# xiaohong-huang/RTK-Visual-Inertial-Navigation

Hardware: AMD Instinct MI355X
Metric: gauss_newton_iterations_per_sec (higher is better)
Workload: dtype f64; 1 GPU; BASELINE cfg4: batch of 512 independent cfg3 windows (20 keyframes, 300 features, 3000 observations, 19 IMU factors, 10 satellites x 20 epochs carrier-phase+pseudorange, gauge prior) over the job, 8 dogleg iterations per solve; windows=512, windows_rank0=512

## Files before the change

### rtk_visual_inertial_navigation_amd/csrc/swf_engine.hip

```cpp
#include <hip/hip_runtime.h>
#include <algorithm>
#include <chrono>
#include <cmath>
#include <cstdio>
#include <cstdlib>
#include <cstring>
#include <string>
#include <memory>
#include <thread>
#include <vector>
#include "../../include/swf_solver.h"
#include "swf_kernels2.h"
#include "swf_kernels3.h"
#include "swf_kernels4.h"
#include "swf_lambda.h"
#include "swf_features.h"
#include "swf_fixprior.h"
#include "swf_plan.h"

static thread_local std::string g_err;
static int fail(int code, const std::string& msg) { g_err = msg; return code; }
#define HIPCHK(x) do { hipError_t e_ = (x); if (e_ != hipSuccess) return fail(SWF_E_NODEVICE, std::string(#x) + ": " + hipGetErrorString(e_)); } while (0)

extern "C" const char* swf_last_error(void) { return g_err.c_str(); }
// ... 101 lines not shown
        bytes = (bytes + 255) & ~(size_t)255;
        if (v.empty() || v.back().used + bytes > v.back().cap) {
            size_t want = std::max(bytes, v.empty() ? first : std::min<size_t>(2 * v.back().cap, (size_t)256 << 20));
            Slab sl;
            sl.dev = (char*)slab_cache().acquire(want);
            if (!sl.dev) return nullptr;
            sl.cap = want;
            if (mirrored) sl.host.assign(want, 0);
            v.push_back(std::move(sl));
        }
        Slab& sl = v.back();
        void* p = sl.dev + sl.used;
        sl.used += bytes;
        return p;
    }
    template <class T> int put(const std::vector<T>& h, const T** out, size_t min_elems = 1) {
        size_t n = std::max(h.size(), min_elems), bytes = n * sizeof(T);
        void* p = bump(data, bytes, true, (size_t)4 << 20);
        if (!p) return -1;
        Slab& sl = data.back();
        char* m = sl.host.data() + ((char*)p - sl.dev);
        if (!h.empty()) memcpy(m, h.data(), h.size() * sizeof(T));
        if (sealed) {
            if (hipMemcpy(p, m, (bytes + 255) & ~(size_t)255, hipMemcpyHostToDevice) != hipSuccess) return -1;
            sl.flushed = sl.used;
        }
        *out = (const T*)p;
        return 0;
    }
    template <class T> int zeros(size_t n, T** out) {
        n = std::max<size_t>(n, 1);
        void* p = bump(zero, n * sizeof(T), false, (size_t)16 << 20);
        if (!p) return -1;
        if (sealed) { if (hipMemset(p, 0, n * sizeof(T)) != hipSuccess) return -1; zero.back().flushed = zero.back().used; }
        *out = (T*)p;
        return 0;
    }
    int flush() {
        for (Slab& sl : data) if (sl.used > sl.flushed) { if (hipMemcpy(sl.dev + sl.flushed, sl.host.data() + sl.flushed, sl.used - sl.flushed, hipMemcpyHostToDevice) != hipSuccess) return -1; sl.flushed = sl.used; }
        for (Slab& sl : zero) if (sl.used > sl.flushed) { if (hipMemset(sl.dev + sl.flushed, 0, sl.used - sl.flushed) != hipSuccess) return -1; sl.flushed = sl.used; }
        sealed = true;
        return 0;
    }
    void release() {
        for (Slab& sl : data) slab_cache().give(sl.dev, sl.cap);
        for (Slab& sl : zero) slab_cache().give(sl.dev, sl.cap);
        data.clear(); zero.clear(); sealed = false;
    }
};

struct swf_batch {
    int device = 0;
    DevBatch D{};
    DevPool pool;
    hipStream_t stream = nullptr;
    std::vector<WinRec> win;
    std::vector<HostWin> hw;
    int max_tiles = 0, max_prior_dim = 0, max_red = 0, min_red = 1 << 30, n_cu = 256;
    bool clc_imu[5] = { false, false, false, false, false };
    CompArgs CA{}; CompMeta CM{}; int n_comp = 0, comp_nmax = 0, comp_nmin = 1 << 30; long long comp_ne = 0;
    bool comp_eigen_root = false;
    void* h_sum = nullptr; size_t h_sum_bytes = 0;
    double* h_x = nullptr;
    double* co_pose0 = nullptr; double* co_sb0 = nullptr;
    int* mg_tail = nullptr; double* mg_A = nullptr; double* mg_b = nullptr; double* mg_J = nullptr; double* mg_r0 = nullptr; double* mg_w = nullptr; int* mg_rank = nullptr; double* mg_M = nullptr;
    bool mg_valid = false; int mg_ld = 0;
    bool mg_host = false; std::vector<double> h_mgA, h_mgJ, h_mgb, h_mgr0, h_mgw; std::vector<int> h_mgrank;
    double* mg_resM = nullptr; double* mg_resb = nullptr; int* mg_resok = nullptr;
    int* mg_rot = nullptr; int* mg_bjok = nullptr; unsigned long long* mg_crit = nullptr;
    int* tc_tail = nullptr; double* tc_A = nullptr; double* tc_Q = nullptr; double* tc_X = nullptr; int* tc_rank = nullptr; bool tc_valid = false; int tc_ld = 0;
    int* am_first = nullptr; int4* am_pairs = nullptr; double* am_rec = nullptr; int am_rec_ld = 0;
    bool am_valid = false, am_host = false; std::vector<double> h_am;
    std::vector<int> am_nb;
    std::vector<int> am_h_first; std::vector<int4> am_h_pairs;
    FixWin* fx_win = nullptr; int* fx_tailcol = nullptr; double* fx_A = nullptr; double* fx_b = nullptr; double* fx_J = nullptr; double* fx_r0 = nullptr;
    double* fx_eig = nullptr; double* fx_x0 = nullptr; int* fx_rank = nullptr; int* fx_applied = nullptr; int fx_ldn = 0, fx_ldx = 0;
    bool fx_valid = false, fx_host = false; FixPriorArgs fx_args{};
    std::vector<FixWin> fx_h_win; std::vector<int> fx_h_tailcol, fx_sel;
    std::vector<double> h_fxA, h_fxb, h_fxJ, h_fxr0, h_fxeig, h_fxx0; std::vector<int> h_fxrank, h_fxapplied;
    bool fc_built = false, fc_valid = false, fc_host = false; FeatArgs fc{}; char* fc_out = nullptr; size_t fc_bytes = 0; int fc_nfeat = 0;
    std::vector<int> fc_feat0; std::vector<char> h_fc;
    hipStream_t aux = nullptr; hipEvent_t ev_fork[3] = { nullptr, nullptr, nullptr };
    ~swf_batch() {
        if (aux) { (void)hipStreamSynchronize(aux); handle_cache().give(aux); }
        for (auto& e : ev_fork) handle_cache().give(e, false);
    }
    WinState* ws_primary = nullptr; WinState* ws_alt = nullptr; WinState* ws_alt2 = nullptr;
    bool no_decide_fuse = false;
    bool no_step_fuse = false;
    int n_pch_split = 0;
    bool no_spec = false;
    bool no_comp_fuse = false;
    bool lat_fuse = false;
    bool rr4_has15 = false, rr4_has16 = false;
    int rr_nmax = 256;
    bool L_full = false;
    int asm_programs = 0;
    int ls_qpb = 1, ls_var = 0, ls_kms = 8; bool ls_folded = false, s_direct = false;
    bool full_final = false;
    int ls_gqpb = 4;
    int timing = 0;
    swf_timing last{};
    std::vector<hipEvent_t> ev;
    std::vector<int> ev_kind;
    int ev_used = 0;
    int64_t jac_bytes = 0, proj_bytes = 0, chol_flops = 0, lm_schur_flops = 0, lm_schur_flops_sym = 0, lm_schur_mfma = 0;
    int last_mode = -1;
};

extern "C" int swf_batch_create(const swf_flat_window* const* windows, int32_t n, void* stream, swf_batch** out) {
    if (!windows || n <= 0 || !out) return fail(SWF_E_INVALID, "swf_batch_create: bad arguments");
    int ndev = 0;
    if (hipGetDeviceCount(&ndev) != hipSuccess || ndev <= 0)
        return fail(SWF_E_NODEVICE, "no HIP device: this library has no CPU fallback");
    int n_cu = 256;
    { int dev = 0; hipDeviceProp_t pr; if (hipGetDevice(&dev) == hipSuccess && hipGetDeviceProperties(&pr, dev) == hipSuccess && pr.multiProcessorCount > 0) n_cu = pr.multiProcessorCount; }
    Plan B;
    {
        std::string err;
        int prc = plan_build(windows, n, plan_shape_from_env(n_cu), B, err);
        if (prc != SWF_OK) return fail(prc, err);
    }
    std::unique_ptr<swf_batch> owner(new swf_batch());
    swf_batch* b = owner.get();
    b->device = current_device();
    b->stream = (hipStream_t)stream;
    b->n_cu = n_cu;
    b->no_comp_fuse = getenv("SWF_NO_COMP_FUSE") != nullptr;
    b->no_spec = getenv("SWF_NO_SPEC_EVAL") != nullptr;
    b->no_step_fuse = getenv("SWF_NO_STEP_FUSE") != nullptr;
    b->no_decide_fuse = getenv("SWF_NO_DECIDE_FUSE") != nullptr;
    b->full_final = getenv("SWF_FULL_FINAL_ELIM") != nullptr;
    b->max_tiles = B.max_tiles; b->max_prior_dim = B.max_prior_dim; b->max_red = B.max_red; b->min_red = B.min_red;
    b->rr_nmax = B.rr_nmax; b->rr4_has15 = B.rr4_has15; b->rr4_has16 = B.rr4_has16; b->n_pch_split = B.n_pch_split;
    b->lat_fuse = B.lat_fuse; b->asm_programs = B.asm_programs;
    b->ls_qpb = B.ls_qpb; b->ls_var = B.ls_var; b->ls_kms = B.ls_kms; b->ls_gqpb = B.ls_gqpb; b->ls_folded = B.ls_folded; b->s_direct = B.s_direct;
    for (int k = 0; k < 5; k++) b->clc_imu[k] = B.clc_imu[k];
    b->n_comp = B.n_comp; b->comp_nmax = B.comp_nmax; b->comp_nmin = B.comp_nmin; b->comp_ne = B.comp_ne;
    b->jac_bytes = B.jac_bytes; b->proj_bytes = B.proj_bytes; b->chol_flops = B.chol_flops;
    b->lm_schur_flops = B.lm_schur_flops; b->lm_schur_flops_sym = B.lm_schur_flops_sym; b->lm_schur_mfma = B.lm_schur_mfma;
    if (B.want_aux) {
        bool ok = (b->aux = handle_cache().stream()) != nullptr;
        for (int i = 0; i < 3 && ok; i++) ok = (b->ev_fork[i] = handle_cache().event(false)) != nullptr;
        if (!ok) { handle_cache().give(b->aux); b->aux = nullptr; }
    }
    DevBatch& D = b->D;
    DevPool& P = b->pool;
    int rc = 0;
    D.n_win = n; D.n_x = (int)B.n_x; D.n_loc_total = (int)B.n_loc; D.max_iter_trace = SWF_MAX_TRACE; D.rr_nmax = B.rr_nmax;
    D.n_lmb = B.n_lmb; D.n_pch = B.n_pch; D.n_proj = B.n_proj; D.n_lm = B.n_lm; D.n_fr = B.n_fr; D.n_fsb = B.n_fsb;
    D.n_gf = (int)B.gf.size(); D.n_imu = (int)B.imu_gf.size(); D.n_sc = (int)B.sc_gf.size(); D.n_prior = (int)B.prior_gf.size(); D.n_idp = (int)B.idp_gf.size();
    D.n_cl = (int)B.cl.size(); D.n_pair = (int)B.pair.size(); D.n_pd = B.n_pd; D.n_po = B.n_po; D.n_cle = B.n_cle;
    for (int k = 0; k < 5; k++) D.n_clc[k] = B.n_clc[k];
    D.as_max_ne = B.as_max_ne; D.as_max_nv = B.as_max_nv;
#define PUT(field) rc |= P.put(B.field, &D.field)
    PUT(win);
    PUT(lmb_rec); PUT(pch_q); PUT(pch_r0); PUT(prior_nch);
    PUT(blk_xoff); PUT(blk_loc); PUT(blk_gs);
    PUT(loc2x); PUT(x_var);
    PUT(p_win); PUT(p_xpose); PUT(p_xex); PUT(p_xlm);
    PUT(p_lpose); PUT(p_llm); PUT(p_fr); PUT(p_lm); PUT(p_uv);
    PUT(lm_win); PUT(lm_obs0); PUT(lm_loc); PUT(lm_col); PUT(lm_fmask);
    PUT(sch_c0); PUT(sch_rec); PUT(sch_km);
    PUT(fr_obs0); PUT(fr_obs); PUT(fr_red);
    PUT(fsb_rec);
    PUT(fsb_perm); PUT(fsb_foff);
    PUT(gf);
    PUT(s_x); PUT(s_loc); PUT(s_ls); PUT(s_joff); PUT(s_ccol);
    PUT(imu_pre); PUT(cp_dat); PUT(pr_dat); PUT(dop_dat); PUT(sp_w); PUT(gx_dat);
    PUT(imu_gf); PUT(sc_gf); PUT(prior_gf); PUT(idp_gf);
    PUT(sc_jt); PUT(imu_jt);
    PUT(prior_dim); PUT(prior_Joff); PUT(prior_roff); PUT(prior_x0off);
    PUT(prior_Jt);
    PUT(prior_colloc); PUT(prior_colcc); PUT(s_pcol); PUT(s_pxo);
    PUT(prior_J); PUT(prior_r0); PUT(prior_x0);
    PUT(cl); PUT(cl_fac); PUT(cl_frow); PUT(cm_loc); PUT(cm_ls); PUT(cm_col);
    PUT(cv_loc);
    PUT(pc_coff); PUT(pc_cld); PUT(pc_voff);
    PUT(asw); PUT(s_tnz);
    PUT(as_dst); PUT(as_cnt); PUT(as_src0); PUT(as_aux); PUT(as_src);
    PUT(av_loc); PUT(av_red); PUT(av_cnt); PUT(av_src0); PUT(av_i); PUT(av_src);
    PUT(pair_d); PUT(pair_o);
    PUT(cle_rec);
    for (int k = 0; k < 5; k++) PUT(clc_rec[k]);
#undef PUT
    {
        const double* ci = nullptr; const double* di = nullptr;
        rc |= P.put(B.C_init, &ci); rc |= P.put(B.dgraw_init, &di);
        D.C = (double*)ci; D.cv_dgraw = (double*)di;
    }
    CompArgs& A = b->CA; CompMeta& Mt = b->CM;
    const int nc = B.n_comp;
    if (nc) {
        A.n = nc; A.want_jac = 1; A.n_iq = (int)B.co_iq_f.size();
        rc |= P.put(B.co_M, &A.M); rc |= P.put(B.co_N, &A.N); rc |= P.put(B.co_eo, &A.e_off); rc |= P.put(B.co_no, &A.n_off);
        rc |= P.put(B.co_pno, &A.pn_off); rc |= P.put(B.co_nno, &A.nn_off); rc |= P.put(B.co_go, &A.g_off); rc |= P.put(B.co_g2o, &A.g2_off);
        { const double* t1 = nullptr; const double* t2 = nullptr; rc |= P.put(B.co_pose, &t1); rc |= P.put(B.co_sb, &t2); A.pose = (double*)t1; A.sb = (double*)t2; }
        { const double* t1 = nullptr; const double* t2 = nullptr; rc |= P.put(B.co_pose, &t1); rc |= P.put(B.co_sb, &t2); b->co_pose0 = (double*)t1; b->co_sb0 = (double*)t2; }
        rc |= P.put(B.co_pose_lin, &A.pose_lin); rc |= P.put(B.co_sb_lin, &A.sb_lin); rc |= P.put(B.co_Hpp, &A.Hpp); rc |= P.put(B.co_HpN, &A.HpN);
        rc |= P.put(B.co_rhs_p, &A.rhs_p); rc |= P.put(B.co_HNN, &A.HNN); rc |= P.put(B.co_rhsN, &A.rhsN); rc |= P.put(B.co_pre, &A.pre); rc |= P.put(B.co_pbgw, &A.pbgw);
        rc |= P.put(B.co_mid, &A.mid); rc |= P.put(B.co_H12, &A.H12);
        rc |= P.put(B.co_iq_f, &A.iq_f); rc |= P.put(B.co_iq_k, &A.iq_k);
        rc |= P.put(B.co_win, &Mt.win); rc |= P.put(B.co_xo_off, &Mt.xo_off); rc |= P.put(B.co_xo, &Mt.xo);
        rc |= P.put(B.co_Joff, &Mt.Joff); rc |= P.put(B.co_roff, &Mt.roff); rc |= P.put(B.co_x0off, &Mt.x0off); rc |= P.put(B.co_Coff, &Mt.Coff); rc |= P.put(B.co_voff, &Mt.voff);
        Mt.prior_J = (double*)D.prior_J; Mt.prior_Jt = (double*)D.prior_Jt; Mt.prior_r0 = (double*)D.prior_r0; Mt.prior_x0 = (double*)D.prior_x0;
    }
    rc |= P.zeros((size_t)B.fs_tot * FS_VAL, &D.fs_part);
    rc |= P.zeros((size_t)std::max<long long>(B.n_loc, 1), &D.jsc);
    rc |= P.zeros(B.n_x, &D.x); rc |= P.zeros(B.n_x, &D.xc); rc |= P.zeros(B.n_x, &D.x0);
    rc |= P.zeros(B.n_loc, &D.g); rc |= P.zeros(B.n_loc, &D.diag); rc |= P.zeros(B.n_loc, &D.rhs); rc |= P.zeros(B.n_loc, &D.vc);
    rc |= P.zeros(B.n_loc, &D.y); rc |= P.zeros(B.n_loc, &D.step);
    rc |= P.zeros(B.S_tot, &D.S); rc |= P.zeros(B.Lt_tot, &D.L);
    if (B.want_Linv) rc |= P.zeros((size_t)n * (CB_MAXT - 1) * 256, &D.Linv);
    if (B.want_Wk) rc |= P.zeros(B.Lt_tot, &D.Wk);
    rc |= P.zeros((size_t)n, &D.ws); rc |= P.zeros((size_t)n, &b->ws_alt); rc |= P.zeros((size_t)n, &b->ws_alt2); rc |= P.zeros((size_t)n * SWF_MAX_TRACE, &D.trace);
    b->ws_primary = D.ws;
    size_t np = (size_t)D.n_proj;
    rc |= P.zeros(2 * np, &D.p_r); rc |= P.zeros(12 * np, &D.p_Jp); rc |= P.zeros(6 * np, &D.p_Jl);
    rc |= P.zeros((size_t)std::max(1, D.n_fsb), &D.p_cpart); rc |= P.zeros((size_t)std::max(1, D.n_lmb), &D.p_apart);
    rc |= P.zeros((size_t)std::max(1, D.n_pch), &D.pr_cpart); rc |= P.zeros((size_t)std::max(1, D.n_pch), &D.pr_apart);
    rc |= P.zeros(6 * (size_t)D.n_lm, &D.lm_Einv); rc |= P.zeros(3 * (size_t)D.n_lm, &D.lm_g);
    rc |= P.zeros(B.P_tot * GEMM_SPLIT, &D.P);
    rc |= P.zeros((size_t)std::max(1, 6 * B.n_fr) * GEMM_SPLIT, &D.lmq);
    rc |= P.zeros((size_t)B.r_tot, &D.g_r); rc |= P.zeros((size_t)B.j_tot, &D.g_J);
    rc |= P.zeros((size_t)D.n_gf, &D.g_cost); rc |= P.zeros((size_t)D.n_gf, &D.g_aux);
    rc |= P.zeros((size_t)B.v_tot, &D.cv_graw); rc |= P.zeros((size_t)B.v_tot, &D.cv_cs);
    rc |= P.zeros((size_t)B.e_tot, &D.cE);
    if (nc) {
        const size_t ne = (size_t)B.co_eo[nc], nn = (size_t)B.co_no[nc], ng = (size_t)B.co_go[nc], ng2 = (size_t)B.co_g2o[nc];
        rc |= P.zeros(ne * 225, &A.hmn_inv); rc |= P.zeros(ne * 225, &A.hmn_2); rc |= P.zeros(ne * 225, &A.hmn_0);
        rc |= P.zeros((size_t)B.co_pno[nc], &A.hmn_N); rc |= P.zeros(ne * 15, &A.rhsmn);
        rc |= P.zeros(ng2, &A.Hd); rc |= P.zeros(ng, &A.rd); rc |= P.zeros(ng2, &A.Ld); rc |= P.zeros(ng, &A.r0);
        rc |= P.zeros((size_t)nc * 32, &A.old); rc |= P.zeros(nn, &A.N_old); rc |= P.zeros((size_t)nc, &A.history); rc |= P.zeros((size_t)nc, &A.status);
        rc |= P.zeros((size_t)nc * 32, &Mt.outer); rc |= P.zeros(nn, &Mt.Nv); rc |= P.zeros((size_t)nc, &Mt.active);
        A.outer = Mt.outer; A.Nv = Mt.Nv; A.active = Mt.active;
        rc |= P.zeros(ng, &A.res_out); rc |= P.zeros(ng2, &A.jac_out);
        rc |= P.zeros((ne + nc) * 450, &A.Jw); rc |= P.zeros((ne + nc) * 16, &A.rw);
        rc |= P.zeros((size_t)nc, &A.todo);
    }
    if (!rc) rc = P.flush();
    if (rc) { P.release(); return fail(SWF_E_NODEVICE, "device allocation / upload failed"); }
    b->win = std::move(B.win); b->hw = std::move(B.hw);
    *out = owner.release();
    int urc = swf_batch_upload_state(b);
    if (urc != SWF_OK) { swf_batch_destroy(b); *out = nullptr; return urc; }
    return SWF_OK;
}

extern "C" int swf_shard_partition(int32_t n, int32_t G, int32_t k, int32_t* first, int32_t* count) {
    if (n < 0 || G <= 0 || k < 0 || k >= G || !first || !count) return fail(SWF_E_INVALID, "swf_shard_partition: bad arguments");
    const int q = n / G, r = n % G;
    *first = k * q + std::min(k, r); *count = q + (k < r ? 1 : 0);
    return SWF_OK;
}

extern "C" int swf_batch_create_on(int32_t device, const swf_flat_window* const* windows, int32_t n, void* stream, swf_batch** out) {
    int ndev = 0;
    if (hipGetDeviceCount(&ndev) != hipSuccess || ndev <= 0) return fail(SWF_E_NODEVICE, "no HIP device: this library has no CPU fallback");
    if (device < 0 || device >= ndev || device >= SWF_MAX_DEVICES) return fail(SWF_E_INVALID, "swf_batch_create_on: no such device");
    DeviceGuard dg_(device);
    return swf_batch_create(windows, n, stream, out);
}

extern "C" int swf_batch_create_sharded(const swf_flat_window* const* windows, int32_t n, uint32_t device_mask,
                                        swf_batch** out_batches, int32_t* out_first, int32_t* out_count, int32_t* n_batches) {
    if (!windows || n <= 0 || !out_batches || !n_batches) return fail(SWF_E_INVALID, "swf_batch_create_sharded: bad arguments");
    int ndev = 0;
    if (hipGetDeviceCount(&ndev) != hipSuccess || ndev <= 0) return fail(SWF_E_NODEVICE, "no HIP device: this library has no CPU fallback");
    std::vector<int> devs;
    for (int d = 0; d < ndev && d < SWF_MAX_DEVICES; d++) if (device_mask == 0 || ((device_mask >> d) & 1u)) devs.push_back(d);
    if (devs.empty()) return fail(SWF_E_INVALID, "swf_batch_create_sharded: device_mask selects no visible device");
    const int G = (int)std::min<size_t>(devs.size(), (size_t)n);
    *n_batches = 0;
    for (int k = 0; k < G; k++) {
        int32_t lo = 0, cnt = 0;
        swf_shard_partition(n, G, k, &lo, &cnt);
        const int hi = lo + cnt;
        swf_batch* bk = nullptr;
        int rc = swf_batch_create_on(devs[k], windows + lo, hi - lo, nullptr, &bk);
        if (rc != SWF_OK) { for (int q = 0; q < *n_batches; q++) swf_batch_destroy(out_batches[q]); *n_batches = 0; return rc; }
        out_batches[k] = bk;
        if (out_first) out_first[k] = lo;
        if (out_count) out_count[k] = hi - lo;
        *n_batches = k + 1;
    }
    return SWF_OK;
}

extern "C" int swf_batch_device(swf_batch* b, int32_t* device) { if (!b || !device) return fail(SWF_E_INVALID, "bad arguments"); *device = b->device; return SWF_OK; }

extern "C" int swf_batch_destroy(swf_batch* b) {
    if (!b) return SWF_OK;
    DeviceGuard dg_(b->device);
    (void)hipStreamSynchronize(b->stream);
    if (b->aux) (void)hipStreamSynchronize(b->aux);
    for (auto& e : b->ev) handle_cache().give(e, true);
    if (b->h_x) (void)hipHostFree(b->h_x);
    if (b->h_sum) (void)hipHostFree(b->h_sum);
    b->pool.release();
    delete b;
    return SWF_OK;
}

extern "C" int swf_batch_upload_state(swf_batch* b) {
    DeviceGuard dg_(b ? b->device : -1);
    if (!b) return fail(SWF_E_INVALID, "null batch");
    const size_t nx = (size_t)b->D.n_x;
    if (!b->h_x && nx) HIPCHK(hipHostMalloc((void**)&b->h_x, nx * sizeof(double), hipHostMallocDefault));
    double* xh = b->h_x;
    for (size_t i = 0; i < b->win.size(); i++) {
        const HostWin& h = b->hw[i];
        double* p = xh + b->win[i].x_base;
        memcpy(p, h.pose, sizeof(double) * 7 * h.n_pose); p += 7 * h.n_pose;
        memcpy(p, h.sb, sizeof(double) * 9 * h.n_sb); p += 9 * h.n_sb;
        memcpy(p, h.lm, sizeof(double) * 3 * h.n_lm); p += 3 * h.n_lm;
        memcpy(p, h.sc, sizeof(double) * h.n_sc);
    }
    HIPCHK(hipMemcpyAsync(b->D.x, xh, nx * sizeof(double), hipMemcpyHostToDevice, b->stream));
    HIPCHK(hipMemcpyAsync(b->D.x0, b->D.x, nx * sizeof(double), hipMemcpyDeviceToDevice, b->stream));
    HIPCHK(hipMemcpyAsync(b->D.xc, b->D.x, nx * sizeof(double), hipMemcpyDeviceToDevice, b->stream));
    std::vector<double> hp, hs;
    if (b->n_comp) {
        hp.resize((size_t)b->comp_ne * 7); hs.resize((size_t)b->comp_ne * 9);
        for (size_t i = 0; i < b->win.size(); i++) {
            const HostWin& h = b->hw[i];
            if (!h.comp_ne) continue;
            memcpy(hp.data() + (size_t)h.comp_e0 * 7, h.comp_pose, sizeof(double) * 7 * h.comp_ne);
            memcpy(hs.data() + (size_t)h.comp_e0 * 9, h.comp_sb, sizeof(double) * 9 * h.comp_ne);
        }
        HIPCHK(hipMemcpyAsync(b->co_pose0, hp.data(), hp.size() * sizeof(double), hipMemcpyHostToDevice, b->stream));
        HIPCHK(hipMemcpyAsync(b->co_sb0, hs.data(), hs.size() * sizeof(double), hipMemcpyHostToDevice, b->stream));
        HIPCHK(hipMemcpyAsync(b->CA.pose, b->co_pose0, hp.size() * sizeof(double), hipMemcpyDeviceToDevice, b->stream));
        HIPCHK(hipMemcpyAsync(b->CA.sb, b->co_sb0, hs.size() * sizeof(double), hipMemcpyDeviceToDevice, b->stream));
        HIPCHK(hipMemsetAsync(b->CA.history, 0, (size_t)b->n_comp * sizeof(int), b->stream));
// ... 83 lines not shown
            }
            slot = b->ev_used++;
            b->ev_kind.push_back(kind);
            (void)hipEventRecord(b->ev[2 * slot], bst);
        }
        ~Bracket() { if (slot >= 0) (void)hipEventRecord(L.b->ev[2 * slot + 1], bst); }
    };
    static int nb(size_t n, int per) { return (int)((n + per - 1) / per); }
    bool comp_fused = false;
    bool comp_fuse_ok(int write_S) const {
        const DevBatch& D = b->D;
        if (!b->n_comp || !write_S || b->no_comp_fuse || !b->lat_fuse || b->aux || b->comp_eigen_root) return false;
        if (b->comp_nmax > CO_SMALLN || b->ls_var > 1 || !D.n_lm || D.n_imu || D.n_idp || b->max_prior_dim > PRIOR_LDS_DIM) return false;
        if (D.n_clc[0] || D.n_clc[1]) return false;
        const int crow = (b->n_comp + D.n_win - 1) / D.n_win;
        return (long long)D.n_win * (GEMM_SPLIT / b->ls_qpb + crow) <= b->n_cu;
    }
    void lin_eval(int write_S, bool spec = false) {
        DevBatch Dv = b->D; Dv.spec = spec ? 1 : 0;
        const DevBatch& D = Dv;
        comp_fused = !spec && comp_fuse_ok(write_S);
        if (comp_fused) {
            hipLaunchKernelGGL(k_comp_gather_prep, dim3(b->n_comp), dim3(256), 0, st, D, b->CA, b->CM);
            Segs S{}; S.e[0] = D.n_fsb; S.e[1] = S.e[0] + nb(D.n_sc, 256);
            {
                Bracket t(*this, SWF_K_EVAL_PS);
                hipLaunchKernelGGL(k_eval_ps_comp_imu, dim3(S.e[1] + (b->CA.n_iq + 7) / 8), dim3(256), 0, st, D, S, b->CA);
            }
            {
                Bracket t(*this, SWF_K_LM_SCHUR);
                lm_qpb = b->ls_qpb; lm_folded = b->ls_folded;
                const int np = GEMM_SPLIT / b->ls_qpb, crow = (b->n_comp + D.n_win - 1) / D.n_win;
                const int qpb = b->ls_qpb, sd = b->s_direct ? 1 : 0, kms = b->ls_kms;
                dim3 grid(D.n_win, np + crow);
                if (b->ls_var == 0) hipLaunchKernelGGL((k_lm_comp<8, 2, 2, 80>), grid, dim3(LS_NT(8, 2)), 0, st, D, O, b->CA, b->CM, qpb, 0, kms, sd, np);
                else hipLaunchKernelGGL((k_lm_comp<8, 5, 2, 144>), grid, dim3(LS_NT(8, 2)), 0, st, D, O, b->CA, b->CM, qpb, 0, kms, sd, np);
                lm_next = ls_tiles_per_launch();
            }
            if (D.n_prior) {
                Segs P{}; P.e[2] = D.n_pch;
                hipLaunchKernelGGL((k_eval_ps<true, true>), dim3(P.e[2]), dim3(256), 0, st, D, P);
            }
            return;
        }
        if (b->n_comp && !spec) {
            const bool wide = b->n_comp <= 2 * b->n_cu;
            {
            hipLaunchKernelGGL(k_comp_gather_prep, dim3(b->n_comp), dim3(256), 0, st, D, b->CA, b->CM);
            hipLaunchKernelGGL(k_comp_imu, dim3((b->CA.n_iq + 7) / 8), dim3(256), 0, st, b->CA);
            if (b->comp_nmin <= CO_SMALLN) {
                if (wide) hipLaunchKernelGGL((k_comp_elim<CO_SMALLN, 1024>), dim3(b->n_comp), dim3(1024), 0, st, b->CA, 0);
                else {
                    if (b->comp_nmin <= CO_TINYN) hipLaunchKernelGGL((k_comp_elim<CO_TINYN, 256>), dim3(b->n_comp), dim3(256), 0, st, b->CA, 0);
                    if (b->comp_nmax > CO_TINYN) hipLaunchKernelGGL((k_comp_elim<CO_SMALLN, 256>), dim3(b->n_comp), dim3(256), 0, st, b->CA, CO_TINYN + 1);
                }
            }
            if (b->comp_nmax > CO_SMALLN) {
                if (wide) hipLaunchKernelGGL((k_comp_elim<CO_MAXN, 1024>), dim3(b->n_comp), dim3(1024), 0, st, b->CA, CO_SMALLN + 1);
                else hipLaunchKernelGGL((k_comp_elim<CO_MAXN, 256>), dim3(b->n_comp), dim3(256), 0, st, b->CA, CO_SMALLN + 1);
            }
            if (b->comp_eigen_root) {
                if (b->comp_nmax <= CO_SMALLN) hipLaunchKernelGGL(k_comp_eigroot<CO_SMALLN>, dim3(b->n_comp), dim3(256), 0, st, b->CA);
                else hipLaunchKernelGGL(k_comp_eigroot<CO_MAXN>, dim3(b->n_comp), dim3(512), 0, st, b->CA);
            }
            hipLaunchKernelGGL(k_comp_scatter, dim3(b->n_comp), dim3(256), 0, st, D, b->CA, b->CM);
            }
        }
        const bool fork = b->aux && !spec;
        hipStream_t sa = fork ? b->aux : st;
        if (fork) { (void)hipEventRecord(b->ev_fork[0], st); (void)hipStreamWaitEvent(b->aux, b->ev_fork[0], 0); }
        bool imu_fused = false;
        if (D.n_proj + D.n_sc + D.n_prior) {
            Bracket t(*this, SWF_K_EVAL_PS);
            bool pf = b->max_prior_dim <= PRIOR_LDS_DIM;
            Segs S{}; S.e[0] = D.n_fsb; S.e[1] = S.e[0] + nb(D.n_sc, 256); S.e[2] = S.e[1] + (pf ? D.n_pch : 0);
            imu_fused = b->lat_fuse && D.n_imu > 0;
            S.e[3] = S.e[2] + (imu_fused ? nb(D.n_imu, IMU_FPB) : 0);
            if (imu_fused) hipLaunchKernelGGL((k_eval_ps<true, true, true>), dim3(S.e[3]), dim3(256), 0, st, D, S);
            else hipLaunchKernelGGL((k_eval_ps<true, true>), dim3(S.e[2]), dim3(256), 0, st, D, S);
        }
        if (D.n_idp) hipLaunchKernelGGL(k_eval_idp<true>, GRID(D.n_idp, 128), dim3(128), 0, st, D);
        if (D.n_prior && b->max_prior_dim > PRIOR_LDS_DIM) { Bracket t(*this, SWF_K_EVAL_PRIOR); hipLaunchKernelGGL(k_eval_prior<true>, dim3(D.n_pch), dim3(256), (2 * b->max_prior_dim + 16) * sizeof(double), st, D); }
        if (fork) (void)hipEventRecord(b->ev_fork[1], st);
        if (D.n_imu && !imu_fused) { Bracket t(*this, SWF_K_EVAL_IMU, sa); hipLaunchKernelGGL(k_eval_imu<true>, GRID(D.n_imu, IMU_FPB), dim3(IMU_FPB * IMU_LPF), 0, sa, D); }
    }
    void lin_elim(int write_S) {
        DevBatch& D = b->D;
        bool clq_fused = false;
        if (comp_fused) {
            Bracket t(*this, SWF_K_CLIQUE_ELIM);
            if (D.n_clc[3]) {
                hipLaunchKernelGGL(k_clique_big2, dim3(D.n_clc[3] + D.n_clc[2]), dim3(CB_NT), 0, st, D, O);
                if (D.n_clc[4]) hipLaunchKernelGGL(k_clique_tall<false>, dim3(D.n_clc[4]), dim3(256), 0, st, D, O);
            } else if (D.n_clc[4] + D.n_clc[2]) hipLaunchKernelGGL(k_clique_tall2, dim3(D.n_clc[4] + D.n_clc[2]), dim3(256), 0, st, D, O);
        } else if (D.n_lm) {
            Bracket t(*this, write_S ? SWF_K_LM_SCHUR : SWF_K_LM_ELIM);
            lm_qpb = b->ls_qpb; lm_folded = b->ls_folded;
            if (!write_S && !b->full_final) {
                dim3 grid(D.n_win, GEMM_SPLIT / b->ls_gqpb);
                hipLaunchKernelGGL((k_lm_schur<8, 2, 2, 80, false, true>), grid, dim3(256), 0, st, D, O, b->ls_gqpb, 0, 0, 0);
            } else if (!write_S) {
                dim3 grid(D.n_win, GEMM_SPLIT / lm_qpb);
                hipLaunchKernelGGL((k_lm_schur<8, 2, 2, 80, false>), grid, dim3(256), 0, st, D, O, lm_qpb, 0, 0, 0);
            } else {
                const int crow = D.n_win > 0 ? (D.n_clc[2] + D.n_win - 1) / D.n_win : 0;
                clq_fused = clq_fuse_ok();
                lm_launch(0, st, clq_fused ? crow : 0);
                lm_next = ls_tiles_per_launch();
            }
        }
        {
            hipStream_t sa = b->aux ? b->aux : st;
            if (b->aux) (void)hipStreamWaitEvent(b->aux, b->ev_fork[1], 0);
            auto cstream = [&](int cls) { return (b->aux && !b->clc_imu[cls]) ? st : sa; };
            if (comp_fused) {
                for (; lm_next < b->max_tiles; lm_next += ls_tiles_per_launch()) { Bracket t(*this, SWF_K_LM_SCHUR, sa); lm_launch(lm_next, sa); }
            } else {
            const bool grad = !write_S && !b->full_final;
            if (D.n_clc[1]) {
                Bracket t(*this, SWF_K_CLIQUE_ELIM, cstream(1));
                if (grad) hipLaunchKernelGGL((k_clique_elim<32, 48, 9, 1, true>), dim3(D.n_clc[1]), dim3(64), 0, cstream(1), D, O);
                else hipLaunchKernelGGL((k_clique_elim<32, 48, 9, 1>), dim3(D.n_clc[1]), dim3(64), 0, cstream(1), D, O);
            }
            if (D.n_clc[0]) {
                Bracket t(*this, SWF_K_CLIQUE_ELIM, cstream(0));
                if (grad) hipLaunchKernelGGL((k_clique_elim<48, 32, 1, 0, true>), dim3(D.n_clc[0]), dim3(64), 0, cstream(0), D, O);
                else hipLaunchKernelGGL((k_clique_elim<48, 32, 1, 0>), dim3(D.n_clc[0]), dim3(64), 0, cstream(0), D, O);
            }
            if (D.n_clc[2] && !clq_fused) {
                Bracket t(*this, SWF_K_CLIQUE_ELIM, cstream(2));
                if (b->lat_fuse) {
                    if (grad) hipLaunchKernelGGL(k_clique_elim4<true>, dim3(D.n_clc[2]), dim3(256), 0, cstream(2), D, O);
                    else hipLaunchKernelGGL(k_clique_elim4<false>, dim3(D.n_clc[2]), dim3(256), 0, cstream(2), D, O);
                }
                else if (grad) hipLaunchKernelGGL((k_clique_elim<64, 64, 9, 2, true>), dim3(D.n_clc[2]), dim3(64), 0, cstream(2), D, O);
                else hipLaunchKernelGGL((k_clique_elim<64, 64, 9, 2>), dim3(D.n_clc[2]), dim3(64), 0, cstream(2), D, O);
            }
            if (D.n_clc[3]) { Bracket t(*this, SWF_K_CLIQUE_ELIM, cstream(3)); hipLaunchKernelGGL(k_clique_big, dim3(D.n_clc[3]), dim3(CB_NT), 0, cstream(3), D, O); }
            if (D.n_clc[4]) {
                Bracket t(*this, SWF_K_CLIQUE_ELIM, cstream(4));
                if (grad) hipLaunchKernelGGL(k_clique_tall<true>, dim3(D.n_clc[4]), dim3(256), 0, cstream(4), D, O);
                else hipLaunchKernelGGL(k_clique_tall<false>, dim3(D.n_clc[4]), dim3(256), 0, cstream(4), D, O);
            }
            if (write_S && D.n_lm) {
                for (; lm_next < b->max_tiles; lm_next += ls_tiles_per_launch()) { Bracket t(*this, SWF_K_LM_SCHUR, sa); lm_launch(lm_next, sa); }
            }
            }
            if (b->aux) (void)hipEventRecord(b->ev_fork[2], b->aux);
        }
        if (b->n_pch_split) hipLaunchKernelGGL(k_prior_graw, dim3(D.n_pch), dim3(256), 0, st, D);
        if (b->aux) (void)hipStreamWaitEvent(st, b->ev_fork[2], 0);
        if (D.n_pd) {
            Bracket t(*this, SWF_K_ASSEMBLE);
            const int nbS = write_S ? nb((size_t)D.as_max_ne, 256) : 0, nbV = nb((size_t)D.as_max_nv, 256);
            hipLaunchKernelGGL(k_assemble_flat, dim3(nbS + nbV, D.n_win), dim3(256), 0, st, D, O, write_S, nbS);
        }
    }
    void reduced() {
        DevBatch& D = b->D;
        Bracket t(*this, SWF_K_CHOL);
        if (b->max_red <= CB_NMAX) {
            if (b->min_red <= b->rr_nmax) {
                if (b->min_red <= 224) hipLaunchKernelGGL(k_chol_rr4<14>, dim3(D.n_win), dim3(R4_NT), 0, st, D, export_full ? 1 : 0);
                if (b->rr4_has15) hipLaunchKernelGGL(k_chol_rr4<15>, dim3(D.n_win), dim3(R4_NT), 0, st, D, export_full ? 1 : 0);
                if (b->rr4_has16) hipLaunchKernelGGL(k_chol_rr4<16>, dim3(D.n_win), dim3(R4_NT), 0, st, D, export_full ? 1 : 0);
            }
            if (b->max_red > b->rr_nmax && D.Wk) {
                const int Tc = (b->max_red + 15) / 16;
                const int nbw = std::max(1, std::min(CC_NB, b->n_cu / D.n_win));
                for (int j = 0; j < Tc; j += 2) hipLaunchKernelGGL(k_chol_col, dim3(D.n_win, nbw), dim3(CC_NT), 0, st, D, j);
                hipLaunchKernelGGL(k_chol_big<true>, dim3(D.n_win), dim3(1024), 0, st, D);
            } else if (b->max_red > b->rr_nmax) hipLaunchKernelGGL(k_chol_big<false>, dim3(D.n_win), dim3(1024), 0, st, D);
        }
        else if (b->max_red + 1 <= 256) hipLaunchKernelGGL(k_chol_solve<256>, dim3(D.n_win), dim3(256), 0, st, D);
        else hipLaunchKernelGGL(k_chol_solve<1024>, dim3(D.n_win), dim3(1024), 0, st, D);
    }
    void step_rest() {
        DevBatch& D = b->D;
        {
            Bracket t(*this, SWF_K_POST_CHOL);
            Segs S{};
            S.e[0] = D.n_lmb; S.e[1] = S.e[0] + nb((size_t)D.n_cle * 16, 256);
            S.e[2] = S.e[1]; S.e[3] = S.e[2] + nb(D.n_sc, 256);
            S.e[4] = S.e[3] + nb((size_t)D.n_imu * 16, 256); S.e[5] = S.e[4] + D.n_pch;
            if (D.n_win < b->n_cu) { if (S.e[5]) hipLaunchKernelGGL(k_post_chol<0>, dim3(S.e[5]), dim3(256), 0, st, D, O, S); }
            else {
                if (S.e[0]) hipLaunchKernelGGL(k_post_chol<1>, dim3(S.e[0]), dim3(256), 0, st, D, O, S);
                if (S.e[5] > S.e[0]) hipLaunchKernelGGL(k_post_chol<2>, dim3(S.e[5] - S.e[0]), dim3(256), 0, st, D, O, S);
            }
        }
        if (!step_fused) dogleg();
    }
    bool step_fused = false;
    void dogleg() {
        DevBatch& D = b->D;
        Bracket t(*this, SWF_K_DOGLEG);
        if (b->lat_fuse) hipLaunchKernelGGL((k_dogleg<16, 4>), dim3(D.n_win), dim3(CTL_NT), 0, st, D, O);
        else hipLaunchKernelGGL((k_dogleg<4, 2>), dim3(D.n_win), dim3(CTL_NT), 0, st, D, O);
    }
    bool clq_fuse_ok() const {
        const DevBatch& D = b->D;
        const int crow = D.n_win > 0 ? (D.n_clc[2] + D.n_win - 1) / D.n_win : 0;
        return b->lat_fuse && b->ls_var <= 2 && D.n_lm > 0 && D.n_clc[2] > 0 && !D.n_clc[0] && !D.n_clc[1]
               && (long long)D.n_win * (GEMM_SPLIT / b->ls_qpb + crow) <= b->n_cu;
    }
    bool decide_fuse_ok() const { return step_fused && !b->no_decide_fuse && clq_fuse_ok() && b->ls_var <= 1 && b->max_tiles <= ls_tiles_per_launch(); }
    bool step_fuse_ok() const {
        const DevBatch& D = b->D;
        return b->lat_fuse && !b->no_step_fuse && !b->aux && D.n_win == 1 && b->win[0].x_n <= XCL_MAX && b->max_prior_dim <= PRIOR_LDS_DIM && !D.n_idp
               && D.n_fsb + nb(D.n_sc, 256) + D.n_pch + nb(D.n_imu, IMU_FPB) > 0;
    }
    void step_eval(bool jac = true) {
        DevBatch& D = b->D;
        Bracket t(*this, jac ? SWF_K_EVAL_PS : SWF_K_POST_DOGLEG);
        Segs S{}; S.e[0] = D.n_fsb; S.e[1] = S.e[0] + nb(D.n_sc, 256); S.e[2] = S.e[1] + D.n_pch;
        const bool imu = D.n_imu > 0;
        S.e[3] = S.e[2] + (imu ? nb(D.n_imu, IMU_FPB) : 0);
        WinState* out = ws_next(D.ws);
        WinState* clr = decide_fused ? ws_next(out) : nullptr;
        if (!jac) {
            if (imu) hipLaunchKernelGGL((k_step_eval<true, false>), dim3(S.e[3]), dim3(256), 0, st, D, O, S, out, b->win[0], clr);
            else hipLaunchKernelGGL((k_step_eval<false, false>), dim3(S.e[2]), dim3(256), 0, st, D, O, S, out, b->win[0], clr);
        } else if (imu) hipLaunchKernelGGL((k_step_eval<true>), dim3(S.e[3]), dim3(256), 0, st, D, O, S, out, b->win[0], clr);
        else hipLaunchKernelGGL((k_step_eval<false>), dim3(S.e[2]), dim3(256), 0, st, D, O, S, out, b->win[0], clr);
        D.ws = out;
    }
    void decide() {
        DevBatch& D = b->D;
        { Bracket t(*this, SWF_K_DECIDE); hipLaunchKernelGGL(k_decide, dim3(D.n_win), dim3(CTL_NT), 0, st, D, O); }
    }
    void cand_eval() {
        DevBatch& D = b->D;
        {
            Bracket t(*this, SWF_K_POST_DOGLEG);
            Segs S{};
            S.e[0] = D.n_fsb; S.e[1] = S.e[0] + nb(D.n_sc, 256);
            S.e[2] = S.e[1] + (b->max_prior_dim <= PRIOR_LDS_DIM ? D.n_pch : 0);
            bool fuse_imu = D.n_win < b->n_cu;
            S.e[3] = S.e[2] + (fuse_imu ? nb(D.n_imu, IMU_FPB) : 0);
            if (S.e[3] && fuse_imu) hipLaunchKernelGGL((k_post_dogleg<true, 0>), dim3(S.e[3]), dim3(256), 0, st, D, O, S);
            else if (S.e[3]) {
                if (S.e[0]) hipLaunchKernelGGL((k_post_dogleg<false, 1>), dim3(S.e[0]), dim3(256), 0, st, D, O, S);
                if (S.e[3] > S.e[0]) hipLaunchKernelGGL((k_post_dogleg<false, 2>), dim3(S.e[3] - S.e[0]), dim3(256), 0, st, D, O, S);
            }
            if (!fuse_imu && D.n_imu) hipLaunchKernelGGL(k_eval_imu<false>, GRID(D.n_imu, IMU_FPB), dim3(IMU_FPB * IMU_LPF), 0, st, D);
            if (D.n_idp) hipLaunchKernelGGL(k_eval_idp<false>, GRID(D.n_idp, 128), dim3(128), 0, st, D);
        }
        {
            Bracket t(*this, SWF_K_CAND_EVAL);
            if (D.n_prior && b->max_prior_dim > PRIOR_LDS_DIM) hipLaunchKernelGGL(k_eval_prior<false>, dim3(D.n_pch), dim3(256), (2 * b->max_prior_dim + 16) * sizeof(double), st, D);
        }
        decide();
    }
};
}

extern "C" int swf_batch_solve(swf_batch* b, const swf_options* opt) {
    DeviceGuard dg_(b ? b->device : -1);
    if (!b || !opt) return fail(SWF_E_INVALID, "swf_batch_solve: bad arguments");
    if (opt->max_num_iterations < 0 || opt->max_num_iterations >= SWF_MAX_TRACE) return fail(SWF_E_INVALID, "max_num_iterations out of range");
    if (opt->trust_region_strategy != SWF_DOGLEG && opt->trust_region_strategy != SWF_LEVENBERG_MARQUARDT) return fail(SWF_E_INVALID, "unknown trust_region_strategy");
    if (opt->composite_root != SWF_ROOT_PIVOTED_CHOLESKY && opt->composite_root != SWF_ROOT_EIGEN) return fail(SWF_E_INVALID, "unknown composite_root");
    b->comp_eigen_root = opt->composite_root == SWF_ROOT_EIGEN;
    if (opt->jacobi_scaling && opt->trust_region_strategy == SWF_DOGLEG && opt->step_mode == SWF_OPTIMIZE)
        return fail(SWF_E_UNSUPPORTED, "jacobi_scaling with the dogleg strategy (the reference sets jacobi_scaling = 0 wherever it selects DOGLEG: R/swf/swf.cpp:26-27)");
    DevBatch& D = b->D;
    Launcher L{ b, to_devopt(opt), b->stream };
    L.export_full = opt->step_mode == SWF_ASSEMBLE_ELIMINATE_ONLY;
    b->L_full = L.export_full || b->min_red > b->rr_nmax || b->max_red > CB_NMAX;
    hipStream_t st = b->stream;
    b->ev_used = 0; b->ev_kind.clear();
    int nlin = 0;
    {
        Launcher::Bracket total(L, SWF_K_TOTAL);
        hipLaunchKernelGGL(k_init, dim3(D.n_win), dim3(256), 0, st, D, L.O);
        auto LIN = [&](int write_S) { L.lin_eval(write_S); L.lin_elim(write_S); nlin++; };
        LIN(1);
        if (opt->step_mode == SWF_ASSEMBLE_ELIMINATE_ONLY) {
            L.reduced();
        } else {
            const bool spec = opt->trust_region_strategy == SWF_DOGLEG && !b->n_comp && !b->no_spec;
            L.step_fused = L.step_fuse_ok();
            for (int it = 1; it <= opt->max_num_iterations; it++) {
                L.reduced();
                L.step_rest();
                if (spec) {
                    L.decide_fused = it < opt->max_num_iterations && L.decide_fuse_ok();
                    if (L.step_fused) L.step_eval(); else L.lin_eval(1, true);
                    if (!L.decide_fused) L.decide();
                    if (b->aux) (void)hipEventRecord(b->ev_fork[1], st);
                    L.lin_elim(it < opt->max_num_iterations ? 1 : 0); nlin++;
                }
                else {
                    if (L.step_fused) { L.decide_fused = false; L.step_eval(false); L.decide(); } else L.cand_eval();
                    LIN(it < opt->max_num_iterations ? 1 : 0);
                }
            }
        }
        hipLaunchKernelGGL(k_finalize, dim3(D.n_win), dim3(256), 0, st, D, L.O, b->ws_primary);
        D.ws = b->ws_primary;
    }
    HIPCHK(hipGetLastError());
    b->last = swf_timing{};
    b->last.jacobian_bytes = b->jac_bytes; b->last.proj_bytes = b->proj_bytes; b->last.chol_flops = b->chol_flops;
    b->last.lm_schur_flops = b->lm_schur_flops; b->last.n_obs = b->D.n_proj;
    b->last.lm_schur_flops_sym = b->lm_schur_flops_sym; b->last.lm_schur_mfma = b->lm_schur_mfma;
    b->last.n_linearizations = nlin;
    b->last_mode = opt->step_mode; b->mg_valid = false; b->tc_valid = false; b->am_valid = false; b->fx_valid = false; b->fc_valid = false;
// ... 494 lines not shown
    const int rc = swf_internal_feature_launch(b->fc, b->stream);
    if (rc) return rc;
    b->fc_valid = true; b->fc_host = false;
    return SWF_OK;
}

extern "C" int swf_batch_get_feature_check(swf_batch* b, int32_t w, double* mean_err, double* depth, int32_t* n_obs, uint8_t* flags,
                                           int32_t* rejected, int32_t* n_rejected, int32_t* n_feat) {
    DeviceGuard dg_(b ? b->device : -1);
    if (!b || w < 0 || w >= (int)b->win.size()) return fail(SWF_E_INVALID, "bad window index");
    if (!b->fc_valid) return fail(SWF_E_STATE, "swf_batch_get_feature_check before swf_batch_check_features (or after a new solve / state upload)");
    if (!b->fc_host) {
        b->h_fc.resize(b->fc_bytes);
        HIPCHK(hipMemcpyAsync(b->h_fc.data(), b->fc_out, b->fc_bytes, hipMemcpyDeviceToHost, b->stream));
        HIPCHK(hipStreamSynchronize(b->stream));
        b->fc_host = true;
    }
    const size_t nf = (size_t)b->fc_nfeat, nw = b->win.size(), f0 = (size_t)b->fc_feat0[w], n = (size_t)b->fc_feat0[w + 1] - f0;
    const double* h_mean = (const double*)b->h_fc.data(); const double* h_depth = h_mean + nf;
    const int* h_nobs = (const int*)(h_depth + nf); const int* h_rej = h_nobs + nf; const int* h_nrej = h_rej + nf;
    const unsigned char* h_flags = (const unsigned char*)(h_nrej + nw);
    if (n_feat) *n_feat = (int32_t)n;
    if (mean_err) memcpy(mean_err, h_mean + f0, n * sizeof(double));
    if (depth) memcpy(depth, h_depth + f0, n * sizeof(double));
    if (n_obs) memcpy(n_obs, h_nobs + f0, n * sizeof(int));
    if (flags) memcpy(flags, h_flags + f0, n);
    if (rejected) memcpy(rejected, h_rej + f0, (size_t)h_nrej[w] * sizeof(int));
    if (n_rejected) *n_rejected = h_nrej[w];
    return SWF_OK;
}

extern "C" int swf_batch_get_prior(swf_batch* b, int32_t w, double* A, double* bv, double* J, double* r0, double* eig, int32_t* n_out, int32_t* rank) {
    DeviceGuard dg_(b ? b->device : -1);
    if (!b || w < 0 || w >= (int)b->win.size()) return fail(SWF_E_INVALID, "bad window index");
    if (!b->mg_valid) return fail(SWF_E_STATE, "swf_batch_get_prior before swf_batch_marginalize");
    HIPCHK(hipStreamSynchronize(b->stream));
    size_t n = (size_t)b->hw[w].tail_dim, o2 = (size_t)w * b->mg_ld * b->mg_ld, o1 = (size_t)w * b->mg_ld;
    if (n_out) *n_out = (int32_t)n;
    const size_t nw = b->win.size(), tot2 = nw * b->mg_ld * b->mg_ld, tot1 = nw * b->mg_ld;
    if (nw >= 8 && tot2 <= ((size_t)1 << 23)) {
        if (!b->mg_host) {
            b->h_mgA.resize(tot2); b->h_mgJ.resize(tot2); b->h_mgb.resize(tot1); b->h_mgr0.resize(tot1); b->h_mgw.resize(tot1); b->h_mgrank.resize(nw);
            HIPCHK(hipMemcpy(b->h_mgA.data(), b->mg_A, tot2 * sizeof(double), hipMemcpyDeviceToHost));
            HIPCHK(hipMemcpy(b->h_mgJ.data(), b->mg_J, tot2 * sizeof(double), hipMemcpyDeviceToHost));
            HIPCHK(hipMemcpy(b->h_mgb.data(), b->mg_b, tot1 * sizeof(double), hipMemcpyDeviceToHost));
            HIPCHK(hipMemcpy(b->h_mgr0.data(), b->mg_r0, tot1 * sizeof(double), hipMemcpyDeviceToHost));
            HIPCHK(hipMemcpy(b->h_mgw.data(), b->mg_w, tot1 * sizeof(double), hipMemcpyDeviceToHost));
            HIPCHK(hipMemcpy(b->h_mgrank.data(), b->mg_rank, nw * sizeof(int), hipMemcpyDeviceToHost));
            b->mg_host = true;
        }
        if (A) memcpy(A, b->h_mgA.data() + o2, n * n * sizeof(double));
        if (J) memcpy(J, b->h_mgJ.data() + o2, n * n * sizeof(double));
        if (bv) memcpy(bv, b->h_mgb.data() + o1, n * sizeof(double));
        if (r0) memcpy(r0, b->h_mgr0.data() + o1, n * sizeof(double));
        if (eig) memcpy(eig, b->h_mgw.data() + o1, n * sizeof(double));
        if (rank) *rank = b->h_mgrank[(size_t)w];
        return SWF_OK;
    }
    if (A) HIPCHK(hipMemcpy(A, b->mg_A + o2, n * n * sizeof(double), hipMemcpyDeviceToHost));
    if (J) HIPCHK(hipMemcpy(J, b->mg_J + o2, n * n * sizeof(double), hipMemcpyDeviceToHost));
    if (bv) HIPCHK(hipMemcpy(bv, b->mg_b + o1, n * sizeof(double), hipMemcpyDeviceToHost));
    if (r0) HIPCHK(hipMemcpy(r0, b->mg_r0 + o1, n * sizeof(double), hipMemcpyDeviceToHost));
    if (eig) HIPCHK(hipMemcpy(eig, b->mg_w + o1, n * sizeof(double), hipMemcpyDeviceToHost));
    if (rank) HIPCHK(hipMemcpy(rank, b->mg_rank + w, sizeof(int32_t), hipMemcpyDeviceToHost));
    return SWF_OK;
}

extern "C" int swf_batch_export_vectors(swf_batch* b, int32_t w, double* grad, double* diag, double* y) {
    DeviceGuard dg_(b ? b->device : -1);
    if (!b || w < 0 || w >= (int)b->win.size()) return fail(SWF_E_INVALID, "bad window index");
    const WinRec& W = b->win[w];
    size_t n = (size_t)W.n_loc;
    HIPCHK(hipStreamSynchronize(b->stream));
    if (grad) HIPCHK(hipMemcpy(grad, b->D.g + W.loc_base, n * sizeof(double), hipMemcpyDeviceToHost));
    if (diag) HIPCHK(hipMemcpy(diag, b->D.diag + W.loc_base, n * sizeof(double), hipMemcpyDeviceToHost));
    if (y) HIPCHK(hipMemcpy(y, b->D.y + W.loc_base, n * sizeof(double), hipMemcpyDeviceToHost));
    return SWF_OK;
}

extern "C" int swf_batch_export_jacobian(swf_batch* b, int32_t w, double* r, double* J, int32_t* n_res_out, int32_t* n_loc_out) {
    DeviceGuard dg_(b ? b->device : -1);
    if (!b || w < 0 || w >= (int)b->win.size()) return fail(SWF_E_INVALID, "bad window index");
    const WinRec& W = b->win[w];
    const DevBatch& D = b->D;
    const int ngf = W.gf1 - W.gf0, nobs = W.proj1 - W.proj0;
    std::vector<GFac> gf((size_t)std::max(ngf, 0));
    HIPCHK(hipStreamSynchronize(b->stream));
    if (ngf > 0) HIPCHK(hipMemcpy(gf.data(), D.gf + W.gf0, (size_t)ngf * sizeof(GFac), hipMemcpyDeviceToHost));
    const int nproj_all = b->hw[w].n_proj_all;
    int nres = 2 * nproj_all;
    for (const GFac& G : gf) if (G.type != GF_PROJX) nres += G.nres;
    if (n_res_out) *n_res_out = nres;
    if (n_loc_out) *n_loc_out = W.n_loc;
    if (!r && !J) return SWF_OK;
    if (b->last_mode < 0) return fail(SWF_E_STATE, "swf_batch_export_jacobian before any solve");
    const size_t nl = (size_t)W.n_loc, N = (size_t)D.n_proj;
    if (J) memset(J, 0, (size_t)nres * nl * sizeof(double));
    auto dl = [&](void* dst, const void* src, size_t bytes) { return bytes == 0 || hipMemcpy(dst, src, bytes, hipMemcpyDeviceToHost) == hipSuccess; };
    bool ok = true;
    if (nobs > 0) {
        std::vector<double> pr(2 * (size_t)nobs), Jp(12 * (size_t)nobs), Jl(6 * (size_t)nobs);
        std::vector<int> lp((size_t)nobs), ll((size_t)nobs);
        for (int k = 0; k < 2; k++) ok &= dl(pr.data() + (size_t)k * nobs, D.p_r + k * N + W.proj0, (size_t)nobs * 8);
        for (int k = 0; k < 12; k++) ok &= dl(Jp.data() + (size_t)k * nobs, D.p_Jp + k * N + W.proj0, (size_t)nobs * 8);
        for (int k = 0; k < 6; k++) ok &= dl(Jl.data() + (size_t)k * nobs, D.p_Jl + k * N + W.proj0, (size_t)nobs * 8);
        ok &= dl(lp.data(), D.p_lpose + W.proj0, (size_t)nobs * 4); ok &= dl(ll.data(), D.p_llm + W.proj0, (size_t)nobs * 4);
        if (!ok) return fail(SWF_E_NODEVICE, "download failed");
        for (int q = 0; q < nobs; q++) {
            const size_t row = 2 * (size_t)b->hw[w].p_orig[q];
            for (int a = 0; a < 2; a++) {
                if (r) r[row + a] = pr[(size_t)a * nobs + q];
                if (!J) continue;
                if (lp[q] >= 0) for (int c = 0; c < 6; c++) J[(row + a) * nl + (lp[q] - W.loc_base) + c] = (c < 3 && ll[q] >= 0) ? -Jl[(size_t)(a * 3 + c) * nobs + q] : Jp[(size_t)(a * 6 + c) * nobs + q];
                if (ll[q] >= 0) for (int c = 0; c < 3; c++) J[(row + a) * nl + (ll[q] - W.loc_base) + c] = Jl[(size_t)(a * 3 + c) * nobs + q];
            }
        }
    }
    size_t row_seq = 2 * (size_t)nproj_all;
    for (const GFac& G : gf) {
        const size_t row = G.type == GF_PROJX ? 2 * (size_t)G.pad : row_seq;
        std::vector<int> sloc((size_t)G.nslot), sls((size_t)G.nslot), sj((size_t)G.nslot), spc((size_t)G.nslot);
        ok &= dl(sloc.data(), D.s_loc + G.slot0, (size_t)G.nslot * 4); ok &= dl(sls.data(), D.s_ls + G.slot0, (size_t)G.nslot * 4);
        ok &= dl(sj.data(), D.s_joff + G.slot0, (size_t)G.nslot * 4); ok &= dl(spc.data(), D.s_pcol + G.slot0, (size_t)G.nslot * 4);
        if (r) ok &= dl(r + row, D.g_r + G.roff, (size_t)G.nres * 8);
        if (J && G.type == GF_PRIOR) {
            int dim = 0; long long jo = 0;
            ok &= dl(&dim, D.prior_dim + G.data, 4); ok &= dl(&jo, D.prior_Joff + G.data, 8);
            std::vector<double> PJ((size_t)dim * dim);
            ok &= dl(PJ.data(), D.prior_J + jo, PJ.size() * 8);
            for (int sl = 0; sl < G.nslot; sl++) {
                if (sloc[sl] < 0) continue;
                for (int k = 0; k < G.nres; k++) for (int c = 0; c < sls[sl]; c++)
                    J[(row + k) * nl + (sloc[sl] - W.loc_base) + c] = PJ[(size_t)k * dim + spc[sl] + c];
            }
        } else if (J) {
            for (int sl = 0; sl < G.nslot; sl++) {
                if (sloc[sl] < 0 || sj[sl] < 0) continue;
                std::vector<double> blk((size_t)sls[sl] * G.jld);
                ok &= dl(blk.data(), D.g_J + sj[sl], (((size_t)sls[sl] - 1) * G.jld + G.nres) * 8);
                for (int k = 0; k < G.nres; k++) for (int c = 0; c < sls[sl]; c++)
                    J[(row + k) * nl + (sloc[sl] - W.loc_base) + c] = blk[(size_t)c * G.jld + k];
            }
        }
        if (G.type != GF_PROJX) row_seq += G.nres;
    }
    if (!ok) return fail(SWF_E_NODEVICE, "download failed");
    return SWF_OK;
}

extern "C" int swf_debug_plan_check(const swf_flat_window* const* windows, int32_t n, int32_t n_cu, int32_t ls_variant, int32_t ls_qpb, int32_t ls_grad_qpb,
                                    int32_t flags, int32_t corrupt_table, int32_t corrupt_index, int32_t* info) {
    if (!windows || n <= 0 || n_cu <= 0) return fail(SWF_E_INVALID, "swf_debug_plan_check: bad arguments");
    PlanShape sh;
    sh.n_cu = n_cu; sh.ls_variant = ls_variant; sh.ls_qpb = ls_qpb; sh.ls_grad_qpb = ls_grad_qpb; sh.no_lat_fuse = flags & 1; sh.no_chol_col = flags & 2;
    Plan B; std::string err;
    int rc = plan_build(windows, n, sh, B, err);
    if (rc != SWF_OK) return fail(rc, err);
    if (corrupt_table) {
        const size_t i = (size_t)corrupt_index;
        if (corrupt_table == 1 && i < B.as_src.size()) B.as_src[i] += 1 << 28;
        else if (corrupt_table == 2 && i < B.sch_rec.size()) B.sch_rec[i] ^= 1;
        else if (corrupt_table == 3 && i < B.s_tnz.size() && B.s_tnz[i]) B.s_tnz[i] &= B.s_tnz[i] - 1;
        else if (corrupt_table == 4 && i < B.prior_colloc.size()) B.prior_colloc[i] ^= 1;
        else if (corrupt_table == 5 && i < B.loc2x.size()) B.loc2x[i] ^= 1;
        else if (corrupt_table == 6 && i < B.co_voff.size()) B.co_voff[i] += 1 << 28;
        else if (corrupt_table == 7 && i < B.pair_o.size()) B.pair_o[i].q_base += 8;
        else return fail(SWF_E_INVALID, "swf_debug_plan_check: nothing to corrupt there");
    }
    if (info) {
        const int v[12] = { B.ls_var, B.ls_qpb, B.ls_gqpb, B.ls_folded, B.lat_fuse, B.want_aux, B.want_Linv, B.want_Wk, B.asm_programs, B.n_pch_split, B.max_red, B.n_pch };
        for (int k = 0; k < 12; k++) info[k] = v[k];
    }
    rc = plan_validate(B, err);
    return rc == SWF_OK ? SWF_OK : fail(rc, err);
}

#ifdef SWF_PROFILE_CHOL
extern "C" int swf_debug_chol_stamps(unsigned long long* out) {
    if (hipDeviceSynchronize() != hipSuccess) return SWF_E_NODEVICE;
    if (hipMemcpyFromSymbol(out, HIP_SYMBOL(g_chol_stamps), 64 * sizeof(unsigned long long)) != hipSuccess) return SWF_E_NODEVICE;
    return SWF_OK;
}
#endif

#ifdef SWF_PROFILE_CHOLW
extern "C" int swf_debug_chol_wstep(int step) {
    if (hipDeviceSynchronize() != hipSuccess) return SWF_E_NODEVICE;
    unsigned long long z[16 * 8] = { 0 };
    if (hipMemcpyToSymbol(HIP_SYMBOL(g_chol_wst), z, sizeof(z)) != hipSuccess) return SWF_E_NODEVICE;
    if (hipMemcpyToSymbol(HIP_SYMBOL(g_chol_wstep), &step, sizeof(int)) != hipSuccess) return SWF_E_NODEVICE;
    return SWF_OK;
}
extern "C" int swf_debug_chol_wstamps(unsigned long long* out) {
    if (hipDeviceSynchronize() != hipSuccess) return SWF_E_NODEVICE;
    if (hipMemcpyFromSymbol(out, HIP_SYMBOL(g_chol_wst), 16 * 8 * sizeof(unsigned long long)) != hipSuccess) return SWF_E_NODEVICE;
    return SWF_OK;
}
extern "C" int swf_debug_chol_pstamps(unsigned long long* out) {
    if (hipDeviceSynchronize() != hipSuccess) return SWF_E_NODEVICE;
    if (hipMemcpyFromSymbol(out, HIP_SYMBOL(g_chol_pst), 16 * sizeof(unsigned long long)) != hipSuccess) return SWF_E_NODEVICE;
    return SWF_OK;
}
extern "C" int swf_debug_chol_cstamps(unsigned long long* out) {
    if (hipDeviceSynchronize() != hipSuccess) return SWF_E_NODEVICE;
    if (hipMemcpyFromSymbol(out, HIP_SYMBOL(g_chol_cst), 32 * sizeof(unsigned long long)) != hipSuccess) return SWF_E_NODEVICE;
    return SWF_OK;
}
#endif

#ifdef SWF_PROFILE_DOG
extern "C" int swf_debug_dog_stamps(unsigned long long* out) {
    if (hipDeviceSynchronize() != hipSuccess) return SWF_E_NODEVICE;
    if (hipMemcpyFromSymbol(out, HIP_SYMBOL(g_dog_stamps), 16 * sizeof(unsigned long long)) != hipSuccess) return SWF_E_NODEVICE;
    return SWF_OK;
}
#endif

#ifdef SWF_PROFILE_CLQ
extern "C" int swf_debug_clq_stamps(unsigned long long* out) {
    if (hipDeviceSynchronize() != hipSuccess) return SWF_E_NODEVICE;
    if (hipMemcpyFromSymbol(out, HIP_SYMBOL(g_clq_stamps), 16 * sizeof(unsigned long long)) != hipSuccess) return SWF_E_NODEVICE;
    return SWF_OK;
}
#endif

#ifdef SWF_PROFILE_EVAL
extern "C" int swf_debug_eval_stamps(unsigned long long* out) {
    if (hipDeviceSynchronize() != hipSuccess) return SWF_E_NODEVICE;
    if (hipMemcpyFromSymbol(out, HIP_SYMBOL(g_eval_stamps), 16 * sizeof(unsigned long long)) != hipSuccess) return SWF_E_NODEVICE;
    return SWF_OK;
}
#endif

#ifdef SWF_PROFILE_GEMM
extern "C" int swf_debug_gemm_stamps(unsigned long long* out) {
    if (hipDeviceSynchronize() != hipSuccess) return SWF_E_NODEVICE;
    if (hipMemcpyFromSymbol(out, HIP_SYMBOL(g_gemm_stamps), 16 * sizeof(unsigned long long)) != hipSuccess) return SWF_E_NODEVICE;
    return SWF_OK;
}
#endif


struct swf_composite {
    CompArgs A{};
    std::vector<void*> bufs;
    int n = 0, nmax = 0, nmin = 0; long long sumM = 0, sumN = 0, sumG = 0, sumG2 = 0;
    std::vector<int> M;
    bool eigen_root = false;
    hipStream_t stream = nullptr;
    ~swf_composite() { for (void* p : bufs) (void)hipFree(p); }
};

extern "C" int swf_composite_destroy(swf_composite* c) { delete c; return SWF_OK; }

extern "C" int swf_composite_create(int32_t n, const int32_t* M, const int32_t* N, const double* pose, const double* sb,
                                    const double* pose_lin, const double* sb_lin, const double* Hpp, const double* HpN,
                                    const double* rhs_p, const double* HNN, const double* rhsN, const double* pre,
                                    const double pbg[3], const double gw[3], void* stream, swf_composite** out) {
    if (!out || n <= 0 || !M || !N || !pose || !sb || !pose_lin || !sb_lin || !Hpp || !HpN || !rhs_p || !HNN || !rhsN || !pre || !pbg || !gw)
        return fail(SWF_E_INVALID, "swf_composite_create: null argument");
    std::vector<int> eo(n + 1, 0), no(n + 1, 0);
    std::vector<long long> pno(n + 1, 0), nno(n + 1, 0), go(n + 1, 0), g2o(n + 1, 0);
    int nmax_ = 0, nmin_ = 1 << 30;
    for (int f = 0; f < n; f++) {
        if (M[f] < 1) return fail(SWF_E_INVALID, "composite factor without hidden epochs");
        if (N[f] < 0 || N[f] > CO_MAXN) return fail(SWF_E_UNSUPPORTED, "composite factor with more than 64 ambiguities");
        nmax_ = std::max(nmax_, (int)N[f]); nmin_ = std::min(nmin_, (int)N[f]);
        eo[f + 1] = eo[f] + M[f]; no[f + 1] = no[f] + N[f];
        pno[f + 1] = pno[f] + 15LL * M[f] * N[f]; nno[f + 1] = nno[f] + (long long)N[f] * N[f];
        go[f + 1] = go[f] + 30 + N[f]; g2o[f + 1] = g2o[f] + (long long)(30 + N[f]) * (30 + N[f]);
    }
    std::unique_ptr<swf_composite> c(new swf_composite());
    c->n = n; c->nmax = nmax_; c->nmin = nmin_; c->sumM = eo[n]; c->sumN = no[n]; c->sumG = go[n]; c->sumG2 = g2o[n]; c->stream = (hipStream_t)stream;
    bool bad = false;
    auto up = [&](const void* src, size_t bytes) -> void* {
        void* d = nullptr;
        if (hipMalloc(&d, std::max<size_t>(bytes, 8)) != hipSuccess) { bad = true; return nullptr; }
        c->bufs.push_back(d);
        if (src) { if (hipMemcpy(d, src, bytes, hipMemcpyHostToDevice) != hipSuccess) bad = true; }
        else if (hipMemset(d, 0, std::max<size_t>(bytes, 8)) != hipSuccess) bad = true;
        return d;
    };
    CompArgs& A = c->A;
    const size_t D = sizeof(double);
    A.n = n;
    A.M = (const int*)up(M, n * sizeof(int)); A.N = (const int*)up(N, n * sizeof(int));
    A.e_off = (const int*)up(eo.data(), (n + 1) * sizeof(int)); A.n_off = (const int*)up(no.data(), (n + 1) * sizeof(int));
    A.pn_off = (const long long*)up(pno.data(), (n + 1) * sizeof(long long)); A.nn_off = (const long long*)up(nno.data(), (n + 1) * sizeof(long long));
    A.g_off = (const long long*)up(go.data(), (n + 1) * sizeof(long long)); A.g2_off = (const long long*)up(g2o.data(), (n + 1) * sizeof(long long));
    A.pose = (double*)up(pose, c->sumM * 7 * D); A.sb = (double*)up(sb, c->sumM * 9 * D);
    A.pose_lin = (const double*)up(pose_lin, c->sumM * 7 * D); A.sb_lin = (const double*)up(sb_lin, c->sumM * 9 * D);
    A.Hpp = (const double*)up(Hpp, c->sumM * 225 * D); A.HpN = (const double*)up(HpN, pno[n] * D); A.rhs_p = (const double*)up(rhs_p, c->sumM * 15 * D);
    A.HNN = (const double*)up(HNN, nno[n] * D); A.rhsN = (const double*)up(rhsN, c->sumN * D);
    A.pre = (const double*)up(pre, (size_t)(c->sumM + n) * SWF_PRE_DOUBLES * D);
    {
        std::vector<double> pg((size_t)n * 6);
        for (int f = 0; f < n; f++) for (int k = 0; k < 3; k++) { pg[(size_t)f * 6 + k] = pbg[k]; pg[(size_t)f * 6 + 3 + k] = gw[k]; }
        A.pbgw = (const double*)up(pg.data(), pg.size() * D);
    }
    A.active = nullptr;
    A.hmn_inv = (double*)up(nullptr, c->sumM * 225 * D); A.hmn_2 = (double*)up(nullptr, c->sumM * 225 * D); A.hmn_0 = (double*)up(nullptr, c->sumM * 225 * D);
    A.hmn_N = (double*)up(nullptr, pno[n] * D); A.rhsmn = (double*)up(nullptr, c->sumM * 15 * D);
    A.Hd = (double*)up(nullptr, c->sumG2 * D); A.rd = (double*)up(nullptr, c->sumG * D); A.Ld = (double*)up(nullptr, c->sumG2 * D); A.r0 = (double*)up(nullptr, c->sumG * D);
    A.old = (double*)up(nullptr, (size_t)n * 32 * D); A.N_old = (double*)up(nullptr, c->sumN * D);
    A.history = (int*)up(nullptr, n * sizeof(int)); A.status = (int*)up(nullptr, n * sizeof(int));
    A.outer = (const double*)up(nullptr, (size_t)n * 32 * D); A.Nv = (const double*)up(nullptr, c->sumN * D);
    A.res_out = (double*)up(nullptr, c->sumG * D); A.jac_out = (double*)up(nullptr, c->sumG2 * D);
    A.Jw = (double*)up(nullptr, (size_t)(c->sumM + n) * 450 * D); A.rw = (double*)up(nullptr, (size_t)(c->sumM + n) * 16 * D);
    {
        std::vector<int> qf, qk;
        for (int f = 0; f < n; f++) for (int k = 0; k <= M[f]; k++) { qf.push_back(f); qk.push_back(k); }
        A.n_iq = (int)qf.size();
        A.iq_f = (const int*)up(qf.data(), qf.size() * sizeof(int)); A.iq_k = (const int*)up(qk.data(), qk.size() * sizeof(int));
        A.todo = (int*)up(nullptr, n * sizeof(int));
    }
    A.mid = (const int*)up(nullptr, n * sizeof(int)); A.H12 = (const double*)up(nullptr, (size_t)n * 225 * D);
    c->M.assign(M, M + n);
    if (bad) return fail(SWF_E_NODEVICE, "swf_composite_create: device allocation / upload failed");
    *out = c.release();
// ... 53 lines not shown
```

### rtk_visual_inertial_navigation_amd/csrc/swf_kernels.h

```cpp
#pragma once
#include "swf_dev.h"

struct DevOpt {
    int max_iter, step_mode, strategy, jacobi;
    double r0, max_r, min_r, min_rel_dec, ftol, gtol, ptol, min_mu, max_mu, mu_inc, min_diag, max_diag;
};



__device__ __forceinline__ double damp_diag(const DevOpt& O, double d, double* jsc_slot, bool first) {
    if (!O.jacobi) return clampd(d, O.min_diag, O.max_diag);
    double q;
    if (first) { double r = 1.0 + sqrt(d > 0.0 ? d : 0.0); q = r * r; *jsc_slot = q; }
    else q = *jsc_slot;
    return clampd(d / q, O.min_diag, O.max_diag) * q;
}

template <bool JAC> __device__ __forceinline__ bool eval_gate(const DevBatch& B, const WinState& s) { return B.spec == 2 ? true : (JAC && !B.spec) ? s.need_lin != 0 : s.eval_cand != 0; }
template <bool JAC> __device__ __forceinline__ const double* eval_src(const DevBatch& B) { return (JAC && !B.spec) ? B.x : B.xc; }

#include "swf_gnss_range.h"

template <bool JAC, bool STORE>
__device__ __forceinline__ double proj_core(const DevBatch& B, int i, const WinRec& W, const double* P, const double* E, const double* X,
// ... 1121 lines not shown
            for (int j = 0; j < MAXE; j++) {
                double v = (lane < de && j < de) ? Me[lane * d + j] : 0.0;
                if (j == lane) v += s.mu * (lane < de ? damp_diag(O, v, B.jsc + C.e_loc + lane, s.iter == 0) : clampd(v, O.min_diag, O.max_diag));
                row[j] = v; row[MAXE + j] = (j == lane) ? 1.0 : 0.0;
            }
            bool bad = false;
#pragma unroll
            for (int k = 0; k < MAXE; k++) {
                if (k < de) {
                    double piv = readlane_d(row[k], k);
                    if (!(piv > 0.0)) bad = true;
                    double ip = __builtin_amdgcn_rcp(piv);
                    ip = ip * (2.0 - piv * ip); ip = ip * (2.0 - piv * ip);
                    double aik = row[k];
#pragma unroll
                    for (int j = 0; j < 2 * MAXE; j++) {
                        double akj = readlane_d(row[j], k) * ip;
                        row[j] = (lane == k) ? akj : row[j] - aik * akj;
                    }
                }
            }
            if (bad && lane == 0) { s.lin_fail = 1; bad_s = 1; }
            if (lane < MAXE) {
#pragma unroll
                for (int j = 0; j < MAXE; j++) Ei[lane][j] = (!bad && lane < de && j < de) ? row[MAXE + j] : 0.0;
            }
        }
        __syncthreads();
        if (bad_s) return;
        if (tid < 9) { double v = 0; for (int j = 0; j < de; j++) v += Ei[tid][j] * ge[j]; Eg[tid] = v; }
        for (int e = tid; e < de * df; e += CB_NT) {
            const int a = e / df, j = e - a * df;
            double tj = 0;
            for (int b2 = 0; b2 < de; b2++) tj += Ei[a][b2] * Me[b2 * d + de + j];
            Tt[a * df + j] = tj;
        }
        __syncthreads();
        double* E = B.cE + C.e_off;
        for (int e = tid; e < de * de; e += CB_NT) E[e] = Ei[e / de][e % de];
        for (int j = tid; j < df; j += CB_NT) {
            double v = 0;
            for (int a = 0; a < de; a++) { E[de * de + a * df + j] = Me[a * d + de + j]; v -= Me[a * d + de + j] * Eg[a]; }
            B.cv_cs[C.v_off + j] = v;
        }
        if (tid < de) E[de * de + de * df + tid] = ge[tid];
    } else {
        for (int j = tid; j < df; j += CB_NT) B.cv_cs[C.v_off + j] = 0.0;
    }
    const long long ntri = (long long)df * (df + 1) / 2;
    for (long long t = tid; t < ntri; t += CB_NT) {
        int i = (int)((sqrt(8.0 * (double)t + 1.0) - 1.0) * 0.5);
        while ((long long)(i + 1) * (i + 2) / 2 <= t) i++;
        while ((long long)i * (i + 1) / 2 > t) i--;
        int j = (int)(t - (long long)i * (i + 1) / 2);
        const double* ci = Jc + (size_t)(de + i) * ldj; const double* cj = Jc + (size_t)(de + j) * ldj;
        double m = 0;
#pragma unroll 4
        for (int k = 0; k < nrow; k++) m += ci[k] * cj[k];
        for (int a = 0; a < de; a++) m -= Me[a * d + de + i] * Tt[a * df + j];
        Cm[(size_t)i * df + j] = m; Cm[(size_t)j * df + i] = m;
    }
}
#undef bad_s
__global__ void __launch_bounds__(CB_NT) k_clique_big(DevBatch B, DevOpt O) {
    __shared__ double Me[CB_MAXED];
    __shared__ double Tt[CB_MAXED];
    __shared__ double Ei[9][9];
    __shared__ double Eg[9], ge[9];
    __shared__ int bad_sv;
    __shared__ double Jl[CB_LDS_J];
    if ((int)blockIdx.x >= B.n_clc[3]) return;
    const Clique& C = B.clc_rec[3][blockIdx.x];
    if ((long long)(C.n_rows | 1) * (C.d_e + C.d_f) <= CB_LDS_J) d_clique_big<true>(B, O, Me, Tt, Ei, Eg, ge, &bad_sv, Jl);
    else d_clique_big<false>(B, O, Me, Tt, Ei, Eg, ge, &bad_sv, Jl);
}
#define CB_LDS_J2 11008
__global__ void __launch_bounds__(CB_NT) k_clique_big2(DevBatch B, DevOpt O) {
    if ((int)blockIdx.x >= B.n_clc[3]) {
        static_assert(CB_NT >= 256, "k_clique_big2: the clique rows keep the four waves d_clique_elim<..., NW = 4> synchronises");
        if (threadIdx.x >= 256) return;
        d_clique_elim<64, 64, 9, 2, 8, 4, 4>(B, O, (int)blockIdx.x - B.n_clc[3]);
        return;
    }
    __shared__ double Me[CB_MAXED];
    __shared__ double Tt[CB_MAXED];
    __shared__ double Ei[9][9];
    __shared__ double Eg[9], ge[9];
    __shared__ int bad_sv;
    __shared__ double Jl[CB_LDS_J2];
    const Clique& C = B.clc_rec[3][blockIdx.x];
    if ((long long)(C.n_rows | 1) * (C.d_e + C.d_f) <= CB_LDS_J2) d_clique_big<true>(B, O, Me, Tt, Ei, Eg, ge, &bad_sv, Jl);
    else d_clique_big<false>(B, O, Me, Tt, Ei, Eg, ge, &bad_sv, Jl);
}

#define FS_HALF 14
__device__ __forceinline__ void d_eval_proj_fs(const DevBatch& B, int blk, double (*V)[FS_HALF], int* foff) {
    ProjBlk<true> Q;
    Q.load(B, blk);
#ifdef SWF_PROFILE_EVAL
    unsigned long long& te_ = Q.te_;
#endif
    const int tid = threadIdx.x, cnt = Q.cnt, nF = Q.nF, rk = Q.rk;
    if (!Q.gate) return;
    if (tid <= nF) foff[tid] = Q.fo;
    for (int e = tid + FS_BLK; e <= nF; e += FS_BLK) foff[e] = B.fsb_foff[Q.foff0 + e];
    double keep[20];
#pragma unroll
    for (int k = 0; k < 20; k++) keep[k] = 0.0;
    double cost = 0.0;
    if (tid < cnt) cost = d_eval_proj_at<true>(B, Q, keep);
    EST(3);
    {
        __shared__ double csum[16];
        cost = block_sum(cost, csum);
        if (tid == 0) B.p_cpart[blk] = cost;
    }
    EST(4);
    double val[FS_VAL];
    {
        const double* a = keep; const double* b = keep + 6;
        int k = 0;
#pragma unroll
        for (int i = 0; i < 6; i++)
#pragma unroll
            for (int j = 0; j <= i; j++) val[k++] = a[i] * a[j] + b[i] * b[j];
#pragma unroll
        for (int i = 0; i < 6; i++) val[21 + i] = a[i] * keep[12] + b[i] * keep[13];
    }
    double* out = B.fs_part + (size_t)Q.out0 * FS_VAL;
#pragma unroll
    for (int half = 0; half < 2; half++) {
        const int v0 = half * FS_HALF, nv = half == 0 ? FS_HALF : FS_VAL - FS_HALF;
        if (half) __syncthreads();
        if (tid < cnt) {
#pragma unroll
            for (int k = 0; k < FS_HALF; k++) if (k < nv) V[rk][k] = val[v0 + k];
        }
        __syncthreads();
        for (int e = tid; e < nF * nv; e += FS_BLK) {
            int f = e / nv, v = e - f * nv;
            double acc = 0;
            int q = foff[f], q1 = foff[f + 1];
            for (; q + 4 <= q1; q += 4) {
                double x0 = V[q][v], x1 = V[q + 1][v], x2 = V[q + 2][v], x3 = V[q + 3][v];
                acc += x0; acc += x1; acc += x2; acc += x3;
            }
            for (; q < q1; q++) acc += V[q][v];
            out[f * FS_VAL + v0 + v] = acc;
        }
    }
    EST(5);
}

__device__ __forceinline__ double as_sum(const double* base, const int* src, int n, int add = 0) {
    double v = 0;
    int c = 0;
    for (; c + 4 <= n; c += 4) {
        const int i0 = src[c], i1 = src[c + 1], i2 = src[c + 2], i3 = src[c + 3];
        const double x0 = base[i0 + add], x1 = base[i1 + add], x2 = base[i2 + add], x3 = base[i3 + add];
        v += x0; v += x1; v += x2; v += x3;
    }
    for (; c < n; c++) v += base[src[c] + add];
    return v;
}
__global__ void __launch_bounds__(256) k_assemble_flat(DevBatch B, DevOpt O, int write_S, int nbS) {
    const AsmWin& A = B.asw[blockIdx.y];
    const WinState& s = B.ws[A.win];
    if (!s.need_lin) return;
    const int tid = threadIdx.x;
    if ((int)blockIdx.x < nbS) {
        if (!write_S) return;
        const int e = blockIdx.x * 256 + tid;
        if (e >= A.ne) return;
        const int k = A.se0 + e;
        const unsigned cnt = B.as_cnt[k];
        const int nC = AS_NC(cnt), nP = AS_NP(cnt), nH = AS_NH(cnt);
        const int* src = B.as_src + B.as_src0[k];
        const int dst = B.as_dst[k];
        double* S = B.S + A.S_base;
        const double* C = B.C + A.C_base;
        const double sold = AS_SOLD(cnt) ? S[dst] : 0.0;
        double v = as_sum(C, src, nC);
        if (AS_SOLD(cnt)) v = sold + v;
        else if (nP) v -= as_sum(B.P + A.P_base, src + nC, nP);
        double hs = 0;
        if (nH) { hs = as_sum(B.fs_part + (size_t)A.fs_base * FS_VAL, src + nC + nP, nH); v += hs; }
        if (AS_DIAG(cnt)) {
            const double* dgr = B.cv_dgraw + A.v_base;
            const int* sd = src + nC + nP + nH;
            double dg = hs;
            int c = 0;
            for (; c + 4 <= nC; c += 4) { const double x0 = dgr[sd[c]], x1 = dgr[sd[c + 1]], x2 = dgr[sd[c + 2]], x3 = dgr[sd[c + 3]]; dg += x0; dg += x1; dg += x2; dg += x3; }
            for (; c < nC; c++) dg += dgr[sd[c]];
            v += s.mu * damp_diag(O, dg, B.jsc + A.loc_base + B.as_aux[k], s.iter == 0);
        }
        S[dst] = v;
        return;
    }
    const int e = (blockIdx.x - nbS) * 256 + tid;
    if (e >= A.nv) return;
    const int k = A.ve0 + e;
    const unsigned cnt = B.av_cnt[k];
    const int nC = AS_NC(cnt), nQ = AS_NP(cnt), nH = AS_NH(cnt);
    const int* src = B.av_src + B.av_src0[k];
    double gi = 0, dg = 0, cs = 0;
    if (nH) {
        const double* fs = B.fs_part + (size_t)A.fs_base * FS_VAL;
        const int i = B.av_i[k];
        const double g0 = as_sum(fs, src, nH, 21 + i), h0 = as_sum(fs, src, nH, i * (i + 1) / 2 + i);
        const double q0 = as_sum(B.lmq + A.q_base, src + nH + nC, nQ);
        gi = g0; dg = h0; cs = -q0;
    }
    {
        const double* gr = B.cv_graw + A.v_base; const double* dgr = B.cv_dgraw + A.v_base; const double* csr = B.cv_cs + A.v_base;
        int c = 0;
        for (; c + 2 <= nC; c += 2) {
            const int v0 = src[nH + c], v1 = src[nH + c + 1];
            const double a0 = gr[v0], b0 = dgr[v0], c0_ = csr[v0], a1 = gr[v1], b1 = dgr[v1], c1_ = csr[v1];
            gi += a0; dg += b0; cs += c0_; gi += a1; dg += b1; cs += c1_;
        }
        for (; c < nC; c++) { const int vo = src[nH + c]; gi += gr[vo]; dg += dgr[vo]; cs += csr[vo]; }
    }
    const int loc = A.loc_base + B.av_loc[k];
    B.g[loc] = gi; B.diag[loc] = dg; B.vc[loc] = gi / clampd(dg, O.min_diag, O.max_diag);
    if (write_S) { B.rhs[loc] = gi + cs; B.S[A.S_base + (size_t)A.n_red * A.n_red + B.av_red[k]] = gi + cs; }
}
```

### rtk_visual_inertial_navigation_amd/csrc/swf_plan.cpp

```cpp
#include <algorithm>
#include <array>
#include <cstdlib>
#include <cstring>
#include <map>
#include <string>
#include <vector>
#include "swf_plan.h"

namespace {
int refuse(std::string& err, int code, const std::string& msg) { err = msg; return code; }
int ls_ncw(int var) { return var <= 1 ? 8 : 12; }
int ls_tpw(int var) { return var == 0 ? 2 : var == 1 ? 5 : 6; }

int plan_window(Plan& B, const swf_flat_window* w, int wi, HostWin& hw, std::string& err) {
    WinRec R{};
    const int nP = w->n_pose, nS = w->n_sb, nL = w->n_lm, nC = w->n_sc;
    const int nb = nP + nS + nL + nC;
    if (nb <= 0) return refuse(err, SWF_E_INVALID, "empty window");
    hw = HostWin{ w->pose, w->sb, w->lm, w->sc, nP, nS, nL, nC, 0 };
    R.x_base = (int)B.n_x; R.blk_base = (int)B.blk_xoff.size(); R.n_blk = nb;
    R.loc_base = (int)B.n_loc;
    std::vector<int> gs(nb), ls(nb), xo(nb), loc(nb, -1), grp(nb, -1);
    int xoff = 0;
    for (int b = 0; b < nb; b++) {
// ... 583 lines not shown
        auto tile_rows = [&](unsigned long long fm) {
            unsigned t = 0;
            for (int f = 0; f < W.nF && f < 64; f++) if ((fm >> f) & 1ULL) { t |= 1u << ((6 * f) / 16); t |= 1u << ((6 * f + 5) / 16); }
            return t;
        };
        std::vector<int> ord; std::vector<unsigned> trs((size_t)(W.lm1 - W.lm0), 0u);
        for (int l = W.lm0; l < W.lm1; l++) {
            if (B.lm_loc[l] < 0) continue;
            int k = B.lm_obs0[l + 1] - B.lm_obs0[l];
            if (k > 64) return refuse(err, SWF_E_UNSUPPORTED, "landmark with more than 64 observations");
            trs[(size_t)(l - W.lm0)] = tile_rows(B.lm_fmask[l]);
            ord.push_back(l);
        }
        auto key = [&](int l) { unsigned t = trs[(size_t)(l - W.lm0)]; int lo = t ? __builtin_ctz(t) : 0, hi = t ? 31 - __builtin_clz(t) : 0; return hi * 64 + lo; };
        std::stable_sort(ord.begin(), ord.end(), [&](int x, int y) { return key(x) < key(y); });
        const int first_task = (int)(rec.size() / 32);
        task_tiles.clear();
        size_t at = 0; int lw = 4;
        auto new_task = [&]() { at = rec.size(); rec.resize(at + 32, 0); for (int g = 0; g < 4; g++) rec[at + g * 8] = -1; task_tiles.emplace_back((size_t)ntl, 0u); lw = 0; };
        for (int l : ord) {
            int o0 = B.lm_obs0[l], k = B.lm_obs0[l + 1] - o0;
            if (lw >= 4) new_task();
            int* r = &rec[at + (size_t)lw * 8];
            r[0] = l; r[1] = B.lm_loc[l]; r[2] = o0; r[3] = o0 + k; r[4] = 3 * lw; r[5] = 0; r[6] = 0; r[7] = 0;
            unsigned t = trs[(size_t)(l - W.lm0)];
            const unsigned ks = lw == 0 ? 1u : lw == 1 ? 3u : lw == 2 ? 6u : 4u;
            std::vector<unsigned>& tt = task_tiles.back();
            for (int tr = 0; tr < nt; tr++) {
                if (!((t >> tr) & 1u)) continue;
                tt[(size_t)tr] |= ks;
                for (int tc = 0; tc < tr; tc++) if ((t >> tc) & 1u) tt[(size_t)(nt + tr * (tr - 1) / 2 + tc)] |= ks;
            }
            lw++;
        }
        if (task_tiles.size() & 1) new_task();
        const int ntask = (int)task_tiles.size();
        for (int c = 0; c < ntask / TW; c++) {
            size_t kw = km.size(); km.resize(kw + (size_t)B.ls_kms, 0);
            for (int g = 0; g < TW; g++) {
                const std::vector<unsigned>& tt = task_tiles[(size_t)(c * TW + g)];
                for (int e = 0; e < ntl; e++) if (tt[(size_t)e]) {
                    B.lm_schur_mfma += __builtin_popcount(tt[(size_t)e]);
                    int lp = e / (NCW * TPW), r = e % (NCW * TPW), sl = r / NCW, cw = r % NCW;
                    km[kw + (size_t)(lp * NCW + cw)] |= (tt[(size_t)e] << (3 * g)) << (3 * TW * sl);
                }
            }
        }
        const int np = ntask / 2;
        for (int sp = 0; sp < GEMM_SPLIT; sp++) c0.push_back(first_task + 2 * (int)((long long)sp * np / GEMM_SPLIT));
    }
    c0.push_back((int)(rec.size() / 32));
    rec.resize(rec.size() + (size_t)32 * 4 * LS_NB, 0);
    km.resize(km.size() + (size_t)B.ls_kms * 2, 0);
    return SWF_OK;
}

void plan_frame_sums(Plan& B) {
    B.fr_obs0.push_back((int)B.fr_obs.size());
    B.fsb_obs0.push_back(B.n_proj); B.fsb_perm.resize((size_t)B.n_proj + 1, 0);
    std::vector<int>& rec = B.fsb_rec;
    rec.assign((size_t)8 * std::max(B.n_fsb, 1), 0);
    for (int k = 0; k < B.n_fsb; k++) {
        int* r = rec.data() + (size_t)8 * k;
        r[0] = B.fsb_win[(size_t)k]; r[1] = B.fsb_obs0[(size_t)k]; r[2] = B.fsb_obs0[(size_t)k + 1] - B.fsb_obs0[(size_t)k];
        r[3] = B.fsb_foff0[(size_t)k]; r[4] = B.fsb_out0[(size_t)k]; r[5] = B.win[(size_t)r[0]].nF;
    }
}

int plan_jt_records(Plan& B, std::string& err) {
    bool fits = true;
    auto jt_recs = [&](const std::vector<int>& list) {
        std::vector<JtRec> out(list.size());
        for (size_t q = 0; q < list.size(); q++) {
            const GFac& G = B.gf[(size_t)list[q]];
            JtRec& r = out[q];
            r = JtRec{};
            r.win = G.win; r.nres = G.nres; r.jld = G.jld; r.nslot = G.nslot; r.roff = G.roff; r.f = list[q];
            if (G.nslot > JT_MAXSLOT) { fits = false; continue; }
            for (int t = 0; t < JT_MAXSLOT; t++) {
                const bool has = t < G.nslot;
                r.joff[t] = has ? B.s_joff[(size_t)G.slot0 + t] : -1; r.loc[t] = has ? B.s_loc[(size_t)G.slot0 + t] : 0; r.ls[t] = has ? B.s_ls[(size_t)G.slot0 + t] : 0;
            }
        }
        return out;
    };
    B.sc_jt = jt_recs(B.sc_gf); B.imu_jt = jt_recs(B.imu_gf);
    if (!fits) return refuse(err, SWF_E_UNSUPPORTED, "scalar / IMU factor with more than JT_MAXSLOT parameter blocks");
    return SWF_OK;
}

void plan_prior_maps(Plan& B) {
    std::vector<double>& Jt = B.prior_Jt;
    Jt.assign(B.prior_J.size(), 0.0);
    for (size_t k = 0; k < B.prior_dim.size(); k++) {
        const size_t n = (size_t)B.prior_dim[k]; const double* J = B.prior_J.data() + B.prior_Joff[k]; double* T = Jt.data() + B.prior_Joff[k];
        for (size_t r = 0; r < n; r++) for (size_t c = 0; c < n; c++) T[c * n + r] = J[r * n + c];
    }
    std::vector<int>&cl = B.prior_colloc, &cc = B.prior_colcc, &pcol = B.s_pcol, &pxo = B.s_pxo;
    cl.assign(B.prior_r0.size(), -1); cc.assign(B.prior_r0.size(), -1); pcol.assign(B.s_ls.size(), 0); pxo.assign(B.s_ls.size(), 0);
    for (const GFac& G : B.gf) {
        if (G.type != GF_PRIOR) continue;
        int col = 0, xo = 0;
        for (int t = 0; t < G.nslot; t++) {
            int l = B.s_ls[G.slot0 + t], lo = B.s_loc[G.slot0 + t], mc = B.s_ccol[G.slot0 + t];
            pcol[G.slot0 + t] = col; pxo[G.slot0 + t] = xo;
            for (int q = 0; q < l; q++) {
                cl[(size_t)B.prior_roff[G.data] + col + q] = lo >= 0 ? lo + q : -1;
                cc[(size_t)B.prior_roff[G.data] + col + q] = mc >= 0 ? mc + q : -1;
            }
            col += l; xo += (l == 6 ? 7 : l);
        }
    }
    std::vector<int>& cvl = B.cv_loc;
    cvl.assign((size_t)std::max(B.v_tot, 1), 0);
    for (const Clique& c : B.cl)
        for (int m = c.mem0; m < c.mem1; m++)
            for (int q = 0; q < B.cm_ls[(size_t)m]; q++) cvl[(size_t)c.v_off + (size_t)B.cm_col[(size_t)m] + (size_t)q] = B.cm_loc[(size_t)m] + q;
}

void plan_pair_clique_classes(Plan& B, std::vector<int>& pd, std::vector<int>& po) {
    std::vector<int> clc[5], cle;
    for (size_t i = 0; i < B.pair.size(); i++) {
        Pair& Pq = B.pair[i]; const WinRec& Rw = B.win[Pq.win];
        Pq.fsb0 = Rw.fsb0; Pq.fsb1 = Rw.fsb1; Pq.n = Rw.n_red; Pq.m = 6 * Rw.nF; Pq.S_base = Rw.S_base; Pq.P_base = Rw.P_base; Pq.q_base = (long long)6 * Rw.fr_base * GEMM_SPLIT;
        if (B.s_direct && !Pq.is_diag && Pq.fa >= 0 && Pq.fb >= 0 && Pq.c0 == Pq.c1) continue;
        (Pq.is_diag ? pd : po).push_back((int)i);
    }
    std::stable_sort(po.begin(), po.end(), [&](int a, int c) {
        return (B.pair[a].la * B.pair[a].lb + 15) / 16 > (B.pair[c].la * B.pair[c].lb + 15) / 16; });
    for (size_t i = 0; i < B.cl.size(); i++) {
        const Clique& c = B.cl[i];
        if (c.d_e > 0) cle.push_back((int)i);
        if (c.is_static) continue;
        int d = c.d_e + c.d_f;
        int cls = (c.d_e <= 1 && d <= 32 && c.n_rows <= 48) ? 0 : (c.n_rows <= 32 && d <= 48) ? 1 : (c.n_rows <= CLQ_MAXR && d <= CLQ_MAXD) ? 2 : (c.n_rows <= CLQ_TALLR && d <= 64) ? 4 : 3;
        if (B.lat_fuse && cls < 2) cls = 2;
        clc[cls].push_back((int)i);
        for (int q = c.fac0; q < c.fac1; q++) if (B.gf[B.cl_fac[q]].type == GF_IMU) B.clc_imu[cls] = true;
    }
    B.n_pd = (int)pd.size(); B.n_po = (int)po.size(); B.n_cle = (int)cle.size();
    std::vector<Pair>&vd = B.pair_d, &vo = B.pair_o;
    for (int i : pd) vd.push_back(B.pair[i]);
    for (int i : po) vo.push_back(B.pair[i]);
    for (int i : cle) B.cle_rec.push_back(B.cl[i]);
    for (int k = 0; k < 5; k++) {
        for (int i : clc[k]) B.clc_rec[k].push_back(B.cl[i]);
        B.n_clc[k] = (int)clc[k].size();
    }
}

int plan_asm_programs(Plan& B, const std::vector<int>& pd, const std::vector<int>& po, std::string& err) {
    const int n_part = B.s_direct ? 0 : B.ls_folded ? 1 : GEMM_SPLIT, n_qpart = B.ls_folded ? 1 : GEMM_SPLIT;
    const int n = B.n_win;
    struct Prog { std::vector<int> dst, src0, aux, src, vloc, vred, vsrc0, vi, vsrc; std::vector<unsigned> cnt, vcnt; };
    std::vector<AsmWin>& asw = B.asw;
    asw.assign((size_t)n, AsmWin{});
    std::vector<int>&t_dst = B.as_dst, &t_src0 = B.as_src0, &t_aux = B.as_aux, &t_src = B.as_src, &tv_loc = B.av_loc, &tv_red = B.av_red, &tv_src0 = B.av_src0, &tv_i = B.av_i, &tv_src = B.av_src;
    std::vector<unsigned>&t_cnt = B.as_cnt, &tv_cnt = B.av_cnt;
    std::map<std::vector<int>, std::array<int, 4>> seen;
    std::vector<std::vector<int>> wpairs((size_t)n);
    for (int i : pd) wpairs[(size_t)B.pair[i].win].push_back(i);
    for (int i : po) wpairs[(size_t)B.pair[i].win].push_back(i);
    bool overflow = false;
    std::vector<unsigned>& tnz = B.s_tnz;
    tnz.assign((size_t)n * 4, 0u);
    for (const Pair& Pq : B.pair) {
        if (B.win[(size_t)Pq.win].n_red > 256) continue;
        for (int I = Pq.ra / 16; I <= (Pq.ra + Pq.la - 1) / 16; I++)
            for (int J = Pq.rb / 16; J <= (Pq.rb + Pq.lb - 1) / 16 && J < I; J++) { const int t = I * (I - 1) / 2 + J; tnz[(size_t)Pq.win * 4 + (t >> 5)] |= 1u << (t & 31); }
    }
    for (int w = 0; w < n; w++) {
        const WinRec& Rw = B.win[w];
        AsmWin& A = asw[(size_t)w];
        A.win = w; A.n_red = Rw.n_red; A.m = 6 * Rw.nF; A.loc_base = Rw.loc_base; A.S_base = Rw.S_base;
        A.P_base = Rw.P_base * GEMM_SPLIT; A.q_base = (long long)6 * Rw.fr_base * GEMM_SPLIT;
        A.fs_base = Rw.fsb1 > Rw.fsb0 ? B.fsb_out0[(size_t)Rw.fsb0] : 0;
        long long Cb = -1; int vb = -1;
        for (int c = Rw.cl0; c < Rw.cl1; c++) { if (Cb < 0 || B.cl[c].C_off < Cb) Cb = B.cl[c].C_off; if (vb < 0 || B.cl[c].v_off < vb) vb = B.cl[c].v_off; }
        A.C_base = Cb < 0 ? 0 : Cb; A.v_base = vb < 0 ? 0 : vb;
        Prog Pg;
        const int nfsb = Rw.fsb1 - Rw.fsb0, mm = A.m;
        for (int pi_ : wpairs[(size_t)w]) {
            const Pair& Pq = B.pair[(size_t)pi_];
            const bool frame_pair = Pq.fa >= 0 && Pq.fb >= 0, obs = Pq.is_diag && Pq.fa >= 0;
            const int ncon = Pq.c1 - Pq.c0;
            for (int i = 0; i < Pq.la; i++) for (int j = 0; j < Pq.lb; j++) {
                if (Pq.is_diag && j > i) continue;
                const bool dg = Pq.is_diag && i == j;
                const int nP = frame_pair ? n_part : 0, nH = obs ? nfsb : 0;
                if (ncon > 4095 || nH > 4095) overflow = true;
                Pg.dst.push_back((Pq.ra + i) * Pq.n + Pq.rb + j);
                Pg.cnt.push_back((unsigned)ncon | ((unsigned)nP << 12) | ((unsigned)nH << 17) | ((dg ? 1u : 0u) << 29) | ((frame_pair && B.s_direct ? 1u : 0u) << 30));
                Pg.src0.push_back((int)Pg.src.size());
                Pg.aux.push_back(dg ? (Pq.loc_a - Rw.loc_base) + i : 0);
                for (int c = Pq.c0; c < Pq.c1; c++) Pg.src.push_back((int)(B.pc_coff[(size_t)c] + (long long)i * B.pc_cld[(size_t)c] + j - A.C_base));
                if (nP) {
                    const int pr = 6 * Pq.fa + i, pc = 6 * Pq.fb + j;
                    const long long pel = pr >= pc ? (long long)pr * mm + pc : (long long)pc * mm + pr;
                    for (int q = 0; q < nP; q++) Pg.src.push_back((int)((long long)q * mm * mm + pel));
                }
                if (nH) {
                    const int hi = i > j ? i : j, lo = i > j ? j : i;
                    for (int k2 = Rw.fsb0; k2 < Rw.fsb1; k2++) Pg.src.push_back((B.fsb_out0[(size_t)k2] - A.fs_base + Pq.fa) * FS_VAL + hi * (hi + 1) / 2 + lo);
                }
                if (dg) for (int c = Pq.c0; c < Pq.c1; c++) Pg.src.push_back(B.pc_voff[(size_t)c] + i - A.v_base);
            }
            if (!Pq.is_diag) continue;
            for (int i = 0; i < Pq.la; i++) {
                const int nH = obs ? nfsb : 0, nQ = obs ? n_qpart : 0;
                Pg.vloc.push_back(Pq.loc_a - Rw.loc_base + i); Pg.vred.push_back(Pq.ra + i); Pg.vi.push_back(obs ? i : 0);
                Pg.vcnt.push_back((unsigned)ncon | ((unsigned)nQ << 12) | ((unsigned)nH << 17));
                Pg.vsrc0.push_back((int)Pg.vsrc.size());
                if (nH) for (int k2 = Rw.fsb0; k2 < Rw.fsb1; k2++) Pg.vsrc.push_back((B.fsb_out0[(size_t)k2] - A.fs_base + Pq.fa) * FS_VAL);
                for (int c = Pq.c0; c < Pq.c1; c++) Pg.vsrc.push_back(B.pc_voff[(size_t)c] + i - A.v_base);
                for (int q = 0; q < nQ; q++) Pg.vsrc.push_back(q * mm + 6 * Pq.fa + i);
            }
        }
        std::vector<int> key;
        key.reserve(Pg.dst.size() * 4 + Pg.src.size() + Pg.vloc.size() * 5 + Pg.vsrc.size() + 8);
        key.push_back((int)Pg.dst.size()); key.push_back((int)Pg.vloc.size());
        key.insert(key.end(), Pg.dst.begin(), Pg.dst.end()); for (unsigned c : Pg.cnt) key.push_back((int)c);
        key.insert(key.end(), Pg.src0.begin(), Pg.src0.end()); key.insert(key.end(), Pg.aux.begin(), Pg.aux.end()); key.insert(key.end(), Pg.src.begin(), Pg.src.end());
        key.insert(key.end(), Pg.vloc.begin(), Pg.vloc.end()); key.insert(key.end(), Pg.vred.begin(), Pg.vred.end()); for (unsigned c : Pg.vcnt) key.push_back((int)c);
        key.insert(key.end(), Pg.vsrc0.begin(), Pg.vsrc0.end()); key.insert(key.end(), Pg.vi.begin(), Pg.vi.end()); key.insert(key.end(), Pg.vsrc.begin(), Pg.vsrc.end());
        auto it = seen.find(key);
        if (it == seen.end()) {
            const int se0 = (int)t_dst.size(), ve0 = (int)tv_loc.size(), so = (int)t_src.size(), vo = (int)tv_src.size();
            t_dst.insert(t_dst.end(), Pg.dst.begin(), Pg.dst.end()); t_cnt.insert(t_cnt.end(), Pg.cnt.begin(), Pg.cnt.end()); t_aux.insert(t_aux.end(), Pg.aux.begin(), Pg.aux.end());
            for (int x : Pg.src0) t_src0.push_back(x + so);
            t_src.insert(t_src.end(), Pg.src.begin(), Pg.src.end());
            tv_loc.insert(tv_loc.end(), Pg.vloc.begin(), Pg.vloc.end()); tv_red.insert(tv_red.end(), Pg.vred.begin(), Pg.vred.end()); tv_cnt.insert(tv_cnt.end(), Pg.vcnt.begin(), Pg.vcnt.end());
            tv_i.insert(tv_i.end(), Pg.vi.begin(), Pg.vi.end());
            for (int x : Pg.vsrc0) tv_src0.push_back(x + vo);
            tv_src.insert(tv_src.end(), Pg.vsrc.begin(), Pg.vsrc.end());
            it = seen.emplace(std::move(key), std::array<int, 4>{ se0, (int)Pg.dst.size(), ve0, (int)Pg.vloc.size() }).first;
        }
        A.se0 = it->second[0]; A.ne = it->second[1]; A.ve0 = it->second[2]; A.nv = it->second[3];
        B.as_max_ne = std::max(B.as_max_ne, A.ne); B.as_max_nv = std::max(B.as_max_nv, A.nv);
    }
    if (overflow) return refuse(err, SWF_E_UNSUPPORTED, "assembly program: more than 4095 contributions to one entry of the reduced system");
    B.asm_programs = (int)seen.size();
    auto nonempty_i = [](std::vector<int>& v) { if (v.empty()) v.push_back(0); };
    auto nonempty_u = [](std::vector<unsigned>& v) { if (v.empty()) v.push_back(0u); };
    nonempty_i(t_dst); nonempty_u(t_cnt); nonempty_i(t_src0); nonempty_i(t_aux); nonempty_i(t_src);
    nonempty_i(tv_loc); nonempty_i(tv_red); nonempty_u(tv_cnt); nonempty_i(tv_src0); nonempty_i(tv_i); nonempty_i(tv_src);
    return SWF_OK;
}

int plan_composite(Plan& B, std::string& err) {
    B.n_comp = (int)B.co_M.size();
    if (B.n_comp) {
        const int nc = B.n_comp;
        std::vector<int>&eo = B.co_eo, &no = B.co_no, &roff = B.co_roff, &x0off = B.co_x0off, &voff = B.co_voff;
        std::vector<long long>&pno = B.co_pno, &nno = B.co_nno, &go = B.co_go, &g2o = B.co_g2o, &Joff = B.co_Joff, &Coff = B.co_Coff;
        eo.assign(nc + 1, 0); no.assign(nc + 1, 0); roff.assign(nc, 0); x0off.assign(nc, 0); voff.assign(nc, 0);
        pno.assign(nc + 1, 0); nno.assign(nc + 1, 0); go.assign(nc + 1, 0); g2o.assign(nc + 1, 0); Joff.assign(nc, 0); Coff.assign(nc, 0);
        for (int f = 0; f < nc; f++) {
            const int M = B.co_M[f], N = B.co_N[f], G = 30 + N;
            B.comp_nmax = std::max(B.comp_nmax, N); B.comp_nmin = std::min(B.comp_nmin, N);
            eo[f + 1] = eo[f] + M; no[f + 1] = no[f] + N; pno[f + 1] = pno[f] + 15LL * M * N; nno[f + 1] = nno[f] + (long long)N * N;
            go[f + 1] = go[f] + G; g2o[f + 1] = g2o[f] + (long long)G * G;
            const GFac& Gf = B.gf[B.co_gf[f]];
            const Clique& Cq = B.cl[Gf.clique];
            if (Cq.is_static ? (Cq.d_f != G || Cq.d_e != 0) : (Cq.d_e <= 0)) return refuse(err, SWF_E_UNSUPPORTED, "composite factor: its blocks must all be variable");
            Joff[f] = B.prior_Joff[Gf.data]; roff[f] = B.prior_roff[Gf.data]; x0off[f] = B.prior_x0off[Gf.data];
            Coff[f] = Cq.is_static ? Cq.C_off : -1; voff[f] = Cq.is_static ? Cq.v_off : -1;
        }
        B.comp_ne = eo[nc];
        std::vector<int>&qf = B.co_iq_f, &qk = B.co_iq_k;
        for (int f = 0; f < nc; f++) for (int k = 0; k <= B.co_M[f]; k++) { qf.push_back(f); qk.push_back(k); }
    }
    return SWF_OK;
}
}

PlanShape plan_shape_from_env(int n_cu) {
    auto num = [](const char* name) { const char* v = getenv(name); return v ? atoi(v) : 0; };
    PlanShape sh;
    sh.n_cu = n_cu;
    sh.no_lat_fuse = getenv("SWF_NO_LAT_FUSE") != nullptr; sh.no_chol_col = getenv("SWF_NO_CHOL_COL") != nullptr;
    sh.ls_variant = num("SWF_LS_VARIANT"); sh.ls_qpb = num("SWF_LS_QPB"); sh.ls_grad_qpb = num("SWF_LS_GRAD_QPB");
    return sh;
}

int plan_build(const swf_flat_window* const* windows, int n, const PlanShape& sh, Plan& B, std::string& err) {
    int rc;
    B.hw.resize((size_t)n);
    for (int i = 0; i < n; i++) if ((rc = plan_window(B, windows[i], i, B.hw[(size_t)i], err)) != SWF_OK) return rc;
    if (B.n_x > 0x7fffffffLL || B.n_loc > 0x7fffffffLL) return refuse(err, SWF_E_UNSUPPORTED, "batch too large for 32-bit offsets");
    B.n_win = n; B.n_cu = sh.n_cu;
    B.n_proj = (int)B.p_win.size(); B.n_lm = (int)B.lm_win.size(); B.n_fsb = (int)B.fsb_win.size();
    B.lat_fuse = n * 8 <= B.n_cu && !sh.no_lat_fuse;
    B.want_aux = (n * 16 <= B.n_cu && !B.lat_fuse) || (2 * n >= B.n_cu && n <= B.n_cu);
    plan_counters(B);
    if ((rc = plan_lm_blocks(B, err)) != SWF_OK) return rc;
    plan_prior_chunks(B);
    if (B.loc2x.empty()) B.loc2x.push_back(-1);
    B.lm_obs0.push_back(B.n_proj);
    plan_schur_shape(B, sh);
    if ((rc = plan_schur_tasks(B, err)) != SWF_OK) return rc;
    plan_frame_sums(B);
    if ((rc = plan_jt_records(B, err)) != SWF_OK) return rc;
    plan_prior_maps(B);
    std::vector<int> pd, po;
    plan_pair_clique_classes(B, pd, po);
    if ((rc = plan_asm_programs(B, pd, po, err)) != SWF_OK) return rc;
    B.C_init.resize((size_t)B.C_tot, 0.0); B.dgraw_init.resize((size_t)B.v_tot, 0.0);
    if ((rc = plan_composite(B, err)) != SWF_OK) return rc;
    B.want_Linv = B.max_red > B.rr_nmax && B.max_red <= CB_NMAX;
    B.want_Wk = B.max_red > B.rr_nmax && B.max_red <= CC_NMAX && n * 4 <= B.n_cu && !sh.no_chol_col;
    return SWF_OK;
}

int plan_validate(const Plan& B, std::string& err) {
#define NEED(cond, table, i) do { if (!(cond)) { err = std::string("plan_validate: ") + (table) + " [" + std::to_string((long long)(i)) + "]: " #cond; return SWF_E_INVALID; } } while (0)
    auto in = [](long long v, long long lo, long long hi) { return v >= lo && v < hi; };
    const int n = B.n_win;
    const long long n_gf = (long long)B.gf.size(), n_cl = (long long)B.cl.size(), n_slot = (long long)B.s_x.size();
    NEED((int)B.win.size() == n && (int)B.asw.size() == n && (int)B.s_tnz.size() == 4 * n, "win", n);
    NEED((int)B.lm_obs0.size() == B.n_lm + 1 && (int)B.lm_fmask.size() == B.n_lm && (int)B.fr_obs0.size() == B.n_fr + 1, "lm_obs0", B.n_lm);
    NEED((int)B.sch_c0.size() == n * GEMM_SPLIT + 1, "sch_c0", B.sch_c0.size());
    for (int q = 0; q < B.n_proj; q++) {
        NEED(in(B.p_win[q], 0, n), "p_win", q);
        const WinRec& W = B.win[B.p_win[q]];
        NEED(in(q, W.proj0, W.proj1) && in(B.p_xpose[q], 0, B.n_x) && in(B.p_xex[q], 0, B.n_x) && in(B.p_xlm[q], 0, B.n_x), "p_x*", q);
        NEED(in(B.p_lpose[q], -1, B.n_loc) && in(B.p_llm[q], -1, B.n_loc) && in(B.p_fr[q], -1, W.nF) && in(B.p_lm[q], W.lm0, W.lm1), "p_l*", q);
        NEED(in(q, B.lm_obs0[B.p_lm[q]], B.lm_obs0[B.p_lm[q] + 1]), "lm_obs0", B.p_lm[q]);
    }
    for (int l = 0; l < B.n_lm; l++) NEED(B.lm_obs0[l] <= B.lm_obs0[l + 1] && in(B.lm_obs0[l], 0, B.n_proj + 1) && in(B.lm_loc[l], -1, B.n_loc) && in(B.lm_win[l], 0, n), "lm_obs0", l);
    for (int f = 0; f < B.n_fr; f++) for (int o = B.fr_obs0[f]; o < B.fr_obs0[f + 1]; o++) NEED(in(o, 0, (long long)B.fr_obs.size()) && in(B.fr_obs[o], 0, B.n_proj), "fr_obs", o);
    for (int k = 0; k < B.n_fsb; k++) {
        const int* r = &B.fsb_rec[(size_t)8 * k];
        NEED(in(r[0], 0, n), "fsb_rec", k);
        const WinRec& W = B.win[r[0]];
        NEED(in(k, W.fsb0, W.fsb1) && r[1] >= W.proj0 && r[2] >= 1 && r[2] <= FS_BLK && r[1] + r[2] <= W.proj1 && r[5] == W.nF, "fsb_rec", k);
        NEED(r[3] >= 0 && r[3] + W.nF + 1 <= (long long)B.fsb_foff.size() && r[4] >= 0 && r[4] + W.nF <= B.fs_tot, "fsb_rec", k);
        std::vector<char> hit((size_t)r[2], 0);
        for (int t = 0; t < r[2]; t++) { const int p = B.fsb_perm[(size_t)r[1] + t]; NEED(in(p, 0, r[2]) && !hit[p], "fsb_perm", r[1] + t); hit[p] = 1; }
        for (int f = 0; f <= W.nF; f++) NEED(in(B.fsb_foff[(size_t)r[3] + f], 0, r[2] + 1), "fsb_foff", r[3] + f);
    }
    for (long long f = 0; f < n_gf; f++) {
        const GFac& G = B.gf[f];
        NEED(in(G.win, 0, n) && G.nslot >= 0 && G.slot0 >= 0 && G.slot0 + G.nslot <= n_slot && G.roff >= 0 && G.roff + G.nres <= B.r_tot && in(G.clique, -1, n_cl), "gf", f);
        for (int t = G.slot0; t < G.slot0 + G.nslot; t++) {
            NEED(in(B.s_x[t], 0, B.n_x) && in(B.s_loc[t], -1, B.n_loc) && B.s_loc[t] + B.s_ls[t] <= B.n_loc, "s_loc", t);
            NEED(B.s_joff[t] == -1 || (B.s_joff[t] >= 0 && B.s_joff[t] + (long long)(B.s_ls[t] - 1) * G.jld + G.nres <= B.j_tot), "s_joff", t);
        }
    }
    for (int pass = 0; pass < 2; pass++) {
        const std::vector<JtRec>& jt = pass ? B.imu_jt : B.sc_jt; const std::vector<int>& list = pass ? B.imu_gf : B.sc_gf;
        NEED(jt.size() == list.size(), pass ? "imu_jt" : "sc_jt", jt.size());
        for (size_t q = 0; q < jt.size(); q++) {
            const JtRec& r = jt[q];
            NEED(in(r.f, 0, n_gf) && r.f == list[q] && in(r.win, 0, n) && r.roff >= 0 && r.roff + r.nres <= B.r_tot && in(r.nslot, 0, JT_MAXSLOT + 1), pass ? "imu_jt" : "sc_jt", q);
            for (int t = 0; t < JT_MAXSLOT; t++)
                NEED(r.loc[t] >= -1 && r.loc[t] + r.ls[t] <= B.n_loc && (r.joff[t] == -1 || (r.loc[t] >= 0 && r.joff[t] >= 0 && r.joff[t] + (long long)(r.ls[t] - 1) * r.jld + r.nres <= B.j_tot)) && (t < r.nslot || r.joff[t] == -1), pass ? "imu_jt" : "sc_jt", q);
        }
    }
    {
        int ch = 0;
        std::vector<int> w_first(n, -1), w_end(n, 0);
        for (size_t q = 0; q < B.prior_gf.size(); q++) {
            NEED(in(B.prior_gf[q], 0, n_gf), "prior_gf", q);
            const GFac& G = B.gf[B.prior_gf[q]];
            NEED(G.type == GF_PRIOR && in(G.data, 0, (long long)B.prior_dim.size()) && B.prior_dim[G.data] == G.nres, "prior_gf", q);
            const long long dim = G.nres;
            NEED(B.prior_Joff[G.data] >= 0 && B.prior_Joff[G.data] + dim * dim <= (long long)B.prior_J.size() && B.prior_Jt.size() == B.prior_J.size(), "prior_Joff", G.data);
            NEED(B.prior_roff[G.data] >= 0 && B.prior_roff[G.data] + dim <= (long long)B.prior_r0.size() && B.prior_x0off[G.data] >= 0, "prior_roff", G.data);
            const int nch = B.prior_nch[q];
            NEED(nch >= 1 && (dim > PRIOR_SPLIT_DIM ? (long long)nch * PRIOR_CHUNK >= dim && (long long)(nch - 1) * PRIOR_CHUNK < dim : nch == 1), "prior_nch", q);
            for (int c = 0; c < nch; c++, ch++) NEED(ch < B.n_pch && B.pch_q[ch] == (int)q && B.pch_r0[ch] == (nch > 1 ? c * PRIOR_CHUNK : 0), "pch_q", ch);
            if (w_first[G.win] < 0) w_first[G.win] = ch - nch;
            w_end[G.win] = ch;
        }
        NEED(ch == B.n_pch, "pch_q", ch);
        for (int w = 0; w < n; w++) NEED(w_first[w] < 0 ? B.win[w].pch0 == B.win[w].pch1 : (B.win[w].pch0 == w_first[w] && B.win[w].pch1 == w_end[w]), "win.pch", w);
    }
    NEED((long long)B.loc2x.size() >= std::max<long long>(B.n_loc, 1) && (long long)B.x_var.size() == B.n_x && B.blk_xoff.size() == B.blk_loc.size() && B.blk_xoff.size() == B.blk_gs.size(), "loc2x", B.loc2x.size());
    for (int w = 0; w < n; w++) {
        const WinRec& W = B.win[w];
        NEED(W.blk_base >= 0 && W.n_blk >= 0 && W.blk_base + W.n_blk <= (long long)B.blk_xoff.size() && W.x_base >= 0 && W.x_base + W.x_n <= B.n_x && W.loc_base >= 0 && W.loc_base + W.n_loc <= B.n_loc, "win.blk", w);
        int xo = W.x_base; long long nvar = 0;
        for (int b = W.blk_base; b < W.blk_base + W.n_blk; b++) {
            const int gs = B.blk_gs[b], ls = gs == 7 ? 6 : gs, lo = B.blk_loc[b];
            NEED((gs == 7 || gs == 9 || gs == 3 || gs == 1) && B.blk_xoff[b] == xo && xo + gs <= W.x_base + W.x_n, "blk_xoff", b);
            NEED(lo == -1 || (lo >= W.loc_base && lo + ls <= W.loc_base + W.n_loc), "blk_loc", b);
            for (int k = 0; k < gs; k++) NEED(B.x_var[(size_t)xo + k] == (lo >= 0 ? 1 : 0), "x_var", xo + k);
            if (lo >= 0) { nvar += ls; for (int k = 0; k < ls; k++) NEED(B.loc2x[(size_t)lo + k] == (gs == 7 ? -1 : xo + k), "loc2x", lo + k); }
            xo += gs;
        }
        NEED(xo == W.x_base + W.x_n && nvar == W.n_loc, "blk_gs: the blocks do not fill the window", w);
        std::vector<char> hit((size_t)(W.lm1 - W.lm0), 0);
        for (int l = W.lm0; l < W.lm1; l++) { const int c = B.lm_col[l]; NEED(c >= 0 && c % 3 == 0 && c / 3 < W.lm1 - W.lm0 && !hit[c / 3], "lm_col", l); hit[c / 3] = 1; }
    }
    NEED(B.prior_colloc.size() == B.prior_r0.size() && B.prior_colcc.size() == B.prior_r0.size() && (long long)B.s_pcol.size() == n_slot && (long long)B.s_pxo.size() == n_slot && (long long)B.s_ccol.size() == n_slot, "prior_colloc", B.prior_colloc.size());
    for (long long f = 0; f < n_gf; f++) {
        const GFac& G = B.gf[f];
        const long long d = G.clique >= 0 ? B.cl[G.clique].d_e + B.cl[G.clique].d_f : 0;
        for (int t = G.slot0; t < G.slot0 + G.nslot; t++) NEED(B.s_ccol[t] == -1 || (B.s_ccol[t] >= 0 && B.s_ccol[t] + B.s_ls[t] <= d), "s_ccol", t);
        if (G.type != GF_PRIOR) continue;
        NEED(in(G.data, 0, (long long)B.prior_dim.size()), "gf.data", f);
        const long long roff = B.prior_roff[G.data], x0o = B.prior_x0off[G.data];
        const long long gsum = ((size_t)G.data + 1 < B.prior_x0off.size() ? B.prior_x0off[G.data + 1] : (long long)B.prior_x0.size()) - x0o;
        int col = 0, xo = 0;
        for (int t = G.slot0; t < G.slot0 + G.nslot; t++) {
            const int l = B.s_ls[t];
            NEED(B.s_pcol[t] == col && col + l <= G.nres && B.s_pxo[t] == xo && xo + (l == 6 ? 7 : l) <= gsum, "s_pcol", t);
            for (int q = 0; q < l; q++) {
                NEED(B.prior_colloc[(size_t)roff + col + q] == (B.s_loc[t] >= 0 ? B.s_loc[t] + q : -1), "prior_colloc", roff + col + q);
                NEED(B.prior_colcc[(size_t)roff + col + q] == (B.s_ccol[t] >= 0 ? B.s_ccol[t] + q : -1), "prior_colcc", roff + col + q);
            }
            col += l; xo += l == 6 ? 7 : l;
        }
        NEED(col == G.nres && xo == gsum, "s_pcol: the slots do not fill the prior", f);
    }
    {
        size_t k = 0;
        for (const Clique& C : B.cl) if (C.d_e > 0) { NEED(k < B.cle_rec.size() && !memcmp(&B.cle_rec[k], &C, sizeof(Clique)), "cle_rec", k); k++; }
        NEED((int)k == B.n_cle && k == B.cle_rec.size(), "cle_rec", k);
    }
    if (const int nc = B.n_comp) {
        NEED((int)B.co_M.size() == nc && (int)B.co_N.size() == nc && (int)B.co_gf.size() == nc && (int)B.co_win.size() == nc && (int)B.co_mid.size() == nc && (int)B.co_xo_off.size() == nc + 1, "co_M", nc);
        NEED((int)B.co_eo.size() == nc + 1 && (int)B.co_no.size() == nc + 1 && (int)B.co_pno.size() == nc + 1 && (int)B.co_nno.size() == nc + 1 && (int)B.co_go.size() == nc + 1 && (int)B.co_g2o.size() == nc + 1, "co_eo", nc);
        NEED((int)B.co_Joff.size() == nc && (int)B.co_roff.size() == nc && (int)B.co_x0off.size() == nc && (int)B.co_Coff.size() == nc && (int)B.co_voff.size() == nc, "co_Joff", nc);
        NEED(B.co_eo[0] == 0 && B.co_no[0] == 0 && B.co_pno[0] == 0 && B.co_nno[0] == 0 && B.co_go[0] == 0 && B.co_g2o[0] == 0 && B.co_xo_off[0] == 0, "co_eo", 0);
        size_t iq = 0;
        for (int f = 0; f < nc; f++) {
            const long long M = B.co_M[f], N = B.co_N[f], G = 30 + N;
            NEED(M >= 1 && N >= 0 && N <= CO_MAXN && in(B.co_win[f], 0, n) && in(B.co_mid[f], 0, M) && in(B.co_gf[f], 0, n_gf) && B.gf[B.co_gf[f]].type == GF_PRIOR && B.gf[B.co_gf[f]].nres == G, "co_M", f);
            NEED(B.co_eo[f + 1] == B.co_eo[f] + M && B.co_no[f + 1] == B.co_no[f] + N && B.co_pno[f + 1] == B.co_pno[f] + 15 * M * N && B.co_nno[f + 1] == B.co_nno[f] + N * N, "co_eo", f + 1);
            NEED(B.co_go[f + 1] == B.co_go[f] + G && B.co_g2o[f + 1] == B.co_g2o[f] + G * G && B.co_xo_off[f + 1] == B.co_xo_off[f] + 4 + N && B.co_xo_off[f + 1] <= (long long)B.co_xo.size(), "co_go", f + 1);
            for (int q = B.co_xo_off[f]; q < B.co_xo_off[f + 1]; q++) NEED(in(B.co_xo[q], B.win[B.co_win[f]].x_base, (long long)B.win[B.co_win[f]].x_base + B.win[B.co_win[f]].x_n), "co_xo", q);
            NEED(B.co_Joff[f] >= 0 && B.co_Joff[f] + G * G <= (long long)B.prior_J.size() && B.co_roff[f] >= 0 && B.co_roff[f] + G <= (long long)B.prior_r0.size() && B.co_x0off[f] >= 0 && B.co_x0off[f] + 32 + N <= (long long)B.prior_x0.size(), "co_Joff", f);
            NEED((B.co_Coff[f] == -1 && B.co_voff[f] == -1) || (B.co_Coff[f] >= 0 && B.co_Coff[f] + G * G <= B.C_tot && B.co_voff[f] >= 0 && B.co_voff[f] + G <= B.v_tot), "co_Coff", f);
            for (int k = 0; k <= M; k++, iq++) NEED(iq < B.co_iq_f.size() && iq < B.co_iq_k.size() && B.co_iq_f[iq] == f && B.co_iq_k[iq] == k, "co_iq_f", iq);
        }
        const size_t ne = (size_t)B.co_eo[nc];
        NEED(iq == B.co_iq_f.size() && (long long)ne == B.comp_ne && B.co_pose.size() == ne * 7 && B.co_sb.size() == ne * 9 && B.co_pose_lin.size() == ne * 7 && B.co_sb_lin.size() == ne * 9, "co_pose", ne);
        NEED(B.co_Hpp.size() == ne * 225 && B.co_rhs_p.size() == ne * 15 && (long long)B.co_HpN.size() == B.co_pno[nc] && (long long)B.co_HNN.size() == B.co_nno[nc] && (long long)B.co_rhsN.size() == B.co_no[nc], "co_Hpp", ne);
        NEED(B.co_pre.size() == (ne + nc) * SWF_PRE_DOUBLES && B.co_H12.size() == (size_t)nc * 225 && B.co_pbgw.size() == (size_t)nc * 6 && (int)B.co_xo.size() == B.co_xo_off[nc], "co_pre", ne);
    }
    std::map<std::array<long long, 3>, int> cl_seen;
    for (long long c = 0; c < n_cl; c++) {
        const Clique& C = B.cl[c]; const long long d = C.d_e + C.d_f;
        NEED(in(C.win, 0, n) && in(c, B.win[C.win].cl0, B.win[C.win].cl1) && C.fac0 >= 0 && C.fac0 <= C.fac1 && C.fac1 <= (long long)B.cl_fac.size() && C.mem0 >= 0 && C.mem0 <= C.mem1 && C.mem1 <= (long long)B.cm_loc.size(), "cl", c);
        NEED(in(C.e_loc, -1, B.n_loc) && C.C_off >= 0 && C.C_off + (long long)C.d_f * C.d_f <= B.C_tot && C.v_off >= 0 && C.v_off + C.d_f <= B.v_tot && C.e_off >= 0 && C.e_off + C.d_e * d + C.d_e <= B.e_tot, "cl", c);
        NEED(C.r_off >= 0 && C.r_off + C.n_rows <= B.r_tot && (C.is_static || (C.j_off >= 0 && C.j_off + C.n_rows * d <= B.j_tot)), "cl", c);
        for (int q = C.fac0; q < C.fac1; q++) NEED(in(B.cl_fac[q], 0, n_gf) && in(B.cl_frow[q], 0, C.n_rows + 1), "cl_fac", q);
        for (int m = C.mem0; m < C.mem1; m++) {
            NEED(B.cm_loc[m] >= 0 && B.cm_loc[m] + B.cm_ls[m] <= B.n_loc && B.cm_col[m] >= 0 && B.cm_col[m] + B.cm_ls[m] <= C.d_f, "cm_loc", m);
            for (int q = 0; q < B.cm_ls[m]; q++) NEED(B.cv_loc[(size_t)C.v_off + B.cm_col[m] + q] == B.cm_loc[m] + q, "cv_loc", C.v_off + B.cm_col[m] + q);
        }
        if (!C.is_static) cl_seen[{ C.fac0, C.mem0, C.e_off }] = 0;
    }
    for (int k = 0; k < 5; k++) {
        NEED((int)B.clc_rec[k].size() == B.n_clc[k], "clc_rec", k);
        for (const Clique& C : B.clc_rec[k]) {
            const long long d = C.d_e + C.d_f; const int R = C.n_rows;
            auto it = cl_seen.find({ C.fac0, C.mem0, C.e_off });
            NEED(it != cl_seen.end() && it->second++ == 0, "clc_rec", k);
            NEED(k == 0 ? (C.d_e <= 1 && d <= 32 && R <= 48) : k == 1 ? (R <= 32 && d <= 48) : k == 2 ? (R <= CLQ_MAXR && d <= CLQ_MAXD) : k == 4 ? (R <= CLQ_TALLR && d <= 64)
                        : (d <= CB_MAXD && C.d_e <= 9 && (long long)C.d_e * d <= CB_MAXED), "clc_rec", k);
        }
    }
    for (auto& kv : cl_seen) NEED(kv.second == 1, "clc_rec: a clique in no class, fac0", kv.first[0]);
    const int TW = B.ls_var <= 1 ? 2 : 1, NCW = ls_ncw(B.ls_var), TPW = ls_tpw(B.ls_var);
    NEED((long long)B.sch_rec.size() >= ((long long)B.sch_c0.back() + 4 * LS_NB) * 32 && (long long)B.sch_km.size() >= ((long long)B.sch_c0.back() / TW + 2) * B.ls_kms, "sch_rec", B.sch_rec.size());
    std::vector<std::vector<const Pair*>> wpair((size_t)n);
    auto pair_ok = [&](const Pair& P) {
        if (!in(P.win, 0, n)) return false;
        const WinRec& W = B.win[P.win];
        return P.ra >= 0 && P.la >= 1 && P.ra + P.la <= W.n_red && P.rb >= 0 && P.lb >= 1 && P.rb + P.lb <= W.n_red && P.rb <= P.ra && in(P.fa, -1, W.nF) && in(P.fb, -1, W.nF)
            && P.c0 >= 0 && P.c0 <= P.c1 && P.c1 <= (long long)B.pc_coff.size() && (P.is_diag ? (P.ra == P.rb && P.la == P.lb) : P.ra != P.rb) && P.loc_a == W.loc_base + W.n_e + P.ra
            && P.fsb0 == W.fsb0 && P.fsb1 == W.fsb1 && P.n == W.n_red && P.m == 6 * W.nF && P.S_base == W.S_base && P.P_base == W.P_base && P.q_base == 6LL * W.fr_base * GEMM_SPLIT;
    };
    NEED((int)B.pair_d.size() == B.n_pd && (int)B.pair_o.size() == B.n_po, "pair_d", B.pair_d.size());
    for (const Pair& P : B.pair) NEED(pair_ok(P), "pair", &P - B.pair.data());
    for (const Pair& P : B.pair_d) { NEED(pair_ok(P) && P.is_diag, "pair_d", &P - B.pair_d.data()); wpair[P.win].push_back(&P); }
    for (const Pair& P : B.pair_o) { NEED(pair_ok(P) && !P.is_diag, "pair_o", &P - B.pair_o.data()); wpair[P.win].push_back(&P); }
    std::map<std::array<int, 4>, std::vector<int>> programs;
    for (int w = 0; w < n; w++) {
        const WinRec& W = B.win[w];
        NEED(W.n_e + W.n_red == W.n_loc && W.loc_base >= 0 && W.loc_base + W.n_loc <= B.n_loc && W.x_base >= 0 && W.x_base + W.x_n <= B.n_x, "win", w);
        NEED(W.S_base >= 0 && W.S_base + (long long)(W.n_red + 1) * W.n_red <= B.S_tot && W.Lt_base + (long long)(W.n_red + 1) * (W.n_red + 1) <= B.Lt_tot && W.P_base + 36LL * W.nF * W.nF <= B.P_tot, "win", w);
        NEED(W.fr_base >= 0 && W.fr_base + W.nF <= B.n_fr && W.nF <= LS_MAXF && W.lm0 <= W.lm1 && W.lm1 <= B.n_lm, "win", w);
        for (int f = 0; f < W.nF; f++) NEED(B.fr_red[W.fr_base + f] >= 0 && B.fr_red[W.fr_base + f] + 6 <= W.n_red, "fr_red", W.fr_base + f);
        {
            int l = W.lm0;
            for (int k = W.lmb0; k < W.lmb1; k++) {
                const int* r = &B.lmb_rec[(size_t)4 * k];
                NEED(k < B.n_lmb && r[2] == l && r[3] >= 1 && r[3] <= 256 && l + r[3] <= W.lm1 && r[0] == B.lm_obs0[l] && r[1] == B.lm_obs0[l + r[3]] - r[0] && r[1] <= 256, "lmb_rec", k);
                l += r[3];
            }
            NEED(l == W.lm1, "lmb_rec", W.lmb1);
        }
        {
            const int* c0 = &B.sch_c0[(size_t)w * GEMM_SPLIT];
            const int t0 = c0[0], t1 = c0[GEMM_SPLIT], m = 6 * W.nF, nt = (m + 15) / 16;
            for (int sp = 0; sp < GEMM_SPLIT; sp++) NEED(c0[sp] >= 0 && c0[sp] <= c0[sp + 1] && (c0[sp] & 1) == 0, "sch_c0", w * GEMM_SPLIT + sp);
            NEED(((t1 - t0) & 1) == 0 && (w > 0 || t0 == 0), "sch_c0", w * GEMM_SPLIT);
            std::vector<int> times((size_t)(W.lm1 - W.lm0), 0);
            for (int t = t0; t < t1; t++) for (int g = 0; g < 4; g++) {
                const int* r = &B.sch_rec[((size_t)t * 4 + g) * 8]; const int L = r[0];
                if (L == -1) continue;
                NEED(in(L, W.lm0, W.lm1) && B.lm_loc[L] >= 0 && r[1] == B.lm_loc[L] && r[2] == B.lm_obs0[L] && r[3] == B.lm_obs0[L + 1] && r[3] - r[2] <= 64 && r[4] == 3 * g, "sch_rec", ((size_t)t * 4 + g) * 8);
                times[L - W.lm0]++;
                unsigned rows = 0;
                for (int f = 0; f < W.nF && f < 64; f++) if ((B.lm_fmask[L] >> f) & 1ULL) { rows |= 1u << ((6 * f) / 16); rows |= 1u << ((6 * f + 5) / 16); }
                const unsigned ks = g == 0 ? 1u : g == 1 ? 3u : g == 2 ? 6u : 4u;
                for (int tr = 0; tr < nt; tr++) for (int tc = 0; tc <= tr; tc++) {
                    if (!((rows >> tr) & 1u) || !((rows >> tc) & 1u)) continue;
                    const int e = tr == tc ? tr : nt + tr * (tr - 1) / 2 + tc, lp = e / (NCW * TPW), rr = e % (NCW * TPW), sl = rr / NCW, cw = rr % NCW;
                    const size_t word = (size_t)(t / TW) * B.ls_kms + (size_t)(lp * NCW + cw);
                    NEED(lp * NCW + cw < B.ls_kms && (((unsigned)B.sch_km[word] >> (3 * TW * sl + 3 * (t % TW))) & ks) == ks, "sch_km", word);
                }
            }
            for (int l = W.lm0; l < W.lm1; l++) NEED(times[l - W.lm0] == (B.lm_loc[l] >= 0 ? 1 : 0), "sch_rec: landmark", l);
        }
        for (int p = W.pair0; p < W.pair1; p++) {
            const Pair& P = B.pair[p];
            NEED(P.win == w, "pair", p);
            for (int c = P.c0; c < P.c1; c++) NEED(B.pc_coff[c] >= 0 && B.pc_coff[c] + (long long)(P.la - 1) * B.pc_cld[c] + P.lb <= B.C_tot && B.pc_voff[c] >= 0 && B.pc_voff[c] + P.la <= B.v_tot, "pc_coff", c);
            if (W.n_red > 256) continue;
            for (int I = P.ra / 16; I <= (P.ra + P.la - 1) / 16; I++) for (int J = P.rb / 16; J <= (P.rb + P.lb - 1) / 16 && J < I; J++) {
                const int t = I * (I - 1) / 2 + J;
                NEED((B.s_tnz[(size_t)w * 4 + (t >> 5)] >> (t & 31)) & 1u, "s_tnz", w * 4 + (t >> 5));
            }
        }
        const AsmWin& A = B.asw[w];
        const long long nS = (long long)B.as_dst.size(), nV = (long long)B.av_loc.size(), mm = A.m;
        NEED(A.win == w && A.n_red == W.n_red && A.m == 6 * W.nF && A.se0 >= 0 && A.se0 + A.ne <= nS && A.ve0 >= 0 && A.ve0 + A.nv <= nV && A.ne <= B.as_max_ne && A.nv <= B.as_max_nv, "asw", w);
        NEED(A.S_base == W.S_base && A.C_base >= 0 && A.v_base >= 0 && A.fs_base >= 0 && A.P_base == W.P_base * GEMM_SPLIT && A.q_base == 6LL * W.fr_base * GEMM_SPLIT && A.loc_base == W.loc_base, "asw", w);
        const long long fs_n = (B.fs_tot - A.fs_base) * FS_VAL, P_n = B.P_tot * GEMM_SPLIT - A.P_base, q_n = (long long)std::max(1, 6 * B.n_fr) * GEMM_SPLIT - A.q_base;
        std::vector<char> written((size_t)W.n_red * W.n_red, 0);
        for (int k = A.se0; k < A.se0 + A.ne; k++) {
            const unsigned cnt = B.as_cnt[k]; const int nC = AS_NC(cnt), nP = AS_NP(cnt), nH = AS_NH(cnt), s0 = B.as_src0[k], dst = B.as_dst[k];
            NEED(in(dst, 0, (long long)W.n_red * W.n_red) && dst % W.n_red <= dst / W.n_red && !written[dst], "as_dst", k);
            written[dst] = 1;
            NEED(s0 >= 0 && s0 + nC + nP + nH + (AS_DIAG(cnt) ? nC : 0) <= (long long)B.as_src.size() && in(B.as_aux[k], 0, W.n_loc) && (!AS_SOLD(cnt) || B.s_direct), "as_src0", k);
            const int* s = &B.as_src[s0];
            for (int c = 0; c < nC; c++) NEED(in(A.C_base + s[c], 0, B.C_tot), "as_src", s0 + c);
            for (int c = nC; c < nC + nP; c++) NEED(in(s[c], 0, P_n) && s[c] < GEMM_SPLIT * mm * mm, "as_src", s0 + c);
            for (int c = nC + nP; c < nC + nP + nH; c++) NEED(in(s[c], 0, fs_n), "as_src", s0 + c);
            if (AS_DIAG(cnt)) for (int c = nC + nP + nH; c < 2 * nC + nP + nH; c++) NEED(in(A.v_base + s[c], 0, B.v_tot), "as_src", s0 + c);
        }
        for (int k = A.ve0; k < A.ve0 + A.nv; k++) {
            const unsigned cnt = B.av_cnt[k]; const int nC = AS_NC(cnt), nQ = AS_NP(cnt), nH = AS_NH(cnt), s0 = B.av_src0[k];
            NEED(in(B.av_loc[k], 0, W.n_loc) && in(B.av_red[k], 0, W.n_red) && in(B.av_i[k], 0, 6) && s0 >= 0 && s0 + nH + nC + nQ <= (long long)B.av_src.size(), "av_src0", k);
            const int* s = &B.av_src[s0];
            for (int c = 0; c < nH; c++) NEED(s[c] >= 0 && s[c] + FS_VAL <= fs_n, "av_src", s0 + c);
            for (int c = nH; c < nH + nC; c++) NEED(in(A.v_base + s[c], 0, B.v_tot), "av_src", s0 + c);
            for (int c = nH + nC; c < nH + nC + nQ; c++) NEED(in(s[c], 0, q_n), "av_src", s0 + c);
        }
        for (const Pair* P : wpair[w]) for (int i = 0; i < P->la; i++) for (int j = 0; j < (P->is_diag ? i + 1 : P->lb); j++)
            NEED(P->ra + i < W.n_red && P->rb + j < W.n_red && written[(size_t)(P->ra + i) * W.n_red + P->rb + j], "as_dst: an entry of pair_d / pair_o is missing, window", w);
        std::vector<int>& key = programs[{ A.se0, A.ne, A.ve0, A.nv }];
        if (key.empty()) {
            key.push_back(A.ne);
            for (int k = A.se0; k < A.se0 + A.ne; k++) {
                const unsigned cnt = B.as_cnt[k]; const int len = AS_NC(cnt) * (AS_DIAG(cnt) ? 2 : 1) + AS_NP(cnt) + AS_NH(cnt);
                key.push_back(B.as_dst[k]); key.push_back((int)cnt); key.push_back(B.as_aux[k]);
                key.insert(key.end(), &B.as_src[B.as_src0[k]], &B.as_src[B.as_src0[k]] + len);
            }
            for (int k = A.ve0; k < A.ve0 + A.nv; k++) {
                const unsigned cnt = B.av_cnt[k]; const int len = AS_NC(cnt) + AS_NP(cnt) + AS_NH(cnt);
                key.push_back(B.av_loc[k]); key.push_back(B.av_red[k]); key.push_back((int)cnt); key.push_back(B.av_i[k]);
                key.insert(key.end(), &B.av_src[B.av_src0[k]], &B.av_src[B.av_src0[k]] + len);
            }
        }
    }
    NEED((int)programs.size() == B.asm_programs, "asw: programs", programs.size());
    for (auto a = programs.begin(); a != programs.end(); ++a) for (auto b = std::next(a); b != programs.end(); ++b)
        NEED(a->second != b->second, "asw: two copies of one program, se0", b->first[0]);
    return SWF_OK;
#undef NEED
}
```

### rtk_visual_inertial_navigation_amd/csrc/swf_plan.h

```cpp
#pragma once
#include <string>
#include <vector>
#include "../../include/swf_solver.h"
#include "swf_records.h"

struct FeatWinSrc {
    int x_base = 0, n_pose = 0, n_sb = 0, n_lm = 0, n_sc = 0;
    std::vector<int> proj_idx; std::vector<double> proj_uv;
    std::vector<int> idp_kind, idp_idx; std::vector<double> idp_pts;
    double pbg[3] = { 0, 0, 0 }; double sqrt_info = 0;
};

struct HostWin {
    double *pose, *sb, *lm, *sc;
    int n_pose, n_sb, n_lm, n_sc;
    int tail_dim;
    double *comp_pose = nullptr, *comp_sb = nullptr;
    int comp_e0 = 0, comp_ne = 0;
    std::vector<int> p_orig;
    int n_proj_all = 0;
    std::vector<int> tail_x;
    FeatWinSrc feat;
    struct LinPrior { int gf, dim, gsum; std::vector<int> col_x; };
    std::vector<LinPrior> lin_prior;
};

struct PlanShape {
    int n_cu = 256;
    bool no_lat_fuse = false;
    int ls_variant = 0;
    int ls_qpb = 0;
    int ls_grad_qpb = 0;
    bool no_chol_col = false;
};
PlanShape plan_shape_from_env(int n_cu);

struct Plan {
    std::vector<WinRec> win;
    std::vector<HostWin> hw;
    std::vector<int> blk_xoff, blk_loc, blk_gs, loc2x;
    std::vector<unsigned char> x_var;
    std::vector<int> p_win, p_xpose, p_xex, p_xlm, p_lpose, p_llm, p_fr, p_lm;
    std::vector<double> p_uv;
    std::vector<int> lm_win, lm_obs0, lm_loc, lm_col;
    std::vector<unsigned long long> lm_fmask;
    std::vector<int> fsb_win, fsb_obs0, fsb_perm, fsb_foff, fsb_foff0, fsb_out0;
    long long fs_tot = 0;
    std::vector<int> fr_obs0, fr_obs, fr_red;
    std::vector<GFac> gf;
    std::vector<int> s_x, s_loc, s_ls, s_joff, s_ccol;
    std::vector<double> imu_pre, cp_dat, pr_dat, dop_dat, sp_w, gx_dat;
    std::vector<int> imu_gf, sc_gf, prior_gf, idp_gf;
    std::vector<int> prior_dim, prior_roff, prior_x0off;
    std::vector<long long> prior_Joff;
    std::vector<double> prior_J, prior_r0, prior_x0;
    std::vector<Clique> cl;
    std::vector<int> cl_fac, cl_frow, cm_loc, cm_ls, cm_col;
    std::vector<double> C_init, dgraw_init;
    std::vector<int> co_M, co_N, co_gf, co_win, co_xo, co_xo_off{ 0 };
    std::vector<double> co_pose, co_sb, co_pose_lin, co_sb_lin, co_Hpp, co_HpN, co_rhs_p, co_HNN, co_rhsN, co_pre, co_pbgw, co_H12;
    std::vector<int> co_mid;
    std::vector<Pair> pair;
    std::vector<long long> pc_coff;
    std::vector<int> pc_cld, pc_voff;
    long long n_x = 0, n_loc = 0, S_tot = 0, Lt_tot = 0, P_tot = 0, C_tot = 0;
    int v_tot = 0, e_tot = 0, r_tot = 0, j_tot = 0, n_fr = 0;
    int max_tiles = 0, max_prior_dim = 0;
    std::vector<int> lmb_rec, pch_q, pch_r0, prior_nch;
    std::vector<int> sch_c0, sch_rec, sch_km;
    std::vector<int> fsb_rec;
    std::vector<JtRec> sc_jt, imu_jt;
    std::vector<double> prior_Jt;
    std::vector<int> prior_colloc, prior_colcc, s_pcol, s_pxo, cv_loc;
    std::vector<Pair> pair_d, pair_o;
    std::vector<Clique> clc_rec[5], cle_rec;
    std::vector<AsmWin> asw;
    std::vector<unsigned> s_tnz;
    std::vector<int> as_dst, as_src0, as_aux, as_src, av_loc, av_red, av_src0, av_i, av_src;
    std::vector<unsigned> as_cnt, av_cnt;
    std::vector<int> co_eo, co_no, co_roff, co_x0off, co_voff, co_iq_f, co_iq_k;
    std::vector<long long> co_pno, co_nno, co_go, co_g2o, co_Joff, co_Coff;
    int n_win = 0, n_proj = 0, n_lm = 0, n_lmb = 0, n_pch = 0, n_fsb = 0, n_pd = 0, n_po = 0, n_cle = 0, n_clc[5] = { 0, 0, 0, 0, 0 };
    int as_max_ne = 0, as_max_nv = 0;
    int n_cu = 256, rr_nmax = 256, max_red = 0, min_red = 1 << 30;
    int ls_qpb = 1, ls_var = 0, ls_kms = 8, ls_gqpb = 4; bool ls_folded = false, s_direct = false;
    bool lat_fuse = false, want_aux = false, want_Linv = false, want_Wk = false;
    bool clc_imu[5] = { false, false, false, false, false };
    int n_pch_split = 0; bool rr4_has15 = false, rr4_has16 = false;
    int n_comp = 0, comp_nmax = 0, comp_nmin = 1 << 30; long long comp_ne = 0;
    int asm_programs = 0;
    int64_t jac_bytes = 0, proj_bytes = 0, chol_flops = 0, lm_schur_flops = 0, lm_schur_flops_sym = 0, lm_schur_mfma = 0;
};

int plan_build(const swf_flat_window* const* windows, int n, const PlanShape& shape, Plan& plan, std::string& err);

int plan_validate(const Plan& plan, std::string& err);
```

### rtk_visual_inertial_navigation_amd/csrc/swf_records.h

```cpp
#pragma once
#include <stdint.h>
#include "../../include/swf_types.h"

struct WinRec {
    int x_base, x_n;
    int blk_base, n_blk;
    int loc_base, n_loc, n_e, n_red;
    long long S_base;
    long long Lt_base;
    int proj0, proj1;
    int lm0, lm1;
    int fr_base, nF;
    long long P_base;
    int gf0, gf1;
    int cl0, cl1;
    int pair0, pair1;
    int fsb0, fsb1;
    int tail_dim;
    int n_pose_blk;
    int lmb0, lmb1;
    int pch0, pch1;
    double proj_sqrt_info, proj_loss_a;
    double pbg[3], gw[3], base[3];
};

struct WinState {
    double radius, mu, x_cost, x_norm, alpha, dogleg_step_norm, step_norm, gmax;
    double jg_sq, initial_cost;
    double lm_dec;
    double model_cost_change;
    int status, iter, need_lin, reuse, eval_cand, lin_fail, invalid_run, nsucc, nunsucc;
    int chol_fail;
};

enum { GF_IMU = 1, GF_CP = 2, GF_PR = 3, GF_DOP = 4, GF_SP = 5, GF_PRIOR = 6, GF_SPR = 7, GF_SCP = 8, GF_FIX = 9, GF_IDP = 10,
       GF_PROJX = 11 };
struct GFac {
    int type, win, nres, nslot;
    int slot0;
    int roff;
    int data;
    int clique;
    int jld;
    int pad;
};

#define JT_MAXSLOT 5
struct alignas(16) JtRec {
    int win, nres, jld, nslot;
    int roff, f, pad0, pad1;
    int joff[JT_MAXSLOT];
    int loc[JT_MAXSLOT];
    int ls[JT_MAXSLOT];
    int pad2;
};
static_assert(sizeof(JtRec) == 96, "JtRec: six 16-byte loads");

struct Clique {
    int win;
    int e_loc, d_e;
    int d_f;
    int fac0, fac1;
    int mem0, mem1;
    long long C_off;
    int v_off;
    int e_off;
    int is_static;
    int n_rows;
    int j_off, r_off;
    int pad0, pad1;
};

struct Pair {
    int win;
    int ra, rb, la, lb;
    int fa, fb;
    int c0, c1;
    int is_diag;
    int loc_a;
    int fsb0, fsb1;
    int n, m;
    long long S_base, P_base;
    long long q_base;
};

struct AsmWin {
    int se0, ne;
    int ve0, nv;
    int n_red, m;
    int loc_base;
    int fs_base;
    int v_base;
    int win;
    long long C_base, S_base, P_base, q_base;
};
#define AS_NC(c) ((c) & 4095u)
#define AS_NP(c) (((c) >> 12) & 31u)
#define AS_NH(c) (((c) >> 17) & 4095u)
#define AS_DIAG(c) (((c) >> 29) & 1u)
#define AS_SOLD(c) (((c) >> 30) & 1u)

struct DevBatch {
    int n_win;
    int n_x, n_loc_total;
    int max_iter_trace;
    double* x; double* xc; double* x0;
    double* g; double* diag; double* rhs; double* y; double* step;
    double* vc;
    double* S; double* L;
    double* Wk;
    double* Linv;
    const WinRec* win; WinState* ws; swf_iteration* trace;
    const int* blk_xoff; const int* blk_loc; const int* blk_gs;
    const int* loc2x;
    const unsigned char* x_var;
    int n_proj;
    const int* p_win; const int* p_xpose; const int* p_xex; const int* p_xlm;
    const int* p_lpose; const int* p_llm; const int* p_fr; const int* p_lm;
    const double* p_uv;
    double* p_r; double* p_Jp; double* p_Jl;
    double* p_cpart; double* p_apart;
    int n_fsb; const int* fsb_rec; const int* fsb_perm; const int* fsb_foff;
    double* fs_part;
    double* jsc;
    int n_lm;
    const int* lm_win; const int* lm_obs0; const int* lm_loc; const int* lm_col;
    double* lm_Einv; double* lm_g;
    double* P;
    double* lmq;
    const int* lmb_rec; int n_lmb;
    const int* sch_c0; const int* sch_rec;
    const int* sch_km;
    const unsigned long long* lm_fmask;
    int n_fr;
    const int* fr_obs0; const int* fr_obs;
    const int* fr_red;
    int n_gf;
    const GFac* gf;
    const int* s_x; const int* s_loc; const int* s_ls; const int* s_joff; const int* s_ccol;
    double* g_r; double* g_J; double* g_cost; double* g_aux;
    const double* imu_pre; const double* cp_dat; const double* pr_dat; const double* dop_dat; const double* sp_w;
    const double* gx_dat;
    int n_imu; const int* imu_gf;
    int n_idp; const int* idp_gf;
    int n_sc;  const int* sc_gf;
    const JtRec* sc_jt; const JtRec* imu_jt;
    int n_prior; const int* prior_gf;
    int n_pch; const int* pch_q; const int* pch_r0; const int* prior_nch;
    double* pr_cpart; double* pr_apart;
    const int* prior_dim; const long long* prior_Joff; const int* prior_roff; const int* prior_x0off;
    const double* prior_J; const double* prior_r0; const double* prior_x0;
    const double* prior_Jt;
    const int* prior_colloc;
    const int* prior_colcc;
    const int* s_pcol; const int* s_pxo;
    int n_cl;
    const Clique* cl;
    const int* cl_fac; const int* cl_frow;
    const int* cm_loc; const int* cm_ls; const int* cm_col;
    double* C; double* cv_graw; double* cv_dgraw; double* cv_cs; double* cE;
    const int* cv_loc;
    int n_clc[5]; const Clique* clc_rec[5];
    int n_cle; const Clique* cle_rec;
    int n_pair;
    const long long* pc_coff; const int* pc_cld; const int* pc_voff;
    int n_pd, n_po; const Pair* pair_d; const Pair* pair_o;
    const AsmWin* asw; int as_max_ne, as_max_nv;
    const int* as_dst; const unsigned* as_cnt; const int* as_src0; const int* as_aux; const int* as_src;
    const int* av_loc; const int* av_red; const unsigned* av_cnt; const int* av_src0; const int* av_i; const int* av_src;
    const unsigned* s_tnz;
    int spec;
    int rr_nmax;
};

#define GEMM_SPLIT 16
#define LS_GRAD_QPB 4
#define LS_NB 4
#define LS_MAXF 64
constexpr bool ls_can_fold(int NCW, int TPW) { return TPW <= 5 && NCW == 8; }
#define PRIOR_SPLIT_DIM 96
#define PRIOR_CHUNK 32
#define CLQ_MAXD 64
#define CLQ_MAXR 64
#define CLQ_TALLR 96
#define CB_MAXD 768
#define CB_MAXED 1536
#define FS_BLK 256
#define FS_VAL 27
#define CB_NMAX 640
#define CC_NMAX 512
#define CTL_NT 256
#define CO_MAXN 64
```

Baseline: 689,300 iterations/s.

## Pack assembly metadata into 16-byte records and add short-entry fast path

Replaces the separate per-entry metadata arrays of the reduced-system assembly kernel with packed 16-byte AsRec records. Entries that sum at most two clique contributions with no partial, Hessian or diagonal terms go to a separate short class, each thread handling several of them with the source offsets stored inline. General entries and vector entries now prefetch source indices in chunks and issue all gathers together before branching on need_lin. This aims to cut scattered metadata loads and raise memory-level parallelism in an irregular gather kernel, at the cost of more plan-builder complexity and some loads that are wasted when a window does not need relinearisation.

```diff
diff --git a/rtk_visual_inertial_navigation_amd/csrc/swf_engine.hip b/rtk_visual_inertial_navigation_amd/csrc/swf_engine.hip
--- a/rtk_visual_inertial_navigation_amd/csrc/swf_engine.hip
+++ b/rtk_visual_inertial_navigation_amd/csrc/swf_engine.hip
@@ -277,7 +277,7 @@
     D.n_gf = (int)B.gf.size(); D.n_imu = (int)B.imu_gf.size(); D.n_sc = (int)B.sc_gf.size(); D.n_prior = (int)B.prior_gf.size(); D.n_idp = (int)B.idp_gf.size();
     D.n_cl = (int)B.cl.size(); D.n_pair = (int)B.pair.size(); D.n_pd = B.n_pd; D.n_po = B.n_po; D.n_cle = B.n_cle;
     for (int k = 0; k < 5; k++) D.n_clc[k] = B.n_clc[k];
-    D.as_max_ne = B.as_max_ne; D.as_max_nv = B.as_max_nv;
+    D.as_max_nsh = B.as_max_nsh; D.as_max_ne = B.as_max_ne; D.as_max_nv = B.as_max_nv;
 #define PUT(field) rc |= P.put(B.field, &D.field)
     PUT(win);
     PUT(lmb_rec); PUT(pch_q); PUT(pch_r0); PUT(prior_nch);
@@ -303,8 +303,8 @@
     PUT(cv_loc);
     PUT(pc_coff); PUT(pc_cld); PUT(pc_voff);
     PUT(asw); PUT(s_tnz);
-    PUT(as_dst); PUT(as_cnt); PUT(as_src0); PUT(as_aux); PUT(as_src);
-    PUT(av_loc); PUT(av_red); PUT(av_cnt); PUT(av_src0); PUT(av_i); PUT(av_src);
+    PUT(as_rec); PUT(as_src);
+    PUT(av_rec); PUT(av_src);
     PUT(pair_d); PUT(pair_o);
     PUT(cle_rec);
     for (int k = 0; k < 5; k++) PUT(clc_rec[k]);
@@ -694,8 +694,12 @@
         if (b->aux) (void)hipStreamWaitEvent(st, b->ev_fork[2], 0);
         if (D.n_pd) {
             Bracket t(*this, SWF_K_ASSEMBLE);
-            const int nbS = write_S ? nb((size_t)D.as_max_ne, 256) : 0, nbV = nb((size_t)D.as_max_nv, 256);
-            hipLaunchKernelGGL(k_assemble_flat, dim3(nbS + nbV, D.n_win), dim3(256), 0, st, D, O, write_S, nbS);
+            const int nbV = nb((size_t)D.as_max_nv, 256);
+            if (write_S) {
+                const int nbSh = nb((size_t)D.as_max_nsh, 256 * AS_EPT), nbG = nb((size_t)D.as_max_ne, 256);
+                hipLaunchKernelGGL(k_assemble_flat<true>, dim3(nbSh + nbG + nbV, D.n_win), dim3(256), 0, st, D, O, nbSh, nbG);
+            }
+            else hipLaunchKernelGGL(k_assemble_flat<false>, dim3(nbV, D.n_win), dim3(256), 0, st, D, O, 0, 0);
         }
     }
     void reduced() {
@@ -1496,7 +1500,7 @@
                                     int32_t flags, int32_t corrupt_table, int32_t corrupt_index, int32_t* info) {
     if (!windows || n <= 0 || n_cu <= 0) return fail(SWF_E_INVALID, "swf_debug_plan_check: bad arguments");
     PlanShape sh;
-    sh.n_cu = n_cu; sh.ls_variant = ls_variant; sh.ls_qpb = ls_qpb; sh.ls_grad_qpb = ls_grad_qpb; sh.no_lat_fuse = flags & 1; sh.no_chol_col = flags & 2;
+    sh.n_cu = n_cu; sh.ls_variant = ls_variant; sh.ls_qpb = ls_qpb; sh.ls_grad_qpb = ls_grad_qpb; sh.no_lat_fuse = flags & 1; sh.no_chol_col = flags & 2; sh.asm_plain = flags & 4;
     Plan B; std::string err;
     int rc = plan_build(windows, n, sh, B, err);
     if (rc != SWF_OK) return fail(rc, err);
@@ -1509,6 +1513,7 @@
         else if (corrupt_table == 5 && i < B.loc2x.size()) B.loc2x[i] ^= 1;
         else if (corrupt_table == 6 && i < B.co_voff.size()) B.co_voff[i] += 1 << 28;
         else if (corrupt_table == 7 && i < B.pair_o.size()) B.pair_o[i].q_base += 8;
+        else if (corrupt_table == 8 && i < (size_t)B.asw[0].nsh) B.as_rec[(size_t)B.asw[0].sh0 + i].z += 1 << 28;
         else return fail(SWF_E_INVALID, "swf_debug_plan_check: nothing to corrupt there");
     }
     if (info) {
diff --git a/rtk_visual_inertial_navigation_amd/csrc/swf_kernels.h b/rtk_visual_inertial_navigation_amd/csrc/swf_kernels.h
--- a/rtk_visual_inertial_navigation_amd/csrc/swf_kernels.h
+++ b/rtk_visual_inertial_navigation_amd/csrc/swf_kernels.h
@@ -1297,76 +1297,134 @@
     EST(5);
 }
 
-__device__ __forceinline__ double as_sum(const double* base, const int* src, int n, int add = 0) {
-    double v = 0;
-    int c = 0;
-    for (; c + 4 <= n; c += 4) {
-        const int i0 = src[c], i1 = src[c + 1], i2 = src[c + 2], i3 = src[c + 3];
-        const double x0 = base[i0 + add], x1 = base[i1 + add], x2 = base[i2 + add], x3 = base[i3 + add];
-        v += x0; v += x1; v += x2; v += x3;
-    }
-    for (; c < n; c++) v += base[src[c] + add];
-    return v;
-}
-__global__ void __launch_bounds__(256) k_assemble_flat(DevBatch B, DevOpt O, int write_S, int nbS) {
+#ifndef AS_EPT
+#define AS_EPT 8
+#endif
+#define AS_CH 16
+#define AV_CH 8
+template <bool WRITE_S>
+__global__ void __launch_bounds__(256) k_assemble_flat(DevBatch B, DevOpt O, int nbSh, int nbG) {
     const AsmWin& A = B.asw[blockIdx.y];
     const WinState& s = B.ws[A.win];
-    if (!s.need_lin) return;
     const int tid = threadIdx.x;
-    if ((int)blockIdx.x < nbS) {
-        if (!write_S) return;
-        const int e = blockIdx.x * 256 + tid;
-        if (e >= A.ne) return;
-        const int k = A.se0 + e;
-        const unsigned cnt = B.as_cnt[k];
-        const int nC = AS_NC(cnt), nP = AS_NP(cnt), nH = AS_NH(cnt);
-        const int* src = B.as_src + B.as_src0[k];
-        const int dst = B.as_dst[k];
+    if (WRITE_S && (int)blockIdx.x < nbSh) {
+        const int e0 = blockIdx.x * (256 * AS_EPT) + tid, last = A.nsh - 1;
+        if ((int)blockIdx.x * (256 * AS_EPT) > last) return;
+        const AsRec* rec = B.as_rec + A.sh0;
+        AsRec R[AS_EPT];
+#pragma unroll
+        for (int j = 0; j < AS_EPT; j++) { const int e = e0 + 256 * j; R[j] = rec[e < last ? e : last]; }
+        const int need = s.need_lin;
         double* S = B.S + A.S_base;
         const double* C = B.C + A.C_base;
+        double xa[AS_EPT], xb[AS_EPT], so[AS_EPT];
+#pragma unroll
+        for (int j = 0; j < AS_EPT; j++) { xa[j] = C[R[j].z]; xb[j] = C[R[j].w]; so[j] = AS_SOLD((unsigned)R[j].y) ? S[R[j].x] : 0.0; }
+        if (!need) return;
+#pragma unroll
+        for (int j = 0; j < AS_EPT; j++) {
+            if (e0 + 256 * j > last) continue;
+            const unsigned cnt = (unsigned)R[j].y;
+            double v = 0;
+            if (AS_NC(cnt) > 0) v += xa[j];
+            if (AS_NC(cnt) > 1) v += xb[j];
+            if (AS_SOLD(cnt)) v = so[j] + v;
+            S[R[j].x] = v;
+        }
+        return;
+    }
+    if (WRITE_S && (int)blockIdx.x < nbSh + nbG) {
+        const int e = ((int)blockIdx.x - nbSh) * 256 + tid;
+        if (e >= A.ne) return;
+        const AsRec R = B.as_rec[A.se0 + e];
+        const int need = s.need_lin, first = s.iter == 0;
+        const double mu = s.mu;
+        const unsigned cnt = (unsigned)R.y;
+        const int nC = AS_NC(cnt), nP = AS_NP(cnt), nH = AS_NH(cnt), dst = R.x;
+        const int e1 = nC, e2 = nC + nP, e3 = e2 + nH, len = e3 + (AS_DIAG(cnt) ? nC : 0), lastp = len > 0 ? len - 1 : 0;
+        const int* src = B.as_src + R.z;
+        double* S = B.S + A.S_base;
+        const double *bC = B.C + A.C_base, *bP = B.P + A.P_base, *bH = B.fs_part + (size_t)A.fs_base * FS_VAL, *bD = B.cv_dgraw + A.v_base;
         const double sold = AS_SOLD(cnt) ? S[dst] : 0.0;
-        double v = as_sum(C, src, nC);
+        int idx[AS_CH];
+#pragma unroll
+        for (int j = 0; j < AS_CH; j++) idx[j] = src[j < lastp ? j : lastp];
+        double aC = 0, aP = 0, aH = 0, aD = 0;
+        for (int c0 = 0; c0 < len; c0 += AS_CH) {
+            double x[AS_CH];
+#pragma unroll
+            for (int j = 0; j < AS_CH; j++) {
+                const int p = c0 + j < lastp ? c0 + j : lastp;
+                const double* base = p < e1 ? bC : p < e2 ? bP : p < e3 ? bH : bD;
+                x[j] = base[idx[j]];
+            }
+            if (c0 + AS_CH < len) {
+#pragma unroll
+                for (int j = 0; j < AS_CH; j++) { const int p = c0 + AS_CH + j; idx[j] = src[p < lastp ? p : lastp]; }
+            }
+#pragma unroll
+            for (int j = 0; j < AS_CH; j++) {
+                const int p = c0 + j;
+                if (p >= len) continue;
+                if (p < e1) aC += x[j];
+                else if (p < e2) aP += x[j];
+                else if (p < e3) aH += x[j];
+                else { if (p == e3) aD = aH; aD += x[j]; }
+            }
+        }
+        if (!need) return;
+        double v = aC;
         if (AS_SOLD(cnt)) v = sold + v;
-        else if (nP) v -= as_sum(B.P + A.P_base, src + nC, nP);
-        double hs = 0;
-        if (nH) { hs = as_sum(B.fs_part + (size_t)A.fs_base * FS_VAL, src + nC + nP, nH); v += hs; }
+        else if (nP) v -= aP;
+        if (nH) v += aH;
         if (AS_DIAG(cnt)) {
-            const double* dgr = B.cv_dgraw + A.v_base;
-            const int* sd = src + nC + nP + nH;
-            double dg = hs;
-            int c = 0;
-            for (; c + 4 <= nC; c += 4) { const double x0 = dgr[sd[c]], x1 = dgr[sd[c + 1]], x2 = dgr[sd[c + 2]], x3 = dgr[sd[c + 3]]; dg += x0; dg += x1; dg += x2; dg += x3; }
-            for (; c < nC; c++) dg += dgr[sd[c]];
-            v += s.mu * damp_diag(O, dg, B.jsc + A.loc_base + B.as_aux[k], s.iter == 0);
+            const double dg = nC ? aD : aH;
+            v += mu * damp_diag(O, dg, B.jsc + A.loc_base + R.w, first);
         }
         S[dst] = v;
         return;
     }
-    const int e = (blockIdx.x - nbS) * 256 + tid;
+    const int e = ((int)blockIdx.x - nbSh - nbG) * 256 + tid;
     if (e >= A.nv) return;
-    const int k = A.ve0 + e;
-    const unsigned cnt = B.av_cnt[k];
-    const int nC = AS_NC(cnt), nQ = AS_NP(cnt), nH = AS_NH(cnt);
-    const int* src = B.av_src + B.av_src0[k];
+    const AsRec R = B.av_rec[A.ve0 + e];
+    const int need = s.need_lin;
+    const unsigned cnt = (unsigned)R.z;
+    const int nC = AS_NC(cnt), nQ = AS_NP(cnt), nH = AS_NH(cnt), i = AV_I(cnt);
+    const int nHQ = nH + nQ, len = nHQ + nC, lastp = len > 0 ? len - 1 : 0;
+    const int* src = B.av_src + R.w;
+    const double *fsg = B.fs_part + (size_t)A.fs_base * FS_VAL + 21 + i, *fsh = B.fs_part + (size_t)A.fs_base * FS_VAL + i * (i + 1) / 2 + i, *lq = B.lmq + A.q_base;
+    const double *gr = B.cv_graw + A.v_base, *dgr = B.cv_dgraw + A.v_base, *csr = B.cv_cs + A.v_base;
+    int idx[AV_CH];
+#pragma unroll
+    for (int j = 0; j < AV_CH; j++) { const int p = j < lastp ? j : lastp; idx[j] = src[p < nH ? p : p < nHQ ? p + nC : p - nQ]; }
     double gi = 0, dg = 0, cs = 0;
-    if (nH) {
-        const double* fs = B.fs_part + (size_t)A.fs_base * FS_VAL;
-        const int i = B.av_i[k];
-        const double g0 = as_sum(fs, src, nH, 21 + i), h0 = as_sum(fs, src, nH, i * (i + 1) / 2 + i);
-        const double q0 = as_sum(B.lmq + A.q_base, src + nH + nC, nQ);
-        gi = g0; dg = h0; cs = -q0;
-    }
-    {
-        const double* gr = B.cv_graw + A.v_base; const double* dgr = B.cv_dgraw + A.v_base; const double* csr = B.cv_cs + A.v_base;
-        int c = 0;
-        for (; c + 2 <= nC; c += 2) {
-            const int v0 = src[nH + c], v1 = src[nH + c + 1];
-            const double a0 = gr[v0], b0 = dgr[v0], c0_ = csr[v0], a1 = gr[v1], b1 = dgr[v1], c1_ = csr[v1];
-            gi += a0; dg += b0; cs += c0_; gi += a1; dg += b1; cs += c1_;
-        }
-        for (; c < nC; c++) { const int vo = src[nH + c]; gi += gr[vo]; dg += dgr[vo]; cs += csr[vo]; }
-    }
-    const int loc = A.loc_base + B.av_loc[k];
+    for (int c0 = 0; c0 < len; c0 += AV_CH) {
+        double x0[AV_CH], x1[AV_CH], x2[AV_CH];
+#pragma unroll
+        for (int j = 0; j < AV_CH; j++) {
+            const int p = c0 + j < lastp ? c0 + j : lastp;
+            const double *p0 = p < nH ? fsg : p < nHQ ? lq : gr, *p1 = p < nH ? fsh : p < nHQ ? lq : dgr, *p2 = p < nH ? fsh : p < nHQ ? lq : csr;
+            x0[j] = p0[idx[j]]; x1[j] = p1[idx[j]]; x2[j] = p2[idx[j]];
+        }
+        if (c0 + AV_CH < len) {
+#pragma unroll
+            for (int j = 0; j < AV_CH; j++) { int p = c0 + AV_CH + j; p = p < lastp ? p : lastp; idx[j] = src[p < nH ? p : p < nHQ ? p + nC : p - nQ]; }
+        }
+#pragma unroll
+        for (int j = 0; j < AV_CH; j++) {
+            const int p = c0 + j;
+            if (p >= len) continue;
+            if (p < nH) { gi += x0[j]; dg += x1[j]; }
+            else if (p < nHQ) cs += x0[j];
+            else {
+                if (p == nHQ) cs = nH ? -cs : 0.0;
+                gi += x0[j]; dg += x1[j]; cs += x2[j];
+            }
+        }
+    }
+    if (nC == 0) cs = nH ? -cs : 0.0;
+    if (!need) return;
+    const int loc = A.loc_base + R.x;
     B.g[loc] = gi; B.diag[loc] = dg; B.vc[loc] = gi / clampd(dg, O.min_diag, O.max_diag);
-    if (write_S) { B.rhs[loc] = gi + cs; B.S[A.S_base + (size_t)A.n_red * A.n_red + B.av_red[k]] = gi + cs; }
-}
+    if (WRITE_S) { B.rhs[loc] = gi + cs; B.S[A.S_base + (size_t)A.n_red * A.n_red + R.y] = gi + cs; }
+}
diff --git a/rtk_visual_inertial_navigation_amd/csrc/swf_plan.cpp b/rtk_visual_inertial_navigation_amd/csrc/swf_plan.cpp
--- a/rtk_visual_inertial_navigation_amd/csrc/swf_plan.cpp
+++ b/rtk_visual_inertial_navigation_amd/csrc/swf_plan.cpp
@@ -759,12 +759,12 @@
 int plan_asm_programs(Plan& B, const std::vector<int>& pd, const std::vector<int>& po, std::string& err) {
     const int n_part = B.s_direct ? 0 : B.ls_folded ? 1 : GEMM_SPLIT, n_qpart = B.ls_folded ? 1 : GEMM_SPLIT;
     const int n = B.n_win;
-    struct Prog { std::vector<int> dst, src0, aux, src, vloc, vred, vsrc0, vi, vsrc; std::vector<unsigned> cnt, vcnt; };
+    struct Prog { std::vector<AsRec> sh, ge, vec; std::vector<int> src, vsrc; };
     std::vector<AsmWin>& asw = B.asw;
     asw.assign((size_t)n, AsmWin{});
-    std::vector<int>&t_dst = B.as_dst, &t_src0 = B.as_src0, &t_aux = B.as_aux, &t_src = B.as_src, &tv_loc = B.av_loc, &tv_red = B.av_red, &tv_src0 = B.av_src0, &tv_i = B.av_i, &tv_src = B.av_src;
-    std::vector<unsigned>&t_cnt = B.as_cnt, &tv_cnt = B.av_cnt;
-    std::map<std::vector<int>, std::array<int, 4>> seen;
+    std::vector<AsRec>&t_rec = B.as_rec, &tv_rec = B.av_rec;
+    std::vector<int>&t_src = B.as_src, &tv_src = B.av_src;
+    std::map<std::vector<int>, std::array<int, 6>> seen;
     std::vector<std::vector<int>> wpairs((size_t)n);
     for (int i : pd) wpairs[(size_t)B.pair[i].win].push_back(i);
     for (int i : po) wpairs[(size_t)B.pair[i].win].push_back(i);
@@ -796,11 +796,15 @@
                 const bool dg = Pq.is_diag && i == j;
                 const int nP = frame_pair ? n_part : 0, nH = obs ? nfsb : 0;
                 if (ncon > 4095 || nH > 4095) overflow = true;
-                Pg.dst.push_back((Pq.ra + i) * Pq.n + Pq.rb + j);
-                Pg.cnt.push_back((unsigned)ncon | ((unsigned)nP << 12) | ((unsigned)nH << 17) | ((dg ? 1u : 0u) << 29) | ((frame_pair && B.s_direct ? 1u : 0u) << 30));
-                Pg.src0.push_back((int)Pg.src.size());
-                Pg.aux.push_back(dg ? (Pq.loc_a - Rw.loc_base) + i : 0);
-                for (int c = Pq.c0; c < Pq.c1; c++) Pg.src.push_back((int)(B.pc_coff[(size_t)c] + (long long)i * B.pc_cld[(size_t)c] + j - A.C_base));
+                const int dst = (Pq.ra + i) * Pq.n + Pq.rb + j;
+                const unsigned cnt = (unsigned)ncon | ((unsigned)nP << 12) | ((unsigned)nH << 17) | ((dg ? 1u : 0u) << 29) | ((frame_pair && B.s_direct ? 1u : 0u) << 30);
+                auto coff = [&](int c) { return (int)(B.pc_coff[(size_t)c] + (long long)i * B.pc_cld[(size_t)c] + j - A.C_base); };
+                if (AS_SHORT(cnt) && !B.asm_plain) {
+                    Pg.sh.push_back(AsRec{ dst, (int)cnt, ncon > 0 ? coff(Pq.c0) : 0, ncon > 1 ? coff(Pq.c0 + 1) : 0 });
+                    continue;
+                }
+                Pg.ge.push_back(AsRec{ dst, (int)cnt, (int)Pg.src.size(), dg ? (Pq.loc_a - Rw.loc_base) + i : 0 });
+                for (int c = Pq.c0; c < Pq.c1; c++) Pg.src.push_back(coff(c));
                 if (nP) {
                     const int pr = 6 * Pq.fa + i, pc = 6 * Pq.fb + j;
                     const long long pel = pr >= pc ? (long long)pr * mm + pc : (long long)pc * mm + pr;
@@ -815,42 +819,37 @@
             if (!Pq.is_diag) continue;
             for (int i = 0; i < Pq.la; i++) {
                 const int nH = obs ? nfsb : 0, nQ = obs ? n_qpart : 0;
-                Pg.vloc.push_back(Pq.loc_a - Rw.loc_base + i); Pg.vred.push_back(Pq.ra + i); Pg.vi.push_back(obs ? i : 0);
-                Pg.vcnt.push_back((unsigned)ncon | ((unsigned)nQ << 12) | ((unsigned)nH << 17));
-                Pg.vsrc0.push_back((int)Pg.vsrc.size());
+                Pg.vec.push_back(AsRec{ Pq.loc_a - Rw.loc_base + i, Pq.ra + i,
+                                        (int)((unsigned)ncon | ((unsigned)nQ << 12) | ((unsigned)nH << 17) | ((unsigned)(obs ? i : 0) << 29)), (int)Pg.vsrc.size() });
                 if (nH) for (int k2 = Rw.fsb0; k2 < Rw.fsb1; k2++) Pg.vsrc.push_back((B.fsb_out0[(size_t)k2] - A.fs_base + Pq.fa) * FS_VAL);
                 for (int c = Pq.c0; c < Pq.c1; c++) Pg.vsrc.push_back(B.pc_voff[(size_t)c] + i - A.v_base);
                 for (int q = 0; q < nQ; q++) Pg.vsrc.push_back(q * mm + 6 * Pq.fa + i);
             }
         }
+        std::stable_sort(Pg.sh.begin(), Pg.sh.end(), [](const AsRec& a, const AsRec& b) { return a.x < b.x; });
         std::vector<int> key;
-        key.reserve(Pg.dst.size() * 4 + Pg.src.size() + Pg.vloc.size() * 5 + Pg.vsrc.size() + 8);
-        key.push_back((int)Pg.dst.size()); key.push_back((int)Pg.vloc.size());
-        key.insert(key.end(), Pg.dst.begin(), Pg.dst.end()); for (unsigned c : Pg.cnt) key.push_back((int)c);
-        key.insert(key.end(), Pg.src0.begin(), Pg.src0.end()); key.insert(key.end(), Pg.aux.begin(), Pg.aux.end()); key.insert(key.end(), Pg.src.begin(), Pg.src.end());
-        key.insert(key.end(), Pg.vloc.begin(), Pg.vloc.end()); key.insert(key.end(), Pg.vred.begin(), Pg.vred.end()); for (unsigned c : Pg.vcnt) key.push_back((int)c);
-        key.insert(key.end(), Pg.vsrc0.begin(), Pg.vsrc0.end()); key.insert(key.end(), Pg.vi.begin(), Pg.vi.end()); key.insert(key.end(), Pg.vsrc.begin(), Pg.vsrc.end());
+        key.reserve((Pg.sh.size() + Pg.ge.size() + Pg.vec.size()) * 4 + Pg.src.size() + Pg.vsrc.size() + 8);
+        key.push_back((int)Pg.sh.size()); key.push_back((int)Pg.ge.size()); key.push_back((int)Pg.vec.size());
+        for (const std::vector<AsRec>* t : { &Pg.sh, &Pg.ge, &Pg.vec }) for (const AsRec& r : *t) { key.push_back(r.x); key.push_back(r.y); key.push_back(r.z); key.push_back(r.w); }
+        key.insert(key.end(), Pg.src.begin(), Pg.src.end()); key.insert(key.end(), Pg.vsrc.begin(), Pg.vsrc.end());
         auto it = seen.find(key);
         if (it == seen.end()) {
-            const int se0 = (int)t_dst.size(), ve0 = (int)tv_loc.size(), so = (int)t_src.size(), vo = (int)tv_src.size();
-            t_dst.insert(t_dst.end(), Pg.dst.begin(), Pg.dst.end()); t_cnt.insert(t_cnt.end(), Pg.cnt.begin(), Pg.cnt.end()); t_aux.insert(t_aux.end(), Pg.aux.begin(), Pg.aux.end());
-            for (int x : Pg.src0) t_src0.push_back(x + so);
+            const int sh0 = (int)t_rec.size(), se0 = sh0 + (int)Pg.sh.size(), ve0 = (int)tv_rec.size(), so = (int)t_src.size(), vo = (int)tv_src.size();
+            t_rec.insert(t_rec.end(), Pg.sh.begin(), Pg.sh.end());
+            for (AsRec r : Pg.ge) { r.z += so; t_rec.push_back(r); }
             t_src.insert(t_src.end(), Pg.src.begin(), Pg.src.end());
-            tv_loc.insert(tv_loc.end(), Pg.vloc.begin(), Pg.vloc.end()); tv_red.insert(tv_red.end(), Pg.vred.begin(), Pg.vred.end()); tv_cnt.insert(tv_cnt.end(), Pg.vcnt.begin(), Pg.vcnt.end());
-            tv_i.insert(tv_i.end(), Pg.vi.begin(), Pg.vi.end());
-            for (int x : Pg.vsrc0) tv_src0.push_back(x + vo);
+            for (AsRec r : Pg.vec) { r.w += vo; tv_rec.push_back(r); }
             tv_src.insert(tv_src.end(), Pg.vsrc.begin(), Pg.vsrc.end());
-            it = seen.emplace(std::move(key), std::array<int, 4>{ se0, (int)Pg.dst.size(), ve0, (int)Pg.vloc.size() }).first;
-        }
-        A.se0 = it->second[0]; A.ne = it->second[1]; A.ve0 = it->second[2]; A.nv = it->second[3];
-        B.as_max_ne = std::max(B.as_max_ne, A.ne); B.as_max_nv = std::max(B.as_max_nv, A.nv);
+            it = seen.emplace(std::move(key), std::array<int, 6>{ sh0, (int)Pg.sh.size(), se0, (int)Pg.ge.size(), ve0, (int)Pg.vec.size() }).first;
+        }
+        A.sh0 = it->second[0]; A.nsh = it->second[1]; A.se0 = it->second[2]; A.ne = it->second[3]; A.ve0 = it->second[4]; A.nv = it->second[5];
+        B.as_max_nsh = std::max(B.as_max_nsh, A.nsh); B.as_max_ne = std::max(B.as_max_ne, A.ne); B.as_max_nv = std::max(B.as_max_nv, A.nv);
     }
     if (overflow) return refuse(err, SWF_E_UNSUPPORTED, "assembly program: more than 4095 contributions to one entry of the reduced system");
     B.asm_programs = (int)seen.size();
-    auto nonempty_i = [](std::vector<int>& v) { if (v.empty()) v.push_back(0); };
-    auto nonempty_u = [](std::vector<unsigned>& v) { if (v.empty()) v.push_back(0u); };
-    nonempty_i(t_dst); nonempty_u(t_cnt); nonempty_i(t_src0); nonempty_i(t_aux); nonempty_i(t_src);
-    nonempty_i(tv_loc); nonempty_i(tv_red); nonempty_u(tv_cnt); nonempty_i(tv_src0); nonempty_i(tv_i); nonempty_i(tv_src);
+    t_src.push_back(0); tv_src.push_back(0);
+    if (t_rec.empty()) t_rec.push_back(AsRec{ 0, 0, 0, 0 });
+    if (tv_rec.empty()) tv_rec.push_back(AsRec{ 0, 0, 0, 0 });
     return SWF_OK;
 }
 
@@ -886,6 +885,7 @@
     PlanShape sh;
     sh.n_cu = n_cu;
     sh.no_lat_fuse = getenv("SWF_NO_LAT_FUSE") != nullptr; sh.no_chol_col = getenv("SWF_NO_CHOL_COL") != nullptr;
+    sh.asm_plain = getenv("SWF_ASM_PLAIN") != nullptr;
     sh.ls_variant = num("SWF_LS_VARIANT"); sh.ls_qpb = num("SWF_LS_QPB"); sh.ls_grad_qpb = num("SWF_LS_GRAD_QPB");
     return sh;
 }
@@ -895,7 +895,7 @@
     B.hw.resize((size_t)n);
     for (int i = 0; i < n; i++) if ((rc = plan_window(B, windows[i], i, B.hw[(size_t)i], err)) != SWF_OK) return rc;
     if (B.n_x > 0x7fffffffLL || B.n_loc > 0x7fffffffLL) return refuse(err, SWF_E_UNSUPPORTED, "batch too large for 32-bit offsets");
-    B.n_win = n; B.n_cu = sh.n_cu;
+    B.n_win = n; B.n_cu = sh.n_cu; B.asm_plain = sh.asm_plain;
     B.n_proj = (int)B.p_win.size(); B.n_lm = (int)B.lm_win.size(); B.n_fsb = (int)B.fsb_win.size();
     B.lat_fuse = n * 8 <= B.n_cu && !sh.no_lat_fuse;
     B.want_aux = (n * 16 <= B.n_cu && !B.lat_fuse) || (2 * n >= B.n_cu && n <= B.n_cu);
@@ -1085,7 +1085,7 @@
     for (const Pair& P : B.pair) NEED(pair_ok(P), "pair", &P - B.pair.data());
     for (const Pair& P : B.pair_d) { NEED(pair_ok(P) && P.is_diag, "pair_d", &P - B.pair_d.data()); wpair[P.win].push_back(&P); }
     for (const Pair& P : B.pair_o) { NEED(pair_ok(P) && !P.is_diag, "pair_o", &P - B.pair_o.data()); wpair[P.win].push_back(&P); }
-    std::map<std::array<int, 4>, std::vector<int>> programs;
+    std::map<std::array<int, 6>, std::vector<int>> programs;
     for (int w = 0; w < n; w++) {
         const WinRec& W = B.win[w];
         NEED(W.n_e + W.n_red == W.n_loc && W.loc_base >= 0 && W.loc_base + W.n_loc <= B.n_loc && W.x_base >= 0 && W.x_base + W.x_n <= B.n_x, "win", w);
@@ -1135,16 +1135,28 @@
             }
         }
         const AsmWin& A = B.asw[w];
-        const long long nS = (long long)B.as_dst.size(), nV = (long long)B.av_loc.size(), mm = A.m;
-        NEED(A.win == w && A.n_red == W.n_red && A.m == 6 * W.nF && A.se0 >= 0 && A.se0 + A.ne <= nS && A.ve0 >= 0 && A.ve0 + A.nv <= nV && A.ne <= B.as_max_ne && A.nv <= B.as_max_nv, "asw", w);
+        const long long nS = (long long)B.as_rec.size(), nV = (long long)B.av_rec.size(), mm = A.m;
+        NEED(A.win == w && A.n_red == W.n_red && A.m == 6 * W.nF && A.sh0 >= 0 && A.nsh >= 0 && A.sh0 + A.nsh <= nS && A.se0 >= 0 && A.ne >= 0 && A.se0 + A.ne <= nS
+             && (A.sh0 + A.nsh <= A.se0 || A.se0 + A.ne <= A.sh0) && A.ve0 >= 0 && A.nv >= 0 && A.ve0 + A.nv <= nV
+             && A.nsh <= B.as_max_nsh && A.ne <= B.as_max_ne && A.nv <= B.as_max_nv && (!B.asm_plain || A.nsh == 0), "asw", w);
         NEED(A.S_base == W.S_base && A.C_base >= 0 && A.v_base >= 0 && A.fs_base >= 0 && A.P_base == W.P_base * GEMM_SPLIT && A.q_base == 6LL * W.fr_base * GEMM_SPLIT && A.loc_base == W.loc_base, "asw", w);
         const long long fs_n = (B.fs_tot - A.fs_base) * FS_VAL, P_n = B.P_tot * GEMM_SPLIT - A.P_base, q_n = (long long)std::max(1, 6 * B.n_fr) * GEMM_SPLIT - A.q_base;
+        const long long src_n = (long long)B.as_src.size() - 1, vsrc_n = (long long)B.av_src.size() - 1;
         std::vector<char> written((size_t)W.n_red * W.n_red, 0);
+        for (int k = A.sh0; k < A.sh0 + A.nsh; k++) {
+            const AsRec& R = B.as_rec[k]; const unsigned cnt = (unsigned)R.y; const int nC = AS_NC(cnt), dst = R.x;
+            NEED(in(dst, 0, (long long)W.n_red * W.n_red) && dst % W.n_red <= dst / W.n_red && !written[dst], "as_rec: short dst", k);
+            written[dst] = 1;
+            NEED(AS_SHORT(cnt) && !(cnt >> 31) && (!AS_SOLD(cnt) || B.s_direct), "as_rec: short class", k);
+            NEED(in(A.C_base + R.z, 0, B.C_tot) && in(A.C_base + R.w, 0, B.C_tot) && (nC > 0 || R.z == 0) && (nC > 1 || R.w == 0), "as_rec: short src", k);
+        }
         for (int k = A.se0; k < A.se0 + A.ne; k++) {
-            const unsigned cnt = B.as_cnt[k]; const int nC = AS_NC(cnt), nP = AS_NP(cnt), nH = AS_NH(cnt), s0 = B.as_src0[k], dst = B.as_dst[k];
-            NEED(in(dst, 0, (long long)W.n_red * W.n_red) && dst % W.n_red <= dst / W.n_red && !written[dst], "as_dst", k);
+            const AsRec& R = B.as_rec[k];
+            const unsigned cnt = (unsigned)R.y; const int nC = AS_NC(cnt), nP = AS_NP(cnt), nH = AS_NH(cnt), s0 = R.z, dst = R.x;
+            NEED(in(dst, 0, (long long)W.n_red * W.n_red) && dst % W.n_red <= dst / W.n_red && !written[dst], "as_rec: dst", k);
             written[dst] = 1;
-            NEED(s0 >= 0 && s0 + nC + nP + nH + (AS_DIAG(cnt) ? nC : 0) <= (long long)B.as_src.size() && in(B.as_aux[k], 0, W.n_loc) && (!AS_SOLD(cnt) || B.s_direct), "as_src0", k);
+            NEED((B.asm_plain || !AS_SHORT(cnt)) && !(cnt >> 31), "as_rec: general class", k);
+            NEED(s0 >= 0 && s0 + nC + nP + nH + (AS_DIAG(cnt) ? nC : 0) <= src_n && in(R.w, 0, W.n_loc) && (!AS_SOLD(cnt) || B.s_direct), "as_rec: src0", k);
             const int* s = &B.as_src[s0];
             for (int c = 0; c < nC; c++) NEED(in(A.C_base + s[c], 0, B.C_tot), "as_src", s0 + c);
             for (int c = nC; c < nC + nP; c++) NEED(in(s[c], 0, P_n) && s[c] < GEMM_SPLIT * mm * mm, "as_src", s0 + c);
@@ -1152,33 +1164,37 @@
             if (AS_DIAG(cnt)) for (int c = nC + nP + nH; c < 2 * nC + nP + nH; c++) NEED(in(A.v_base + s[c], 0, B.v_tot), "as_src", s0 + c);
         }
         for (int k = A.ve0; k < A.ve0 + A.nv; k++) {
-            const unsigned cnt = B.av_cnt[k]; const int nC = AS_NC(cnt), nQ = AS_NP(cnt), nH = AS_NH(cnt), s0 = B.av_src0[k];
-            NEED(in(B.av_loc[k], 0, W.n_loc) && in(B.av_red[k], 0, W.n_red) && in(B.av_i[k], 0, 6) && s0 >= 0 && s0 + nH + nC + nQ <= (long long)B.av_src.size(), "av_src0", k);
+            const AsRec& R = B.av_rec[k];
+            const unsigned cnt = (unsigned)R.z; const int nC = AS_NC(cnt), nQ = AS_NP(cnt), nH = AS_NH(cnt), s0 = R.w;
+            NEED(in(R.x, 0, W.n_loc) && in(R.y, 0, W.n_red) && in(AV_I(cnt), 0, 6) && s0 >= 0 && s0 + nH + nC + nQ <= vsrc_n, "av_rec", k);
             const int* s = &B.av_src[s0];
             for (int c = 0; c < nH; c++) NEED(s[c] >= 0 && s[c] + FS_VAL <= fs_n, "av_src", s0 + c);
             for (int c = nH; c < nH + nC; c++) NEED(in(A.v_base + s[c], 0, B.v_tot), "av_src", s0 + c);
             for (int c = nH + nC; c < nH + nC + nQ; c++) NEED(in(s[c], 0, q_n), "av_src", s0 + c);
         }
         for (const Pair* P : wpair[w]) for (int i = 0; i < P->la; i++) for (int j = 0; j < (P->is_diag ? i + 1 : P->lb); j++)
-            NEED(P->ra + i < W.n_red && P->rb + j < W.n_red && written[(size_t)(P->ra + i) * W.n_red + P->rb + j], "as_dst: an entry of pair_d / pair_o is missing, window", w);
-        std::vector<int>& key = programs[{ A.se0, A.ne, A.ve0, A.nv }];
+            NEED(P->ra + i < W.n_red && P->rb + j < W.n_red && written[(size_t)(P->ra + i) * W.n_red + P->rb + j], "as_rec: an entry of pair_d / pair_o is missing, window", w);
+        std::vector<int>& key = programs[{ A.sh0, A.nsh, A.se0, A.ne, A.ve0, A.nv }];
         if (key.empty()) {
-            key.push_back(A.ne);
+            key.push_back(A.nsh); key.push_back(A.ne);
+            for (int k = A.sh0; k < A.sh0 + A.nsh; k++) { const AsRec& R = B.as_rec[k]; key.push_back(R.x); key.push_back(R.y); key.push_back(R.z); key.push_back(R.w); }
             for (int k = A.se0; k < A.se0 + A.ne; k++) {
-                const unsigned cnt = B.as_cnt[k]; const int len = AS_NC(cnt) * (AS_DIAG(cnt) ? 2 : 1) + AS_NP(cnt) + AS_NH(cnt);
-                key.push_back(B.as_dst[k]); key.push_back((int)cnt); key.push_back(B.as_aux[k]);
-                key.insert(key.end(), &B.as_src[B.as_src0[k]], &B.as_src[B.as_src0[k]] + len);
+                const AsRec& R = B.as_rec[k];
+                const unsigned cnt = (unsigned)R.y; const int len = AS_NC(cnt) * (AS_DIAG(cnt) ? 2 : 1) + AS_NP(cnt) + AS_NH(cnt);
+                key.push_back(R.x); key.push_back(R.y); key.push_back(R.w);
+                key.insert(key.end(), &B.as_src[R.z], &B.as_src[R.z] + len);
             }
             for (int k = A.ve0; k < A.ve0 + A.nv; k++) {
-                const unsigned cnt = B.av_cnt[k]; const int len = AS_NC(cnt) + AS_NP(cnt) + AS_NH(cnt);
-                key.push_back(B.av_loc[k]); key.push_back(B.av_red[k]); key.push_back((int)cnt); key.push_back(B.av_i[k]);
-                key.insert(key.end(), &B.av_src[B.av_src0[k]], &B.av_src[B.av_src0[k]] + len);
+                const AsRec& R = B.av_rec[k];
+                const unsigned cnt = (unsigned)R.z; const int len = AS_NC(cnt) + AS_NP(cnt) + AS_NH(cnt);
+                key.push_back(R.x); key.push_back(R.y); key.push_back(R.z);
+                key.insert(key.end(), &B.av_src[R.w], &B.av_src[R.w] + len);
             }
         }
     }
     NEED((int)programs.size() == B.asm_programs, "asw: programs", programs.size());
     for (auto a = programs.begin(); a != programs.end(); ++a) for (auto b = std::next(a); b != programs.end(); ++b)
-        NEED(a->second != b->second, "asw: two copies of one program, se0", b->first[0]);
+        NEED(a->second != b->second, "asw: two copies of one program, se0", b->first[2]);
     return SWF_OK;
 #undef NEED
 }
diff --git a/rtk_visual_inertial_navigation_amd/csrc/swf_plan.h b/rtk_visual_inertial_navigation_amd/csrc/swf_plan.h
--- a/rtk_visual_inertial_navigation_amd/csrc/swf_plan.h
+++ b/rtk_visual_inertial_navigation_amd/csrc/swf_plan.h
@@ -32,6 +32,7 @@
     int ls_qpb = 0;
     int ls_grad_qpb = 0;
     bool no_chol_col = false;
+    bool asm_plain = false;
 };
 PlanShape plan_shape_from_env(int n_cu);
 
@@ -76,14 +77,15 @@
     std::vector<Clique> clc_rec[5], cle_rec;
     std::vector<AsmWin> asw;
     std::vector<unsigned> s_tnz;
-    std::vector<int> as_dst, as_src0, as_aux, as_src, av_loc, av_red, av_src0, av_i, av_src;
-    std::vector<unsigned> as_cnt, av_cnt;
+    std::vector<AsRec> as_rec, av_rec;
+    std::vector<int> as_src, av_src;
     std::vector<int> co_eo, co_no, co_roff, co_x0off, co_voff, co_iq_f, co_iq_k;
     std::vector<long long> co_pno, co_nno, co_go, co_g2o, co_Joff, co_Coff;
     int n_win = 0, n_proj = 0, n_lm = 0, n_lmb = 0, n_pch = 0, n_fsb = 0, n_pd = 0, n_po = 0, n_cle = 0, n_clc[5] = { 0, 0, 0, 0, 0 };
-    int as_max_ne = 0, as_max_nv = 0;
+    int as_max_nsh = 0, as_max_ne = 0, as_max_nv = 0;
     int n_cu = 256, rr_nmax = 256, max_red = 0, min_red = 1 << 30;
     int ls_qpb = 1, ls_var = 0, ls_kms = 8, ls_gqpb = 4; bool ls_folded = false, s_direct = false;
+    bool asm_plain = false;
     bool lat_fuse = false, want_aux = false, want_Linv = false, want_Wk = false;
     bool clc_imu[5] = { false, false, false, false, false };
     int n_pch_split = 0; bool rr4_has15 = false, rr4_has16 = false;
diff --git a/rtk_visual_inertial_navigation_amd/csrc/swf_records.h b/rtk_visual_inertial_navigation_amd/csrc/swf_records.h
--- a/rtk_visual_inertial_navigation_amd/csrc/swf_records.h
+++ b/rtk_visual_inertial_navigation_amd/csrc/swf_records.h
@@ -84,7 +84,9 @@
     long long q_base;
 };
 
+struct alignas(16) AsRec { int x, y, z, w; };
 struct AsmWin {
+    int sh0, nsh;
     int se0, ne;
     int ve0, nv;
     int n_red, m;
@@ -99,6 +101,8 @@
 #define AS_NH(c) (((c) >> 17) & 4095u)
 #define AS_DIAG(c) (((c) >> 29) & 1u)
 #define AS_SOLD(c) (((c) >> 30) & 1u)
+#define AV_I(c) ((c) >> 29)
+#define AS_SHORT(c) (!AS_DIAG(c) && AS_NP(c) == 0 && AS_NH(c) == 0 && AS_NC(c) <= 2)
 
 struct DevBatch {
     int n_win;
@@ -165,9 +169,9 @@
     int n_pair;
     const long long* pc_coff; const int* pc_cld; const int* pc_voff;
     int n_pd, n_po; const Pair* pair_d; const Pair* pair_o;
-    const AsmWin* asw; int as_max_ne, as_max_nv;
-    const int* as_dst; const unsigned* as_cnt; const int* as_src0; const int* as_aux; const int* as_src;
-    const int* av_loc; const int* av_red; const unsigned* av_cnt; const int* av_src0; const int* av_i; const int* av_src;
+    const AsmWin* asw; int as_max_nsh, as_max_ne, as_max_nv;
+    const AsRec* as_rec; const int* as_src;
+    const AsRec* av_rec; const int* av_src;
     const unsigned* s_tnz;
     int spec;
     int rr_nmax;
```

Result: no change. 695,500 iterations/s (median of 6 runs) (+0.9%).
